# antoni-wojcik/OpenCL-Raytracing

Hardware: AMD Instinct MI355X
Metric: Msamples/sec (rays/sec) at 1920×1080, 64 spp; % HBM roofline (higher is better)
Workload: dtype f32

## Files before the change

### include/rt_amd.h

```cpp
#ifndef RT_AMD_H
#define RT_AMD_H

#include <stddef.h>
#include <stdint.h>

#ifdef __cplusplus
extern "C" {
#endif

#define RT_ABI_VERSION 3

#define RT_OK 0
#define RT_EINVAL (-1)
#define RT_ENODEVICE (-2)
#define RT_EHIP (-3)
#define RT_ESTATE (-4)
#define RT_ERANGE (-5)

#define RT_TRIANGLE_EPSILON 0.0000001f
#define RT_MIN_DISTANCE 0.001f
#define RT_MAX_DISTANCE 1000.0f
#define RT_DEPTH 30
#define RT_RANDOM_BUFFER_SIZE 100000
#define RT_RANDOM_TABLE_FLOATS (4 * RT_RANDOM_BUFFER_SIZE)
// ... 140 lines not shown
int rt_sample_counter(const rt_context *ctx, uint32_t *out);

int rt_clear(rt_context *ctx);
int rt_render_spp(rt_context *ctx, const float camera[12], uint32_t first_sample, uint32_t n_samples);
int rt_resolve(rt_context *ctx);

typedef struct rt_adaptive_params {
    uint32_t batch;
    uint32_t min_spp;
    uint32_t max_spp;
    float threshold;
    uint32_t block_w, block_h;
} rt_adaptive_params;

typedef struct rt_adaptive_stats {
    uint32_t rounds;
    uint64_t pixel_samples;
    uint32_t blocks, blocks_at_max;
} rt_adaptive_stats;

int rt_render_adaptive(rt_context *ctx, const float camera[12], const rt_adaptive_params *p, rt_adaptive_stats *out);
int rt_read_sample_counts(rt_context *ctx, uint32_t *counts, size_t bytes);
int rt_read_block_error(rt_context *ctx, float *err, size_t bytes);

typedef struct rt_feature {
    float pos[3];
    float t;
    float normal[3];
    uint32_t object;
    float albedo[3];
    uint32_t material;
    float dir[3];
    uint32_t face;
    float u, v;
    uint32_t tex;
    uint32_t flags;
} rt_feature;
#define RT_FEATURE_HIT 1u

int rt_render_features(rt_context *ctx, const float camera[12]);
int rt_read_features(rt_context *ctx, rt_feature *out, size_t bytes);
int rt_device_features(rt_context *ctx, void **d_features);

#define RT_FOLLOW_REFLECTIVE 1u
#define RT_FOLLOW_REFRACTIVE 2u
#define RT_FOLLOW_DIELECTRIC 4u
#define RT_FEATURE_CHAIN_MAX 29u
#define RT_FEATURE_CUT 2u
#define RT_FEATURE_CHAIN_LENGTH(flags) (((flags) >> 8) & 31u)
#define RT_FEATURE_CHAIN_SIGNATURE(flags) ((flags) & 0xFFFF0000u)
typedef struct rt_feature_chain_params { uint32_t follow; uint32_t max_chain; } rt_feature_chain_params;
int rt_render_features_chain(rt_context *ctx, const float camera[12], const rt_feature_chain_params *p);
int rt_feature_chain_signature(const uint32_t *objects, uint32_t n, uint32_t *sig_out);

typedef struct rt_denoise_params {
    uint32_t iterations;
    float sigma_color, sigma_normal, sigma_position, sigma_albedo;
    uint32_t flags;
} rt_denoise_params;
#define RT_DENOISE_SPLIT_OBJECTS 1u
#define RT_DENOISE_SPLIT_CHAINS 4u
#define RT_DENOISE_MAX_ITERATIONS 8u

int rt_denoise(rt_context *ctx, const rt_denoise_params *p);
int rt_read_denoised(rt_context *ctx, float *rgba, size_t bytes);
int rt_device_denoised(rt_context *ctx, void **d_rgba);

typedef struct rt_denoise_variance_params {
    uint32_t iterations;
    float sigma_luminance;
    float sigma_normal, sigma_position, sigma_albedo;
    uint32_t flags;
} rt_denoise_variance_params;
#define RT_DENOISE_VARIANCE_EPS 1e-4f

int rt_denoise_variance(rt_context *ctx, const rt_denoise_variance_params *p);
int rt_read_variance(rt_context *ctx, int which, float *out, size_t bytes);
int rt_device_variance(rt_context *ctx, int which, void **d_out);

#define RT_DENOISE_MOMENTS_MIN_COUNT 4u
int rt_read_moments(rt_context *ctx, float *m2, size_t bytes);
int rt_device_moments(rt_context *ctx, void **d_m2);
int rt_moments_merge(uint32_t nA, const float sumA[3], float m2A, uint32_t nB, const float sumB[3], float m2B, float *m2_out);
int rt_denoise_moments(rt_context *ctx, const rt_denoise_variance_params *p);

int rt_sync(rt_context *ctx);

int rt_trace_samples(rt_context *ctx, const float camera[12], const uint32_t *x, const uint32_t *y,
                     const uint32_t *sample, size_t n, float *out_rgb);


int rt_read_image(rt_context *ctx, float *rgba, size_t bytes);

int rt_read_linear(rt_context *ctx, float *rgba, size_t bytes);

int rt_device_image(rt_context *ctx, void **d_rgba);
int rt_device_accum(rt_context *ctx, void **d_rgba);

#define RT_OPT_PREFIX_SHARING 1
#define RT_OPT_MAX_THREADS_PER_LAUNCH 2
#define RT_OPT_SAMPLE_QUEUE 3
#define RT_OPT_ACCEL 4
#define RT_OPT_WALK_SLICES 5
#define RT_OPT_PREFIX_TREE 7
#define RT_OPT_WAVE_FILL 8
#define RT_OPT_PREFIX_CACHE 9
#define RT_OPT_LOOKAHEAD 10
#define RT_OPT_EXACT_GRID 11
#define RT_OPT_MOMENTS 12
#define RT_OPT_ARITH 6
#define RT_ARITH_IEEE 0
#define RT_ARITH_ROCM_OCL_NOCONTRACT 1
#define RT_ARITH_ROCM_OCL 2
int rt_set_option(rt_context *ctx, int option, int value);


int rt_enable_counters(rt_context *ctx, int enable);
int rt_reset_counters(rt_context *ctx);
int rt_get_counters(rt_context *ctx, rt_counters *out);

int rt_debug_check_accel(const rt_scene_desc *scene, uint64_t stats[8], char *err, size_t err_len);

int rt_get_debug_counters(rt_context *ctx, uint64_t out[2]);

int rt_walk_overflow(rt_context *ctx, uint32_t *flags_out);

uint64_t rt_counters_bytes(const rt_counters *c);

int rt_last_kernel_ms(rt_context *ctx, float *ms);

int rt_kernel_ms_history(rt_context *ctx, float *ms, size_t cap, size_t *n_out);

int rt_debug_hit(rt_context *ctx, int kind, const float *rays, const uint32_t *prim, const uint32_t *face, size_t n,
                 float *out12);
int rt_debug_material(rt_context *ctx, int routine, const float *in16, size_t n, float *out9);
int rt_debug_div3(rt_context *ctx, const float *in4, size_t n, float *out6);
int rt_debug_builtin(rt_context *ctx, int op, const float *in8, size_t n, float *out4);
int rt_debug_queue_sums(rt_context *ctx, const float *in3, uint32_t npix, uint32_t count, uint32_t group_log2, float *out4);

int rt_stage_ms_history(rt_context *ctx, float *first_ms, float *second_ms, size_t cap, size_t *n_out);

int rt_prefix_cache_stats(rt_context *ctx, uint64_t *hits, uint64_t *misses);

int rt_lookahead_stats(rt_context *ctx, uint64_t *batches, uint64_t *served, uint64_t *direct, uint64_t *discarded);

int rt_lookahead_plan(int width, int height, int option_value, uint32_t sample_counter, uint32_t *batch_out);

int rt_sample_units(uint32_t seg_cap, uint32_t pixels_per_unit, uint32_t count_light, uint32_t count_heavy, uint32_t *units_out);

int rt_sample_grid_stats(rt_context *ctx, uint64_t *launches, uint64_t *exact, uint64_t *workgroups, uint64_t *live_last);

int rt_debug_live_list(rt_context *ctx, uint32_t out[4]);

int rt_device_info(rt_context *ctx, char *name, size_t name_len, int *cu_count, char *arch, size_t arch_len);

#ifdef __cplusplus
}
#endif
#endif
```

### opencl-raytracing_amd/_abi.py

```python
import ctypes as C

import numpy as np

RT_ABI_VERSION = 3
DEPTH = 30
RANDOM_BUFFER_SIZE = 100000
RANDOM_TABLE_FLOATS = 4 * RANDOM_BUFFER_SIZE
MAX_DIM = 16384
MAX_SAMPLE = 65535

T_REFRACTIVE, T_REFLECTIVE, T_DIELECTRIC, T_DIFFUSE, T_TEXTURED, T_LIGHT = range(6)
MAT_NAMES = {
    "refractive": T_REFRACTIVE,
    "reflective": T_REFLECTIVE,
    "dielectric": T_DIELECTRIC,
    "diffuse": T_DIFFUSE,
    "textured": T_TEXTURED,
    "light": T_LIGHT,
}

MATERIAL = np.dtype([("type", "<i4"), ("_p0", "<i4", (3,)), ("color", "<f4", (4,)), ("extra_data", "<f4"),
                     ("_p1", "<i4", (3,))])
SPHERE = np.dtype([("pos", "<f4", (4,)), ("r", "<f4"), ("mat_ID", "<u4"), ("_p", "<u4", (2,))])
PLANE = np.dtype([("pos", "<f4", (4,)), ("normal", "<f4", (4,)), ("mat_ID", "<u4"), ("_p", "<u4", (3,))])
# ... 4 lines not shown
assert (MATERIAL.itemsize, SPHERE.itemsize, PLANE.itemsize, LENS.itemsize, MESH.itemsize, MODEL.itemsize) == \
    (48, 32, 48, 64, 16, 12)


class SceneDesc(C.Structure):
    _fields_ = [(n, C.c_void_p) for n in ("materials", "spheres", "planes", "lenses", "vertices", "uvs", "indices",
                                          "meshes", "models")] + \
               [(n, C.c_uint32) for n in ("material_count", "sphere_count", "plane_count", "lens_count",
                                          "vertex_count", "uv_count", "index_count", "mesh_count", "model_count",
                                          "_pad")]


COUNTER_FIELDS = ("samples", "bounces", "t_sphere", "t_plane", "t_lens", "t_model", "t_mesh", "t_tri", "h_tri",
                  "h_bounce", "n_scatter", "n_dielectric", "n_texfetch", "image_reads")


class Counters(C.Structure):
    _fields_ = [(n, C.c_uint64) for n in COUNTER_FIELDS]

    def as_dict(self):
        return {n: int(getattr(self, n)) for n in COUNTER_FIELDS}

    def algorithmic_bytes(self):
        c = self
        return (32 * c.t_sphere + 48 * c.t_plane + 64 * c.t_lens + 12 * c.t_model + 16 * c.t_mesh + 60 * c.t_tri +
                36 * c.h_tri + 48 * c.h_bounce + 12 * c.n_scatter + 4 * c.n_dielectric + 64 * c.n_texfetch +
                64 * c.samples + 16 * c.image_reads)


class AdaptiveParams(C.Structure):
    _fields_ = [("batch", C.c_uint32), ("min_spp", C.c_uint32), ("max_spp", C.c_uint32), ("threshold", C.c_float),
                ("block_w", C.c_uint32), ("block_h", C.c_uint32)]


ADAPTIVE_STATS_FIELDS = ("rounds", "pixel_samples", "blocks", "blocks_at_max")


class AdaptiveStats(C.Structure):
    _fields_ = [("rounds", C.c_uint32), ("pixel_samples", C.c_uint64), ("blocks", C.c_uint32),
                ("blocks_at_max", C.c_uint32)]

    def as_dict(self):
        return {n: int(getattr(self, n)) for n in ADAPTIVE_STATS_FIELDS}


def adaptive_prototypes(lib):
    vp, sz = C.c_void_p, C.c_size_t
    lib.rt_render_adaptive.argtypes = [vp, vp, C.POINTER(AdaptiveParams), C.POINTER(AdaptiveStats)]
    lib.rt_read_sample_counts.argtypes = [vp, vp, sz]
    lib.rt_read_block_error.argtypes = [vp, vp, sz]


def block_error_reference(accum, half, block_w, block_h):
    accum = np.asarray(accum, dtype=np.float32)
    half = np.asarray(half, dtype=np.float32)
    h, w = accum.shape[:2]
    with np.errstate(divide="ignore", invalid="ignore", over="ignore"):
        i = accum[..., :3] / accum[..., 3:4]
        a = half[..., :3] / half[..., 3:4]
        d = np.abs(i - a)
        num = (d[..., 0] + d[..., 1]) + d[..., 2]
        den = np.sqrt((i[..., 0] + i[..., 1]) + i[..., 2])
        ok = den > 0
        e = np.where(ok, num / np.where(ok, den, np.float32(1)), np.float32(0)).astype(np.float64)
    by, bx = -(-h // block_h), -(-w // block_w)
    pad = np.full((by * block_h, bx * block_w), np.nan)
    pad[:h, :w] = e
    return np.nanmean(pad.reshape(by, block_h, bx, block_w), axis=(1, 3))


FEATURE = np.dtype([("pos", "<f4", (3,)), ("t", "<f4"), ("normal", "<f4", (3,)), ("object", "<u4"),
                    ("albedo", "<f4", (3,)), ("material", "<u4"), ("dir", "<f4", (3,)), ("face", "<u4"),
                    ("u", "<f4"), ("v", "<f4"), ("tex", "<u4"), ("flags", "<u4")])
assert FEATURE.itemsize == 80
FEATURE_HIT = 1
FEATURE_CUT = 2
FOLLOW_REFLECTIVE, FOLLOW_REFRACTIVE, FOLLOW_DIELECTRIC = 1, 2, 4
FOLLOW_NAMES = {"mirror": FOLLOW_REFLECTIVE, "glass": FOLLOW_REFRACTIVE, "dielectric": FOLLOW_DIELECTRIC}
FEATURE_CHAIN_MAX = 29
NO_ID = 0xFFFFFFFF
OBJECT_KINDS = ("sphere", "plane", "lens", "mesh")
DENOISE_SPLIT_OBJECTS = 1
DENOISE_SPLIT_CHAINS = 4
DENOISE_MAX_ITERATIONS = 8
DENOISE_DEFAULTS = dict(iterations=5, sigma_color=0.5, sigma_normal=0.1, sigma_position=2.0, sigma_albedo=0.2,
                        split_objects=True)


def denoise_flags(split_objects, split_chains=False):
    return (DENOISE_SPLIT_OBJECTS if split_objects else 0) | (DENOISE_SPLIT_CHAINS if split_chains else 0)


class FeatureChainParams(C.Structure):
    _fields_ = [("follow", C.c_uint32), ("max_chain", C.c_uint32)]


class DenoiseParams(C.Structure):
    _fields_ = [("iterations", C.c_uint32), ("sigma_color", C.c_float), ("sigma_normal", C.c_float),
                ("sigma_position", C.c_float), ("sigma_albedo", C.c_float), ("flags", C.c_uint32)]


DENOISE_VARIANCE_EPS = 1e-4
DENOISE_VARIANCE_DEFAULTS = dict(iterations=5, sigma_luminance=4.0, sigma_normal=0.1, sigma_position=2.0,
                                 sigma_albedo=0.2, split_objects=True)


class DenoiseVarianceParams(C.Structure):
    _fields_ = [("iterations", C.c_uint32), ("sigma_luminance", C.c_float), ("sigma_normal", C.c_float),
                ("sigma_position", C.c_float), ("sigma_albedo", C.c_float), ("flags", C.c_uint32)]


def denoise_prototypes(lib):
    vp, sz = C.c_void_p, C.c_size_t
    lib.rt_render_features.argtypes = [vp, vp]
    lib.rt_read_features.argtypes = [vp, vp, sz]
    lib.rt_device_features.argtypes = [vp, C.POINTER(vp)]
    lib.rt_denoise.argtypes = [vp, C.POINTER(DenoiseParams)]
    lib.rt_read_denoised.argtypes = [vp, vp, sz]
    lib.rt_device_denoised.argtypes = [vp, C.POINTER(vp)]
    lib.rt_denoise_variance.argtypes = [vp, C.POINTER(DenoiseVarianceParams)]
    lib.rt_read_variance.argtypes = [vp, C.c_int, vp, sz]
    lib.rt_device_variance.argtypes = [vp, C.c_int, C.POINTER(vp)]
    lib.rt_render_features_chain.argtypes = [vp, vp, C.POINTER(FeatureChainParams)]
    lib.rt_feature_chain_signature.argtypes = [vp, C.c_uint32, C.POINTER(C.c_uint32)]


DENOISE_MOMENTS_MIN_COUNT = 4


def moments_prototypes(lib):
    vp, sz, u32, f32 = C.c_void_p, C.c_size_t, C.c_uint32, C.c_float
    f3 = C.POINTER(f32)
    lib.rt_read_moments.argtypes = [vp, vp, sz]
    lib.rt_device_moments.argtypes = [vp, C.POINTER(vp)]
    lib.rt_moments_merge.argtypes = [u32, f3, f32, u32, f3, f32, f3]
    lib.rt_denoise_moments.argtypes = [vp, C.POINTER(DenoiseVarianceParams)]


def prefix_cache_prototypes(lib):
    lib.rt_prefix_cache_stats.argtypes = [C.c_void_p, C.POINTER(C.c_uint64), C.POINTER(C.c_uint64)]


def lookahead_prototypes(lib):
    p64 = C.POINTER(C.c_uint64)
    lib.rt_lookahead_stats.argtypes = [C.c_void_p, p64, p64, p64, p64]
    lib.rt_lookahead_plan.argtypes = [C.c_int, C.c_int, C.c_int, C.c_uint32, C.POINTER(C.c_uint32)]


def sample_grid_prototypes(lib):
    p64, u32 = C.POINTER(C.c_uint64), C.c_uint32
    lib.rt_sample_units.argtypes = [u32, u32, u32, u32, C.POINTER(u32)]
    lib.rt_sample_grid_stats.argtypes = [C.c_void_p, p64, p64, p64, p64]
    lib.rt_debug_live_list.argtypes = [C.c_void_p, C.POINTER(u32)]


def queue_sums_prototypes(lib):
    u32 = C.c_uint32
    lib.rt_debug_queue_sums.argtypes = [C.c_void_p, C.c_void_p, u32, u32, u32, C.c_void_p]


def split_features(rec):
    return {"position": rec["pos"].copy(), "depth": rec["t"].copy(), "normal": rec["normal"].copy(),
            "albedo": rec["albedo"].copy(), "object": rec["object"].copy(), "material": rec["material"].copy(),
            "face": rec["face"].copy(), "direction": rec["dir"].copy(),
            "uv": np.stack([rec["u"], rec["v"]], axis=-1), "texture": rec["tex"].copy(),
            "hit": (rec["flags"] & FEATURE_HIT) != 0,
            "chain_length": ((rec["flags"] >> 8) & 31).astype(np.uint32),
            "chain_signature": (rec["flags"] & np.uint32(0xFFFF0000)).astype(np.uint32),
            "cut": (rec["flags"] & FEATURE_CUT) != 0, "chain_word": (rec["flags"] >> 8).astype(np.uint32)}


def ptr(a):
    if a is None or a.size == 0:
        return None
    return a.ctypes.data_as(C.c_void_p)
```

### opencl-raytracing_amd/csrc/pt_device.hpp

```cpp
#pragma once
#include "pt_arith.hpp"

namespace PT_NS {

#ifndef PT_RNG_PREFETCH
#define PT_RNG_PREFETCH 0
#endif
#ifndef PT_BEHIND_SKIP
#define PT_BEHIND_SKIP 1
#endif

#ifndef PT_FACE_MASK
#define PT_FACE_MASK 1
#endif
#ifndef PT_NO_MODELS
#define PT_NO_MODELS 0
#endif
#ifndef PT_STAMPS
#define PT_STAMPS 0
#endif
#if PT_STAMPS
#define PT_STAMP(c, k)                                                         \
    do {                                                                       \
        unsigned long long now_ = __builtin_amdgcn_s_memtime();                \
        (c).st[k] += now_ - (c).st_last;                                       \
        (c).st_last = now_;                                                    \
    } while (0)
#else
#define PT_STAMP(c, k) do { } while (0)
#endif


typedef float v4f __attribute__((ext_vector_type(4)));
typedef const v4f __attribute__((address_space(3))) *LdsV4;
PT_DEV float4 lds_ld(LdsV4 p, uint32_t i) {
    v4f t = p[i];
    return make_float4(t.x, t.y, t.z, t.w);
}
PT_DEV LdsV4 lds_ptr(const float4 *generic) { return (LdsV4)generic; }

struct Ctx {
    const DeviceScene &sc;
    LdsV4 lmat;
    LaneCounters *cn;
    LdsV4 lwin = nullptr;
    LdsV4 lpln = nullptr;
    LdsV4 lfaces = nullptr;
#if PT_STAMPS
    mutable unsigned long long st[8] = {0, 0, 0, 0, 0, 0, 0, 0};
    mutable unsigned long long st_last = 0;
#endif
};

PT_DEV float schlick_r0(float ratio) {
    float r0 = (1.0f - ratio) / (1.0f + ratio);
    r0 *= r0;
    return r0;
}

PT_DEV LdsV4 stage_materials(const DeviceScene &sc, float4 *lds) {
    const uint32_t nm = lds_mat_n(sc.material_count), nw = lds_win_n(sc.sphere_count), np = lds_pln_n(sc.plane_count);
    if (nm)
        for (uint32_t i = threadIdx.x; i < sc.material_count; i += blockDim.x) {
            const rt_material &m = sc.materials[i];
            lds[2 * i] = make_float4(m.color.x, m.color.y, m.color.z, m.extra_data);
            float inv = 1.0f / m.extra_data;
            lds[2 * i + 1] = make_float4(__int_as_float(m.type), inv, schlick_r0(m.extra_data), schlick_r0(inv));
        }
    if (nw)
        for (uint32_t i = threadIdx.x; i < sc.sphere_count; i += blockDim.x) {
            const rt_sphere &s = sc.spheres[i];
            lds[nm + 2 * i] = make_float4(s.pos.x, s.pos.y, s.pos.z, s.r);
            lds[nm + 2 * i + 1] = make_float4(__uint_as_float(s.mat_ID), 0.0f, 0.0f, 0.0f);
        }
    if (np)
        for (uint32_t i = threadIdx.x; i < sc.plane_count; i += blockDim.x) {
            const rt_plane &p = sc.planes[i];
            lds[nm + nw + i] = make_float4(p.normal.x, p.normal.y, p.normal.z, __uint_as_float(p.mat_ID));
        }
    __syncthreads();
    return nm ? lds_ptr(lds) : (LdsV4) nullptr;
}
PT_DEV LdsV4 staged_winners(const DeviceScene &sc, const float4 *lds) {
    return lds_win_n(sc.sphere_count) ? lds_ptr(lds + lds_mat_n(sc.material_count)) : (LdsV4) nullptr;
}
PT_DEV LdsV4 staged_planes(const DeviceScene &sc, const float4 *lds) {
    return lds_pln_n(sc.plane_count) ? lds_ptr(lds + lds_mat_n(sc.material_count) + lds_win_n(sc.sphere_count)) : (LdsV4) nullptr;
}

PT_DEV void load_material(const Ctx &c, uint32_t id, int &type, float &extra, V3 &col) {
    if (c.lmat) {
        float4 a = lds_ld(c.lmat, 2 * id);
        type = __float_as_int(lds_ld(c.lmat, 2 * id + 1).x);
        extra = a.w;
        col = mk(a.x, a.y, a.z);
    } else {
        const rt_material &m = c.sc.materials[id];
        type = m.type;
        extra = m.extra_data;
        col = ld3(m.color);
    }
}

PT_DEV uint32_t dir_hash(V3 d) {
    float dp = dot(d, mk(123.9898f, 348.233f, 433.3314f));
    return (uint32_t)fabs((double)dp * 438.5453);
}
struct Rnd {
    V3 v;
    float u;
};
PT_DEV Rnd fetch_rnd(const float *__restrict__ table, V3 dir, uint32_t s_seed, uint32_t gx, uint32_t gy) {
    uint32_t hsh = dir_hash(dir);
    uint32_t iv = (hsh + (s_seed * 2683u + gx * 3931u + gy * 2504u) * 3u) % RT_RANDOM_BUFFER_SIZE;
    uint32_t iu = (hsh + (s_seed * 2683u + gx * 3931u + gy)) % RT_RANDOM_BUFFER_SIZE;
    const float *t = table + iv;
    Rnd r;
    r.v = mk(t[0], t[1], t[2]);
    r.u = table[3 * RT_RANDOM_BUFFER_SIZE + iu];
    return r;
}

PT_DEV uint32_t rnd_base_v(uint32_t sample, uint32_t gx, uint32_t gy) { return (sample * 2683u + gx * 3931u + gy * 2504u) * 3u; }
PT_DEV uint32_t rnd_base_u(uint32_t sample, uint32_t gx, uint32_t gy) { return sample * 2683u + gx * 3931u + gy; }
PT_DEV Rnd fetch_rnd_b(const float *__restrict__ table, V3 dir, uint32_t depth, uint32_t bv, uint32_t bu) {
    uint32_t hsh = dir_hash(dir);
    uint32_t iv = (hsh + bv + depth * 8049u) % RT_RANDOM_BUFFER_SIZE;
    uint32_t iu = (hsh + bu + depth * 2683u) % RT_RANDOM_BUFFER_SIZE;
    const float *t = table + iv;
    Rnd r;
    r.v = mk(t[0], t[1], t[2]);
    r.u = table[3 * RT_RANDOM_BUFFER_SIZE + iu];
    return r;
}

enum : uint32_t { K_SPHERE = 0u << 30, K_PLANE = 1u << 30, K_LENS = 2u << 30, K_MESH = 3u << 30, K_MASK = 3u << 30 };
#define PT_NO_HIT 0xFFFFFFFFu

#define PT_MISS INFINITY
template <bool FAST = false>
PT_DEV float sphere_root(float b, float cc, float dis);
PT_DEV void sphere_disc(const Ray &r, float4 s, float &b, float &cc, float &dis) {
    V3 oc = xyz(s) - r.o;
    b = dot(oc, r.d);
#if PT_CONTRACT
    cc = __builtin_fmaf(-s.w, s.w, dot(oc, oc));
    dis = __builtin_fmaf(b, b, -cc);
#else
    cc = dot(oc, oc) - s.w;
    dis = b * b - cc;
#endif
}
template <bool FAST = false>
PT_DEV float sphere_t(const Ray &r, float4 s) {
    float b, cc, dis;
    sphere_disc(r, s, b, cc, dis);
    return sphere_root<FAST>(b, cc, dis);
}
#define PT_SPHERE_W_IS_RADIUS PT_CONTRACT
#define PT_BVH_END 0x0FFFFFFFu
#ifndef PT_SPHERE_LEAF_EVERY
#define PT_SPHERE_LEAF_EVERY 4u
#endif
PT_DEV bool sphere_needs_roots(float b, float cc, float dis) {
    return dis > 0 && !(PT_BEHIND_SKIP && b < 0.0f && cc > 0.0f && b > (PT_OCL ? -1024.0f : -4096.0f));
}
template <bool FAST = false>
PT_DEV float sphere_roots(float b, float dis) {
    float d = sqrt1<FAST>(dis);
    float t = PT_MISS;
    float t0 = b - d;
    if (in_range(t0)) t = t0;
    else {
        float t1 = b + d;
        if (in_range(t1)) t = t1;
    }
    return t;
}
template <bool FAST>
PT_DEV float sphere_root(float b, float cc, float dis) {
    return sphere_needs_roots(b, cc, dis) ? sphere_roots<FAST>(b, dis) : PT_MISS;
}
#ifndef PT_ROOT_UPDATE
#define PT_ROOT_UPDATE 1
#endif
template <bool FAST>
PT_DEV void sphere_take(const Ray &r, float4 s, uint32_t id, float &best_t, uint32_t &best_id) {
    float b, cc, dis;
    sphere_disc(r, s, b, cc, dis);
    if (sphere_needs_roots(b, cc, dis)) {
        const float t = sphere_roots<FAST>(b, dis);
        if (t < best_t) {
            best_t = t;
            best_id = id;
        }
    }
}
template <class T>
PT_DEV const T *at32(const T *base, uint32_t byte_offset) {
    return reinterpret_cast<const T *>(reinterpret_cast<const char *>(base) + byte_offset);
}

PT_DEV V3 cull_inverse(V3 d) {
    V3 i = mk(__builtin_amdgcn_rcpf(d.x), __builtin_amdgcn_rcpf(d.y), __builtin_amdgcn_rcpf(d.z));
    return mk(fminf(fmaxf(i.x, -1.0e30f), 1.0e30f), fminf(fmaxf(i.y, -1.0e30f), 1.0e30f), fminf(fmaxf(i.z, -1.0e30f), 1.0e30f));
}
template <bool COUNT>
PT_DEV void hit_spheres_bvh(const DeviceScene &sc, const Ray &r, float &best_t, uint32_t &best_id, LaneCounters *cn) {
    float dd = dot(r.d, r.d);
    float c_ray = 2.0e-6f + 2.0f * fabsf(dd - 1.0f) * (__builtin_amdgcn_rcpf(fminf(dd, 1.0f)) * 1.000002f);
    float k_ray = __builtin_amdgcn_sqrtf(2.0f * c_ray) * 1.02f;
    float o_max = fmaxf(fmaxf(fabsf(r.o.x), fabsf(r.o.y)), fabsf(r.o.z));
    V3 inv = cull_inverse(r.d);
    const uint32_t oct = (r.d.x < 0.0f ? 1u : 0u) | (r.d.y < 0.0f ? 2u : 0u) | (r.d.z < 0.0f ? 4u : 0u);

    uint32_t cur = 1u;
    uint32_t best_slot = PT_NO_HIT;
    bool at_leaf = false;
    uint32_t leaf_b = 0, leaf_skip = 0;
    for (uint32_t guard = 0; guard < (PT_SPHERE_LEAF_EVERY + 1u) * sc.bvh_node_count + 8u; guard++) {
      if (cur != PT_BVH_END && !at_leaf) {
        float4 a = *at32(sc.bvh_nodes, cur << 4);
        float4 b = *at32(sc.bvh_links, (cur << 7) + (oct << 4));
        uint32_t skip = __float_as_uint(b.x) & PT_BVH_END;
        {
            const uint32_t axis_bits = __float_as_uint(b.x) & 0x30000000u, child = __float_as_uint(a.w);
            a.w = __uint_as_float(axis_bits);
            b = make_float4(b.y, b.z, b.w, __uint_as_float(child));
        }
        uint32_t A = __float_as_uint(a.w), B = __float_as_uint(b.w);
        asm("" : "+v"(A), "+v"(B), "+v"(skip));
        if (COUNT) cn->c[CN_DBG_BVH_NODES]++;
        const V3 dc = mk(a.x - r.o.x, a.y - r.o.y, a.z - r.o.z);
        float fx = fabsf(dc.x) + b.x, fy = fabsf(dc.y) + b.y, fz = fabsf(dc.z) + b.z;
// ... 701 lines not shown
```

### opencl-raytracing_amd/csrc/pt_kernels.hip

```cpp
#include <hip/hip_runtime.h>

#include <algorithm>

#include "pt_device.hpp"
#include "pt_moments.hpp"
#include "pt_chain.hpp"
#include "rt_context.hpp"
#include "pt_kernels.hpp"

namespace PT_NS {
using namespace rtamd;


PT_DEV uint32_t live_take(const FrameParams &fp, const uint32_t *__restrict__ live_count, uint32_t unit, uint32_t want,
                          uint32_t &first) {
    const uint32_t cap = fp.seg_cap;
    const uint32_t cnt_l = min(live_count[0], cap);
    const uint32_t cnt_h = min(live_count[LIVE_HEAVY_COUNTER], cap - cnt_l);
    const uint32_t units_h = want ? (cnt_h + want - 1u) / want : 0u;
    const bool heavy = unit < units_h;
    const uint32_t cnt = heavy ? cnt_h : cnt_l;
    const unsigned long long start64 = (unsigned long long)(heavy ? unit : unit - units_h) * want;
    const uint32_t start = (uint32_t)min(start64, (unsigned long long)cnt);
    first = (heavy ? cap - cnt_h : 0u) + start;
// ... 214 lines not shown
    if (!COUNT && is_final) {
        uint32_t before = 0;
        for (uint32_t k = 0; k < wv; k++) before += s_wave_f[k];
        FinalPix e;
        e.slot = slot;
        e.r = rec.out.x;
        e.g = rec.out.y;
        e.b = rec.out.z;
        finals[blockIdx.x * 256u + before + lanes_below(fm)] = e;
    }
    if (!COUNT && threadIdx.x == 0) final_n[blockIdx.x] = s_wave_f[0] + s_wave_f[1] + s_wave_f[2] + s_wave_f[3];
    flush_counters<COUNT>(cn, counters, fp.count);
    if (!TREES) return;
    const uint32_t tree0 = s_tree0;
    const uint32_t nt = tree0 < fp.tree_cap ? min(s_wave_g[0] + s_wave_g[1] + s_wave_g[2] + s_wave_g[3], fp.tree_cap - tree0) : 0u;
    if (nt == 0u) return;
    if (glass) {
        uint32_t before = 0;
        for (uint32_t k = 0; k < wv; k++) before += s_wave_g[k];
        const uint32_t j = before + lanes_below(gm);
        if (j < nt) {
            s_tpos[j] = pos;
            fp.trees[tree0 + j].dec[0].hsh = 0u;
        }
    }
    __syncthreads();
    for (uint32_t level = 0; level < PT_TREE_LEVELS; level++) {
        const uint32_t items = 2u * (level ? s_wn[level] : nt);
        for (uint32_t t = threadIdx.x; t < items; t += 256u) {
            const uint32_t e = level ? (uint32_t)s_wait[(level - 1u) & 1u][t >> 1] : (1u << 8) | (t >> 1);
            const uint32_t j = e & 0xFFu, heap = e >> 8, which = t & 1u, tree = tree0 + j;
            if (tree_step<ACCEL>(c, fp.trees + tree, tree, heap, which, level + 1u == PT_TREE_LEVELS, recs + s_tpos[j],
                                 fp.tree_wait + (size_t)tree * PT_TREE_WAITS)) {
                const uint32_t k = atomicAdd(&s_wn[level + 1u], 1u);
                s_wait[level & 1u][k] = (uint16_t)(((2u * heap + which) << 8) | j);
            }
        }
        if (level + 1u < PT_TREE_LEVELS) __syncthreads();
    }
}

__global__ __launch_bounds__(256) void pt_final_replay(FrameParams fp, const FinalPix *__restrict__ finals,
                                                       const uint32_t *__restrict__ final_n, float4 *__restrict__ accum) {
    if (threadIdx.x >= min(final_n[blockIdx.x], 256u)) return;
    const FinalPix e = finals[blockIdx.x * 256u + threadIdx.x];
    uint32_t x = 0, y = 0;
    if (!slot_to_pixel(fp, e.slot, x, y)) return;
    const V3 fsum = final_sum(mk(e.r, e.g, e.b), fp.count, fp.group_log2);
    if (fp.m2) moments_update(accum, fp.m2, (size_t)y * fp.w + x, fsum, fp.count, 0.0f);
    accumulate(accum, (size_t)y * fp.w + x, fsum, fp.count);
}

PT_DEV size_t ring_at(const FrameParams &fp, size_t pix, uint32_t j) {
    return PT_RING_PIXEL_MAJOR ? pix * fp.count + j : j * ((size_t)fp.w * fp.h) + pix;
}

__global__ __launch_bounds__(256) void pt_final_retrace(FrameParams fp, const FinalPix *__restrict__ finals,
                                                        const uint32_t *__restrict__ final_n) {
    if (threadIdx.x >= min(final_n[blockIdx.x], 256u)) return;
    const FinalPix e = finals[blockIdx.x * 256u + threadIdx.x];
    uint32_t x = 0, y = 0;
    if (!slot_to_pixel(fp, e.slot, x, y)) return;
    const size_t pix = (size_t)y * fp.w + x;
    const float4 at = fp.la_image[pix];
    V3 prev = mk(at.x, at.y, at.z);
    const V3 sum = mk(0.0f, 0.0f, 0.0f) + mk(e.r, e.g, e.b);
    for (uint32_t j = 0; j < fp.count; j++) {
        prev = retrace_step(prev, sum, fp.first + j);
        fp.la_ring[ring_at(fp, pix, j)] = make_float4(prev.x, prev.y, prev.z, 1.0f);
    }
}

template <bool COUNT, bool ACCEL>
__global__ __launch_bounds__(256) void pt_samples(DeviceScene sc, FrameParams fp, const PixelRec *__restrict__ recs,
                                                  const uint32_t *__restrict__ live,
                                                  const uint32_t *__restrict__ live_count,
                                                  float4 *__restrict__ accum, unsigned long long *counters) {
    __shared__ float4 s_mat[PT_LDS_STATIC_FLOAT4];
    {
        uint32_t e0 = 0;
        if (live_take(fp, live_count, (blockIdx.x * 256u) >> fp.group_log2, 1u, e0) == 0u) return;
    }
    LaneCounters cn;
    if (COUNT) zero_counters(cn);
    Ctx c{sc, stage_materials(sc, s_mat), &cn};
    c.lwin = staged_winners(sc, s_mat);
    c.lpln = staged_planes(sc, s_mat);

    uint32_t tid = blockIdx.x * 256u + threadIdx.x;
    uint32_t g = 1u << fp.group_log2;
    uint32_t li = tid >> fp.group_log2;
    uint32_t lane = tid & (g - 1u);
    uint32_t entry = 0;
    bool valid = live_take(fp, live_count, li, 1u, entry) != 0u;
    uint32_t x = 0, y = 0;
    V3 sum = mk(0.0f, 0.0f, 0.0f);
    const bool mom = fp.m2 != nullptr;
    LaneMoments lm{0.0f, 0.0f};
    if (valid) {
        uint32_t slot = live[entry];
        (void)slot_to_pixel(fp, slot, x, y);
        PixelRec rec = recs[entry];
        for (uint32_t s = fp.first + lane; s < fp.first + fp.count; s += g) {
            if (COUNT) cn.c[CN_SAMPLES]++;
            const V3 rad = radiance_from_rec<COUNT, ACCEL>(c, rec, s, x, y, fp.trees);
            if (mom) moments_fold(lm, sum, rad);
            sum = sum + rad;
        }
    }
    sum = mom ? group_sum_moments(sum, lm, g) : group_sum(sum, g);
    if (valid && lane == 0) {
        if (mom) moments_update(accum, fp.m2, (size_t)y * fp.w + x, sum, fp.count, lm.m2);
        accumulate(accum, (size_t)y * fp.w + x, sum, fp.count);
    }
    flush_counters<COUNT>(cn, counters, 1);
}

#ifndef QUEUE_SLOTS
#define QUEUE_SLOTS 512
#endif
#ifndef PT_REFILL_MIN
#define PT_REFILL_MIN 1
#endif
#ifndef QUEUE_MAX_PIXELS
#define QUEUE_MAX_PIXELS 16
#endif
#define QUEUE_REC_F4 5u
#define QUEUE_XY_F4 1u
static_assert(sizeof(PixelRec) == QUEUE_REC_F4 * sizeof(float4), "a queue record is a PixelRec");
PT_HD uint32_t queue_pixel_bytes(uint32_t count) { return (QUEUE_REC_F4 + QUEUE_XY_F4) * 16u + count * 3u * 4u; }
PT_HD uint32_t queue_xy_f4(uint32_t pixels_per_wave) { return pixels_per_wave * QUEUE_REC_F4; }
PT_HD uint32_t queue_slot_f4(uint32_t pixels_per_wave) { return pixels_per_wave * (QUEUE_REC_F4 + QUEUE_XY_F4); }
PT_HD uint32_t queue_wave_lds_bytes(uint32_t pixels_per_wave, uint32_t count) {
    return (pixels_per_wave * queue_pixel_bytes(count) + 15u) & ~15u;
}
PT_HD uint32_t queue_faces_f4(const DeviceScene &sc) { return lds_static_used(sc.material_count, sc.sphere_count, sc.plane_count); }
PT_HD uint32_t queue_static_f4(const DeviceScene &sc, uint32_t face_f4) { return queue_faces_f4(sc) + face_f4; }
#ifndef PT_Q_WAVES
#define PT_Q_WAVES 6
#endif
#ifndef PT_Q_WAVES_ACCEL
#define PT_Q_WAVES_ACCEL 5
#endif
#ifndef PT_Q_WAVES_SPHERE_BVH
#define PT_Q_WAVES_SPHERE_BVH 6
#endif
static_assert(QUEUE_SLOTS >= RT_SPP_PER_LAUNCH, "rt_render_spp's launches must fit a wave's sample queue");
#ifndef QUEUE_MIN_SAMPLES
#define QUEUE_MIN_SAMPLES 384u
#endif
#ifndef PT_LDS_GRANULE
#define PT_LDS_GRANULE 1024u
#endif
__host__ inline uint32_t queue_pixels_per_wave(uint32_t count, uint32_t waves, uint32_t static_float4) {
    auto fit = [&](uint32_t waves_per_simd) {
        uint32_t workgroups = waves_per_simd * 4u;
        uint32_t budget = 163840u / workgroups / PT_LDS_GRANULE * PT_LDS_GRANULE;
        uint32_t per_wave = budget - static_float4 * (uint32_t)sizeof(float4) - 15u;
        uint32_t p = per_wave / queue_pixel_bytes(count);
        if (p * count > QUEUE_SLOTS) p = QUEUE_SLOTS / count;
        return p > QUEUE_MAX_PIXELS ? (uint32_t)QUEUE_MAX_PIXELS : p;
    };
    uint32_t p = fit(waves);
    if (p * count < QUEUE_MIN_SAMPLES) {
        uint32_t p5 = fit(5u);
        if (p5 > p) p = p5;
    }
    return p < 1u ? 1u : p;
}
#ifndef PT_UNITS_PER_WAVE_SLOT
#define PT_UNITS_PER_WAVE_SLOT 16u
#endif
#ifndef PT_TREE_MIN_SAMPLES
#define PT_TREE_MIN_SAMPLES 24u
#endif
#ifndef PT_LDS_FACE_CAP
#define PT_LDS_FACE_CAP 64u
#endif

struct alignas(16) QueueF4 { float x, y, z, w; };
struct alignas(16) QueueXY { uint32_t x, y, bv, bu; };
typedef QueueF4 __attribute__((address_space(3))) *LdsQueueF4;
typedef QueueXY __attribute__((address_space(3))) *LdsQueueXY;
typedef float __attribute__((address_space(3))) *LdsF32;
typedef v4f __attribute__((address_space(3))) *LdsV4Rw;
struct WaveQueue {
    LdsQueueF4 rec;
    LdsQueueXY xy;
    LdsF32 slot;
    uint32_t npix;
    uint32_t count;
    uint32_t total;
    uint32_t count_log2;
    float inv_count;
};

PT_DEV WaveQueue queue_stage(const DeviceScene &sc, const FrameParams &fp, const PixelRec *__restrict__ recs,
                             const uint32_t *__restrict__ live, uint32_t npix, uint32_t pix0,
                             uint32_t pixels_per_wave, float4 *lds, uint32_t face_f4) {
    float4 *wave_lds = lds + queue_static_f4(sc, face_f4);
    WaveQueue q;
    q.rec = (LdsQueueF4)wave_lds;
    q.xy = (LdsQueueXY)(wave_lds + queue_xy_f4(pixels_per_wave));
    q.slot = (LdsF32)(wave_lds + queue_slot_f4(pixels_per_wave));
    const uint32_t lane = threadIdx.x;
    q.npix = npix;
    q.count = fp.count;
    q.total = q.npix * q.count;
    for (uint32_t i = lane; i < q.npix * QUEUE_REC_F4; i += 64u) {
        uint32_t p = i / QUEUE_REC_F4, part = i - p * QUEUE_REC_F4;
        const float4 t = reinterpret_cast<const float4 *>(recs + pix0 + p)[part];
        *(LdsV4Rw)(q.rec + i) = v4f{t.x, t.y, t.z, t.w};
    }
    if (lane < q.npix) {
        uint32_t x = 0, y = 0;
        (void)slot_to_pixel(fp, live[pix0 + lane], x, y);
        q.xy[lane].x = x;
        q.xy[lane].y = y;
        q.xy[lane].bv = rnd_base_v(0u, x, y);
        q.xy[lane].bu = rnd_base_u(0u, x, y);
    }
    __builtin_amdgcn_fence(__ATOMIC_SEQ_CST, "wavefront");
    __builtin_amdgcn_wave_barrier();
    q.inv_count = fp.inv_count;
    q.count_log2 = (q.count & (q.count - 1u)) == 0u ? (uint32_t)__builtin_ctz(q.count) : 0xFFu;
    return q;
}

struct QueueEntry {
    float4 q0, q1, q2, q3, q4;
    uint32_t bits, bv, bu;
};
PT_DEV QueueEntry queue_fetch(const WaveQueue &q, const DeviceScene &sc, const FrameParams &fp, uint32_t idx) {
    const uint32_t p = q.count_log2 != 0xFFu ? idx >> q.count_log2 : (uint32_t)(((float)idx + 0.5f) * q.inv_count);
    const uint32_t sample = fp.first + (idx - p * q.count);
    auto part = [&](uint32_t k) {
        const LdsQueueF4 f = q.rec + (QUEUE_REC_F4 * p + k);
        return make_float4(f->x, f->y, f->z, f->w);
    };
    QueueEntry e;
    e.q0 = part(0);
    e.q1 = part(1);
    e.q2 = part(2);
    e.q3 = part(3);
    e.q4 = part(4);
    e.bv = sample * 8049u + q.xy[p].bv;
    e.bu = sample * 2683u + q.xy[p].bu;
    e.bits = __float_as_uint(e.q0.w);
    if ((e.bits & 0xFFu) == REC_TREE) {
        const float4 *lf = tree_leaf(fp.trees + __float_as_uint(e.q4.w), sc.table, e.bu);
        e.q0 = lf[0]; e.q1 = lf[1]; e.q2 = lf[2]; e.q3 = lf[3]; e.q4 = lf[4];
        e.bits = __float_as_uint(e.q0.w);
    }
    return e;
}

PT_DEV void queue_put(const WaveQueue &q, uint32_t idx, V3 rgb) {
    q.slot[3 * idx] = rgb.x;
    q.slot[3 * idx + 1] = rgb.y;
    q.slot[3 * idx + 2] = rgb.z;
}

#ifndef PT_QUEUE_SUMS_TREE
#define PT_QUEUE_SUMS_TREE 1
#endif
PT_DEV V3 queue_lane_sum(const WaveQueue &q, uint32_t p, uint32_t l, uint32_t g) {
    V3 sum = mk(0.0f, 0.0f, 0.0f);
    const uint32_t n = p < q.npix ? q.count : 0u;
    for (uint32_t j = l; j < n; j += g) {
        const LdsF32 sl = q.slot + 3u * (p * q.count + j);
        sum = sum + mk(sl[0], sl[1], sl[2]);
    }
    return sum;
}
template <int OFF>
PT_DEV float row_add(float v) {
    return v + __int_as_float(__builtin_amdgcn_update_dpp(0, __float_as_int(v), 0x100 + OFF, 0xF, 0xF, false));
}
template <int OFF>
PT_DEV V3 row_add(V3 v) { return mk(row_add<OFF>(v.x), row_add<OFF>(v.y), row_add<OFF>(v.z)); }
PT_DEV float row_pair_add(float a, float b) {
    const auto r = __builtin_amdgcn_permlane16_swap(__float_as_uint(a), __float_as_uint(b), false, false);
    return __uint_as_float(r[0]) + __uint_as_float(r[1]);
}
PT_DEV void queue_sums_tree(const WaveQueue &q, const FrameParams &fp, float4 *__restrict__ accum) {
    const uint32_t lane = threadIdx.x, gl = fp.group_log2;
    if (gl >= 5u) {
        const uint32_t half = lane >> 5, i = lane & 31u, g = 1u << gl, row = lane >> 4;
        for (uint32_t pb = 0; pb < q.npix; pb += 4u) {
            V3 a = queue_lane_sum(q, pb + half, i, g), b = queue_lane_sum(q, pb + 2u + half, i, g);
            if (gl == 6u) {
                a = a + queue_lane_sum(q, pb + half, i + 32u, g);
                b = b + queue_lane_sum(q, pb + 2u + half, i + 32u, g);
            }
            V3 sum = mk(row_pair_add(a.x, b.x), row_pair_add(a.y, b.y), row_pair_add(a.z, b.z));
            sum = row_add<1>(row_add<2>(row_add<4>(row_add<8>(sum))));
            const uint32_t p = pb + ((row & 1u) << 1 | row >> 1);
            if (p < q.npix && (lane & 15u) == 0u) accumulate(accum, (size_t)q.xy[p].y * fp.w + q.xy[p].x, sum, q.count);
        }
    } else {
        const uint32_t g = 1u << gl, ppp = 64u >> gl;
        for (uint32_t pb = 0; pb < q.npix; pb += ppp) {
            const uint32_t p = pb + (lane >> gl), l = lane & (g - 1u);
            V3 sum = queue_lane_sum(q, p, l, g);
            if (gl >= 4u) sum = row_add<8>(sum);
            if (gl >= 3u) sum = row_add<4>(sum);
            if (gl >= 2u) sum = row_add<2>(sum);
            if (gl >= 1u) sum = row_add<1>(sum);
            if (p < q.npix && l == 0u) accumulate(accum, (size_t)q.xy[p].y * fp.w + q.xy[p].x, sum, q.count);
        }
    }
}
template <bool MOMENTS, bool BUTTERFLY = false>
PT_DEV void queue_sums(const WaveQueue &q, const FrameParams &fp, float4 *__restrict__ accum) {
    __builtin_amdgcn_fence(__ATOMIC_SEQ_CST, "wavefront");
    __builtin_amdgcn_wave_barrier();
    if (PT_QUEUE_SUMS_TREE && !MOMENTS && !BUTTERFLY) return queue_sums_tree(q, fp, accum);
    const uint32_t lane = threadIdx.x;
    const uint32_t g = 1u << fp.group_log2, ppp = 64u >> fp.group_log2;
    for (uint32_t pb = 0; pb < q.npix; pb += ppp) {
        uint32_t p = pb + (lane >> fp.group_log2), l = lane & (g - 1u);
        V3 sum = mk(0.0f, 0.0f, 0.0f);
        if (p < q.npix)
            for (uint32_t j = l; j < q.count; j += g) {
                const LdsF32 sl = q.slot + 3u * (p * q.count + j);
                sum = sum + mk(sl[0], sl[1], sl[2]);
            }
        sum = group_sum(sum, g);
        if (MOMENTS) {
            const float mean = moments_lum(sum.x, sum.y, sum.z) / (float)q.count;
            float dev2 = 0.0f;
            if (p < q.npix)
                for (uint32_t j = l; j < q.count; j += g) {
                    const LdsF32 sl = q.slot + 3u * (p * q.count + j);
                    const float d = moments_lum(sl[0], sl[1], sl[2]) - mean;
                    dev2 += d * d;
                }
            for (uint32_t off = g >> 1; off > 0; off >>= 1) dev2 += __shfl_xor(dev2, off);
            if (p < q.npix && l == 0) moments_update(accum, fp.m2, (size_t)q.xy[p].y * fp.w + q.xy[p].x, sum, q.count, dev2);
        }
        if (p < q.npix && l == 0) accumulate(accum, (size_t)q.xy[p].y * fp.w + q.xy[p].x, sum, q.count);
    }
}

static_assert(QUEUE_MAX_PIXELS * 4u <= 64u, "queue_replay maps (pixel, channel) to the wave's lanes");
PT_DEV void queue_replay(const WaveQueue &q, const FrameParams &fp) {
    __builtin_amdgcn_fence(__ATOMIC_SEQ_CST, "wavefront");
    __builtin_amdgcn_wave_barrier();
    const uint32_t lane = threadIdx.x, ch = lane & 3u;
    const bool alpha = ch == 3u;
    for (uint32_t pb = 0; pb < q.npix; pb += 16u) {
        const uint32_t p = pb + (lane >> 2);
        if (p >= q.npix) continue;
        const size_t pix = (size_t)q.xy[p].y * fp.w + q.xy[p].x;
        float prev = reinterpret_cast<const float *>(fp.la_image)[4u * pix + ch];
        float *out = reinterpret_cast<float *>(fp.la_ring) + ch;
        const LdsF32 sl = q.slot + 3u * (p * q.count) + (alpha ? 0u : ch);
        for (uint32_t j = 0; j < q.count; j++) {
            prev = retrace_step1(prev, 0.0f + sl[3u * j], fp.first + j);
            out[4u * ring_at(fp, pix, j)] = alpha ? 1.0f : prev;
        }
    }
}

template <bool COUNT, bool ACCEL, int GEOM, int WAVES, bool MOMENTS = false>
__global__ __launch_bounds__(64, WAVES) void pt_samples_q(DeviceScene sc, FrameParams fp, const PixelRec *__restrict__ recs,
                                                    const uint32_t *__restrict__ live,
                                                    const uint32_t *__restrict__ live_count,
                                                    float4 *__restrict__ accum, unsigned long long *counters,
                                                    uint32_t pixels_per_wave) {
    extern __shared__ float4 s_dyn[];
    constexpr bool FAST = PT_OCL && !COUNT && !ACCEL && GEOM != 2;
    uint32_t pix0 = 0;
    const uint32_t npix = live_take(fp, live_count, blockIdx.x, pixels_per_wave, pix0);
    if (npix == 0u) return;
    float4 *s_mat = s_dyn;
    LaneCounters cn;
    if (COUNT) zero_counters(cn);
    Ctx c{sc, stage_materials(sc, s_mat), &cn};
    c.lwin = staged_winners(sc, s_mat);
    c.lpln = staged_planes(sc, s_mat);
    if (GEOM != 0 && fp.lds_face_f4) {
        float4 *s_faces = s_dyn + queue_faces_f4(sc);
        for (uint32_t i = threadIdx.x; i < fp.lds_face_f4; i += blockDim.x) s_faces[i] = sc.faces[i];
        __syncthreads();
        c.lfaces = lds_ptr(s_faces);
    }

    const WaveQueue q = queue_stage(sc, fp, recs, live, npix, pix0, pixels_per_wave, s_dyn, GEOM != 0 ? fp.lds_face_f4 : 0u);

    uint32_t next = 0;
    bool active = false;
    uint32_t idx = 0, depth = 0, bv = 0, bu = 0;
    V3 col = mk(0.0f, 0.0f, 0.0f), out = mk(0.0f, 0.0f, 0.0f);
    Ray r;
    r.o = r.d = mk(0.0f, 0.0f, 0.0f);
    V3 hn = mk(0.0f, 0.0f, 0.0f);
    uint32_t hmat = 0;
    Rnd rnd;
    rnd.v = mk(0.0f, 0.0f, 0.0f);
    rnd.u = 0.0f;

#if PT_STAMPS
    c.st_last = __builtin_amdgcn_s_memtime();
#endif
    while (true) {
        PT_STAMP(c, 5);
        bool need = !active;
        unsigned long long m = __ballot(need);
        if (m && next < q.total && ((uint32_t)__popcll(m) >= PT_REFILL_MIN || m == ~0ull)) {
            uint32_t cand = next + lanes_below(m);
            if (need && cand < q.total) {
                idx = cand;
                const QueueEntry e = queue_fetch(q, sc, fp, idx);
                bv = e.bv;
                bu = e.bu;
                if (COUNT) cn.c[CN_SAMPLES]++;
                depth = (e.bits >> 8) & 0xFFu;
                hn = xyz(e.q1);
                r.o = xyz(e.q0);
                r.d = xyz(e.q2);
                hmat = __float_as_uint(e.q2.w);
                out = xyz(e.q3);
                col = xyz(e.q4);
                if ((e.bits & 0xFFu) == REC_FINAL) {
                    queue_put(q, idx, out);
                } else {
                    if (PT_RNG_PREFETCH) rnd = fetch_rnd_b(sc.table, r.d, depth, bv, bu);
                    active = true;
                }
            }
            next += (uint32_t)__popcll(m);
        }
        if (!__any(active) && next >= q.total) break;
        PT_STAMP(c, 0);
#ifdef PT_EXP_PAD
#define PT_STR2(x) #x
#define PT_STR(x) PT_STR2(x)
#ifdef PT_EXP_PAD_NOP
        asm volatile(".rept " PT_STR(PT_EXP_PAD) "\n\tv_nop\n\t.endr");
#else
        asm volatile(".rept " PT_STR(PT_EXP_PAD) "\n\tv_or_b32 %0, %0, %0\n\t.endr" : "+v"(idx));
#endif
#endif
#ifdef PT_QSTAT
        if (COUNT && __any(active)) {
            uint32_t na = (uint32_t)__popcll(__ballot(active));
            if (threadIdx.x == 0) cn.c[CN_DBG_BVH_NODES] += na;
            if (threadIdx.x == 0) cn.c[CN_DBG_BVH_TESTS] += 64u;
        }
#endif
        if (active) {
            if (!PT_RNG_PREFETCH) rnd = fetch_rnd_b(sc.table, r.d, depth, bv, bu);
            Hit at;
            at.p = r.o;
            at.n = hn;
            at.u = at.v = 0.0f;
            at.tex = 0;
            at.mat = hmat;
            int type;
            float extra;
            V3 mcol;
            load_material(c, hmat, type, extra, mcol);
            scatter<COUNT, FAST>(c, r, out, at, type, extra, col, rnd, false);
            depth++;
            if (depth >= RT_DEPTH) {
                queue_put(q, idx, out);
                active = false;
            }
        }
        PT_STAMP(c, 1);
        if (active) {
            if (PT_RNG_PREFETCH == 1) rnd = fetch_rnd_b(sc.table, r.d, depth, bv, bu);
            V3 res;
            bool done = false;
            Hit h;
            Nearest nb;
            hit_primitives<COUNT, ACCEL, GEOM != 0, FAST>(c, r, nb);
            if (GEOM != 0) hit_models<COUNT, GEOM == 2>(c, r, nb);
            if (!hit_finish<COUNT, GEOM == 0>(c, r, nb, h)) {
                res = mk(0.0f, 0.0f, 0.0f);
                done = true;
            } else {
                if (COUNT) cn.c[CN_H_BOUNCE]++;
                r.o = h.p;
                hn = h.n;
                hmat = h.mat;
                int type;
                float extra;
                load_material(c, h.mat, type, extra, col);
                if (type == RT_LIGHT) {
                    res = vmin(out, col);
                    done = true;
                } else if (type == RT_TEXTURED) {
                    if (COUNT) cn.c[CN_N_TEXFETCH]++;
                    col = texture_rgb(c.sc, h.u, h.v, h.tex);
                }
            }
            if (done) {
                queue_put(q, idx, res);
                active = false;
            } else if (PT_RNG_PREFETCH == 2) {
                rnd = fetch_rnd_b(sc.table, r.d, depth, bv, bu);
            }
        }
        PT_STAMP(c, 4);
    }
#if PT_STAMPS
    if (threadIdx.x == 0 && q.npix)
        for (int k = 0; k < 6; k++) atomicAdd(&counters[(size_t)COUNTER_REPLICAS * COUNTER_STRIDE + k], c.st[k]);
#endif
    if (!COUNT && !MOMENTS && fp.la_ring) queue_replay(q, fp);
    else queue_sums<MOMENTS, COUNT || ACCEL>(q, fp, accum);
    flush_counters<COUNT>(cn, counters, 1);
}

#ifndef PT_WALK_STEPS
#define PT_WALK_STEPS 24u
#endif
#ifndef PT_W_CHEAP_AGAIN
#define PT_W_CHEAP_AGAIN 8u
#endif
#ifndef PT_W_CHEAP_REPEATS
#define PT_W_CHEAP_REPEATS 4u
#endif
#ifndef PT_W_WAVES
#define PT_W_WAVES 6
#endif
#ifndef PT_W_WAVES_MULTI
#define PT_W_WAVES_MULTI 4
#endif
template <bool MULTI, bool MOMENTS = false>
__global__ __launch_bounds__(64, MULTI ? PT_W_WAVES_MULTI : PT_W_WAVES) void pt_samples_w(DeviceScene sc, FrameParams fp, const PixelRec *__restrict__ recs,
                                                    const uint32_t *__restrict__ live,
                                                    const uint32_t *__restrict__ live_count,
                                                    float4 *__restrict__ accum, uint32_t pixels_per_wave,
                                                    const uint2 *__restrict__ jobs, uint32_t n_jobs
#ifdef PT_WSTAT
                                                    , unsigned long long *wstat
#endif
                                                    ) {
    extern __shared__ float4 s_dyn[];
    uint32_t pix0 = 0;
    const uint32_t npix = live_take(fp, live_count, blockIdx.x, pixels_per_wave, pix0);
    if (npix == 0u) return;
    float4 *s_mat = s_dyn;
    Ctx c{sc, stage_materials(sc, s_mat), nullptr};
    c.lwin = staged_winners(sc, s_mat);
    c.lpln = staged_planes(sc, s_mat);
    const WaveQueue q = queue_stage(sc, fp, recs, live, npix, pix0, pixels_per_wave, s_dyn, 0u);

    const uint32_t mesh0 = jobs[0].x, mat0 = jobs[0].y;
    const uint32_t faces0 = sc.meshes[mesh0].face_count;
    const uint32_t root0 = sc.mesh_bvh_root[mesh0];

    uint32_t next = 0;
    bool active = false;
    int phase = 0;
    uint32_t idx = 0, depth = 0, bv = 0, bu = 0;
    V3 col = mk(0.0f, 0.0f, 0.0f), out = mk(0.0f, 0.0f, 0.0f);
    Ray r;
    r.o = r.d = mk(0.0f, 0.0f, 0.0f);
    V3 hn = mk(0.0f, 0.0f, 0.0f);
    uint32_t hmat = 0;
    float nb_t = RT_MAX_DISTANCE;
    uint32_t nb_id = PT_NO_HIT;
    MeshWalk wpos = mesh_walk_start(0);
    uint32_t wbest = 0;
    float wt = 0.0f, wu = 0.0f, wv = 0.0f;
    uint32_t job = 0;
    uint32_t nb_face = 0, nb_mat = 0;
    float nb_u = 0.0f, nb_v = 0.0f;

    auto enter_job = [&]() {
        while (job < n_jobs) {
            const uint32_t mesh_n = jobs[job].x;
            wbest = sc.meshes[mesh_n].face_count;
            wt = wu = wv = 0.0f;
            wpos = mesh_walk_first(sc, r, sc.mesh_bvh_root[mesh_n], wbest);
            if (wpos.cur != PT_MESH_END) return true;
            job++;
        }
        return false;
    };
#ifdef PT_WSTAT
    WalkStat ws = {0, 0, 0, 0, 0};
    unsigned long long it_n = 0, it_active = 0, it_p0 = 0, it_p1 = 0, it_p2 = 0, it_walk_calls = 0;
#endif
    for (unsigned long long guard = ((unsigned long long)q.total + 1ull) * (RT_DEPTH + 2ull) * (3ull * (1ull << 28) / PT_WALK_STEPS + 4ull); guard; guard--) {
        const bool walking = active && phase == 1;
        const bool wants_cheap = (active && phase != 1) || (!active && next < q.total);
        const uint32_t n_cheap = (uint32_t)__popcll(__ballot(wants_cheap));
        const bool any_walk = __any(walking);
        if (n_cheap == 0u && !any_walk) break;
#ifdef PT_WSTAT
        it_n++;
        it_active += __popcll(__ballot(active));
        it_p0 += __popcll(__ballot(active && phase == 0));
        it_p1 += __popcll(__ballot(active && phase == 1));
        it_p2 += __popcll(__ballot(active && phase == 2));
#endif
        if (n_cheap) {
          for (uint32_t again = 0;; again++) {
            if (active && phase == 2) {
                Nearest nb;
                nb.t = nb_t;
                nb.id = nb_id;
                if (MULTI) {
                    nb.face = nb_face;
                    nb.mat = nb_mat;
                    nb.u = nb_u;
                    nb.v = nb_v;
                } else if (wbest < faces0 && wt < RT_MAX_DISTANCE && wt < nb.t) {
                    nb.t = wt;
                    nb.id = K_MESH | mesh0;
                    nb.face = wbest;
                    nb.mat = mat0;
                    nb.u = wu;
                    nb.v = wv;
                }
                V3 res;
                bool done = false;
                Hit h;
                h.p = h.n = mk(0.0f, 0.0f, 0.0f);
                h.u = h.v = 0.0f;
                h.tex = h.mat = 0;
                if (!hit_finish<false>(c, r, nb, h)) {
                    res = mk(0.0f, 0.0f, 0.0f);
                    done = true;
                } else {
                    int type;
                    float extra;
                    load_material(c, h.mat, type, extra, col);
                    if (type == RT_LIGHT) {
                        res = vmin(out, col);
                        done = true;
                    } else if (type == RT_TEXTURED) {
                        col = texture_rgb(c.sc, h.u, h.v, h.tex);
                    }
                }
                phase = 0;
                if (done) {
                    queue_put(q, idx, res);
                    active = false;
                } else {
                    r.o = h.p;
                    hn = h.n;
                    hmat = h.mat;
                }
            }
            bool need = !active;
            unsigned long long m = __ballot(need);
            if (m && next < q.total) {
                uint32_t cand = next + lanes_below(m);
                if (need && cand < q.total) {
                    idx = cand;
                    const QueueEntry e = queue_fetch(q, sc, fp, idx);
                    bv = e.bv;
                    bu = e.bu;
                    if ((e.bits & 0xFFu) == REC_FINAL) {
                        queue_put(q, idx, xyz(e.q3));
                    } else {
                        depth = (e.bits >> 8) & 0xFFu;
                        hn = xyz(e.q1);
                        r.o = xyz(e.q0);
                        r.d = xyz(e.q2);
                        hmat = __float_as_uint(e.q2.w);
// ... 261 lines not shown
        }
        if (t < PT_MISS) {
            nb.t = t;
            hit = hit_finish<false>(c, r, nb, h);
            if (kind == 4) h.mat = h.tex = 0;
        }
    }
    put_hit(out + 12 * (size_t)i, hit, nb.t, h);
}

__global__ __launch_bounds__(256) void pt_debug_material(DeviceScene sc, int routine, const float *__restrict__ in,
                                                         uint32_t n, float *__restrict__ out) {
    __shared__ float4 s_mat[PT_LDS_STATIC_FLOAT4];
    Ctx c{sc, stage_materials(sc, s_mat), nullptr};
    uint32_t i = blockIdx.x * 256u + threadIdx.x;
    if (i >= n) return;
    const float *v = in + 16 * (size_t)i;
    Ray r;
    r.o = mk(0.0f, 0.0f, 0.0f);
    r.d = mk(v[0], v[1], v[2]);
    Hit h;
    h.p = mk(v[3], v[4], v[5]);
    h.n = mk(v[6], v[7], v[8]);
    h.u = h.v = 0.0f;
    h.tex = 0;
    h.mat = __float_as_uint(v[12]);
    V3 out_col = mk(v[9], v[10], v[11]);
    uint32_t seed = __float_as_uint(v[13]), gx = __float_as_uint(v[14]), gy = __float_as_uint(v[15]);
    int type;
    float extra;
    V3 col;
    load_material(c, h.mat, type, extra, col);
    int as_type = routine == 0 ? (type == RT_REFLECTIVE ? RT_REFLECTIVE : -1) : routine == 1 ? RT_REFRACTIVE
                  : routine == 2 ? RT_DIFFUSE : RT_DIELECTRIC;
    Rnd rnd = fetch_rnd(sc.table, r.d, seed, gx, gy);
    if (as_type == -1) {
        float k = 2.0f * dot(r.d, h.n);
        r.o = h.p;
        r.d = normalize(nmad(h.n, k, r.d));
    } else {
        scatter<false>(c, r, out_col, h, as_type, extra, mk(INFINITY, INFINITY, INFINITY), rnd);
    }
    float *o = out + 9 * (size_t)i;
    o[0] = r.o.x; o[1] = r.o.y; o[2] = r.o.z;
    o[3] = r.d.x; o[4] = r.d.y; o[5] = r.d.z;
    o[6] = out_col.x; o[7] = out_col.y; o[8] = out_col.z;
}

__global__ __launch_bounds__(256) void pt_debug_div3(const float *__restrict__ in, uint32_t n, float *__restrict__ out) {
    uint32_t i = blockIdx.x * 256u + threadIdx.x;
    if (i >= n) return;
    V3 a = mk(in[4 * i], in[4 * i + 1], in[4 * i + 2]);
    float d = in[4 * i + 3];
    V3 q = a / d, s = q;
    if (div3_in_range(a, d)) {
        float nd = -d, rr = __builtin_amdgcn_rcpf(d);
        float e = __builtin_fmaf(nd, rr, 1.0f);
        rr = __builtin_fmaf(e, rr, rr);
        s = V3{div_shared(a.x, nd, rr), div_shared(a.y, nd, rr), div_shared(a.z, nd, rr)};
    }
    float *o = out + 6 * (size_t)i;
    o[0] = s.x; o[1] = s.y; o[2] = s.z; o[3] = q.x; o[4] = q.y; o[5] = q.z;
}

__global__ __launch_bounds__(64) void pt_debug_queue_sums(const float *__restrict__ in, uint32_t npix, uint32_t count,
                                                          uint32_t group_log2, float4 *__restrict__ accum) {
    __shared__ float4 s_q[QUEUE_MAX_PIXELS * QUEUE_XY_F4 + (QUEUE_SLOTS * 3u + 3u) / 4u];
    WaveQueue q;
    q.rec = nullptr;
    q.xy = (LdsQueueXY)s_q;
    q.slot = (LdsF32)(s_q + QUEUE_MAX_PIXELS * QUEUE_XY_F4);
    q.npix = npix;
    q.count = count;
    q.total = npix * count;
    q.count_log2 = 0xFFu;
    q.inv_count = 0.0f;
    const uint32_t lane = threadIdx.x;
    if (lane < npix) {
        q.xy[lane].x = lane;
        q.xy[lane].y = 0u;
    }
    for (uint32_t i = lane; i < 3u * q.total; i += 64u) q.slot[i] = in[i];
    FrameParams fp = {};
    fp.w = (int)npix;
    fp.h = 1;
    fp.count = count;
    fp.group_log2 = group_log2;
    queue_sums<false>(q, fp, accum);
}


#define PT_DISPATCH(count_on, accel_on, CALL)                           \
    do {                                                                \
        if (count_on) { if (accel_on) CALL(true, true); else CALL(true, false); }   \
        else { if (accel_on) CALL(false, true); else CALL(false, false); }          \
    } while (0)

static void apply_mask(FrameParams &fp, const BlockMask *mask) {
    if (!mask) return;
    fp.block_active = mask->active;
    fp.blk_w_log2 = mask->w_log2;
    fp.blk_h_log2 = mask->h_log2;
    fp.blocks_x = mask->blocks_x;
}

template <int MODE>
int launch_render(rt_context *ctx, const float cam[12], uint32_t first, uint32_t count, uint32_t glog2, float4 *accum,
                  const BlockMask *mask, float *m2) {
    FrameParams fp = frame_params(ctx, cam, first, count, glog2);
    apply_mask(fp, mask);
    fp.m2 = MODE == MODE_ACCUM ? m2 : nullptr;
    DeviceScene sc = device_scene(ctx);
    uint32_t slots = fp.slot_end;
    if (slots == 0) return RT_OK;
    uint32_t slots_per_launch = ctx->max_threads_per_launch >> glog2;
    if (slots_per_launch == 0) slots_per_launch = 1;
    hipEvent_t *evp = ctx->ev[ctx->ev_count % rt_context::EV_RING];
    HIP_TRY(ctx, hipEventRecord(evp[0], ctx->stream));
    HIP_TRY(ctx, hipEventRecord(evp[2], ctx->stream));
    for (uint32_t b = 0; b < slots; b += slots_per_launch) {
        fp.slot_begin = b;
        fp.slot_end = b + slots_per_launch < slots ? b + slots_per_launch : slots;
        uint64_t threads = (uint64_t)(fp.slot_end - fp.slot_begin) << glog2;
        dim3 grid((unsigned)((threads + 255) / 256)), block(256);
#define PT_CALL(C, A) \
    hipLaunchKernelGGL((pt_render<MODE, C, A>), grid, block, 0, ctx->stream, sc, fp, accum, ctx->image.p, ctx->counters.p)
        PT_DISPATCH(ctx->count_enabled, scene_has_accel(sc), PT_CALL);
#undef PT_CALL
    }
    HIP_TRY(ctx, hipGetLastError());
    HIP_TRY(ctx, hipEventRecord(evp[1], ctx->stream));
    ctx->ev_count++;
    return RT_OK;
}

static int launch_fused_any(rt_context *ctx, const float cam[12], uint32_t first, uint32_t count, uint32_t glog2, float4 *accum,
                            const BlockMask *mask, float4 *ring, float *m2) {
    FrameParams fp = frame_params(ctx, cam, first, count, glog2);
    apply_mask(fp, mask);
    fp.m2 = m2;
    if (ring) {
        if (accum || m2 || mask || ctx->count_enabled || ctx->world != 1 || !ctx->sample_queue || count > QUEUE_SLOTS ||
            (ctx->max_threads_per_launch >> glog2) < fp.slot_end)
            return fail(ctx, RT_EINVAL, "a look-ahead launch needs the sample queue, an unsharded frame in one slot range and no counters");
        fp.la_ring = ring;
        fp.la_image = ctx->image.p;
    }
    DeviceScene sc = device_scene(ctx);
    uint32_t slots = fp.slot_end;
    if (slots == 0) return RT_OK;
    int rc = ensure_slots(ctx, slots);
    if (rc) return rc;
    const rt_context::Slots &ss = ctx->slots;
    uint32_t *live_count = ss.live.p + ss.capacity + 256u;
    uint32_t slots_per_launch = ctx->max_threads_per_launch >> glog2;
    if (slots_per_launch == 0) slots_per_launch = 1;
    rt_context::PrefixCache &pc = ctx->prefix_cache;
    const bool tree_on = ctx->prefix_tree == 2 || (ctx->prefix_tree == 1 && count >= PT_TREE_MIN_SAMPLES);
    const bool keepable = !mask && !ctx->count_enabled && slots_per_launch >= slots;
    uint32_t cam_bits[12];
    memcpy(cam_bits, cam, sizeof cam_bits);
    const bool hit = pc.enabled && pc.valid && keepable && pc.key_generation == pc.generation && pc.key_tree_on == tree_on &&
                     memcmp(pc.key_cam, cam_bits, sizeof cam_bits) == 0;
    pc.valid = false;
    rt_context::SampleGrid &sg = ctx->sample_grid;
    if (!hit) pc.counts_state = rt_context::PrefixCache::COUNTS_UNKNOWN;
    else if (sg.exact && pc.counts_state == rt_context::PrefixCache::COUNTS_UNKNOWN) {
        HIP_TRY(ctx, hipMemcpyAsync(sg.h_counts, live_count, LIVE_COUNT_STRIDE * sizeof(uint32_t), hipMemcpyDeviceToHost, ctx->stream));
        HIP_TRY(ctx, hipEventRecord(sg.counts_ev, ctx->stream));
        pc.counts_state = rt_context::PrefixCache::COUNTS_IN_FLIGHT;
    } else if (sg.exact && pc.counts_state == rt_context::PrefixCache::COUNTS_IN_FLIGHT) {
        const hipError_t q = hipEventQuery(sg.counts_ev);
        if (q == hipSuccess) {
            pc.count_light = sg.h_counts[0];
            pc.count_heavy = sg.h_counts[LIVE_HEAVY_COUNTER];
            pc.counts_state = rt_context::PrefixCache::COUNTS_KNOWN;
        } else {
            (void)hipGetLastError();
            if (q != hipErrorNotReady) return fail(ctx, RT_EHIP, "hipEventQuery: %s", hipGetErrorString(q));
        }
    }
    const bool exact = hit && sg.exact && pc.counts_state == rt_context::PrefixCache::COUNTS_KNOWN;
    hipEvent_t *evp = ctx->ev[ctx->ev_count % rt_context::EV_RING];
    HIP_TRY(ctx, hipEventRecord(evp[0], ctx->stream));
    for (uint32_t b = 0; b < slots; b += slots_per_launch) {
        fp.slot_begin = b;
        fp.slot_end = b + slots_per_launch < slots ? b + slots_per_launch : slots;
        uint32_t n = fp.slot_end - fp.slot_begin;
        if (!hit) HIP_TRY(ctx, hipMemsetAsync(live_count, 0, LIVE_COUNT_STRIDE * sizeof(uint32_t), ctx->stream));
        fp.trees = ss.trees.p;
        fp.tree_wait = ss.tree_wait.p;
        fp.tree_count = live_count + LIVE_TREE_COUNTER;
        fp.tree_cap = (tree_on && !ctx->count_enabled) ? (uint32_t)ss.tree_capacity : 0u;
        const uint32_t prefix_blocks = (n + 255) / 256;
        fp.seg_cap = prefix_blocks * 256u;
        dim3 block(256), grid1(prefix_blocks);
        fp.lds_face_f4 = 0u;
        uint32_t static_f4 = queue_static_f4(sc, 0u);
        const bool sphere_bvh_only = sc.bvh_node_count != 0 && sc.mesh_bvh_root == nullptr;
        const bool simple_geom = sc.lens_count == 0 && sc.model_count == 0;
        const uint32_t q_waves = !scene_has_accel(sc) ? PT_Q_WAVES : ((sphere_bvh_only && simple_geom) ? PT_Q_WAVES_SPHERE_BVH : PT_Q_WAVES_ACCEL);
        uint32_t ppw = queue_pixels_per_wave(count, q_waves, static_f4);
        const uint32_t want_units = (uint32_t)(ctx->cu_count > 0 ? ctx->cu_count : 256) * 4u * 6u * PT_UNITS_PER_WAVE_SLOT;
        const uint32_t ppw_full = (64u + count - 1u) / count;
        const uint32_t ppw_par = !ctx->wave_fill ? QUEUE_MAX_PIXELS : std::max(n / want_units, ppw_full);
        if (ppw > ppw_par) ppw = ppw_par;
        if (PT_FACE_MASK && !simple_geom && sc.mesh_bvh_root == nullptr && !ctx->count_enabled) {
            const size_t nf = ctx->h_faces.size() / 3u - (ctx->h_faces.empty() ? 0u : 1u);
            if (nf > 0 && nf <= PT_LDS_FACE_CAP &&
                queue_pixels_per_wave(count, q_waves, static_f4 + 3u * (uint32_t)nf) >= ppw) {
                fp.lds_face_f4 = 3u * (uint32_t)nf;
                static_f4 = queue_static_f4(sc, fp.lds_face_f4);
            }
        }
        bool queue = ctx->sample_queue && count <= QUEUE_SLOTS;
        auto queue_lds = [&](uint32_t pixels_per_wave) { return static_f4 * sizeof(float4) + (size_t)queue_wave_lds_bytes(pixels_per_wave, count); };
#define PT_LAUNCH_PREFIX(K) \
    hipLaunchKernelGGL(K, grid1, block, 0, ctx->stream, sc, fp, ss.recs.p, ss.live.p, live_count, accum, ctx->counters.p, ss.finals.p, ss.final_n.p)
#define PT_CALL_PREFIX(C, A) PT_LAUNCH_PREFIX((pt_prefix<C, A>))
        bool accel_on = scene_has_accel(sc);
        if (hit && !ring) hipLaunchKernelGGL(pt_final_replay, grid1, block, 0, ctx->stream, fp, ss.finals.p, ss.final_n.p, accum);
        else if (hit) {}
        else if (fp.tree_cap) PT_LAUNCH_PREFIX((accel_on ? pt_prefix<false, true, true> : pt_prefix<false, false, true>));
        else PT_DISPATCH(ctx->count_enabled, accel_on, PT_CALL_PREFIX);
#undef PT_CALL_PREFIX
#undef PT_LAUNCH_PREFIX
        if (ring) hipLaunchKernelGGL(pt_final_retrace, grid1, block, 0, ctx->stream, fp, ss.finals.p, ss.final_n.p);
        HIP_TRY(ctx, hipEventRecord(evp[2], ctx->stream));
        uint32_t launched = 0;
        auto units = [&](uint32_t per_unit) {
            uint32_t u = (fp.seg_cap + per_unit - 1) / per_unit + 1u;
            sg.last_cap = fp.seg_cap;
            sg.last_per_unit = per_unit;
            if (exact) (void)rt_sample_units(fp.seg_cap, per_unit, pc.count_light, pc.count_heavy, &u);
            return u;
        };
#define PT_GRID(U, LAUNCH) do { launched = (U); if (launched) { LAUNCH; } } while (0)
#define PT_CALL_QUEUE_M(C, A, G, W, M) \
    PT_GRID(units(ppw), hipLaunchKernelGGL((pt_samples_q<C, A, G, W, M>), dim3(launched), dim3(64), queue_lds(ppw), ctx->stream, sc, fp, ss.recs.p, ss.live.p, live_count, accum, ctx->counters.p, ppw))
#define PT_CALL_QUEUE_W(C, A, G, W) do { if (fp.m2) PT_CALL_QUEUE_M(C, A, G, W, true); else PT_CALL_QUEUE_M(C, A, G, W, false); } while (0)
#define PT_CALL_QUEUE(C, A)                                                                       \
    do {                                                                                          \
        if (!(A)) { if (simple_geom) PT_CALL_QUEUE_W(C, false, 0, PT_Q_WAVES); else PT_CALL_QUEUE_W(C, false, 1, PT_Q_WAVES); } \
        else if (sphere_bvh_only) { if (simple_geom) PT_CALL_QUEUE_W(C, true, 0, PT_Q_WAVES_SPHERE_BVH); else PT_CALL_QUEUE_W(C, true, 1, PT_Q_WAVES_ACCEL); } \
        else PT_CALL_QUEUE_W(C, true, 2, PT_Q_WAVES_ACCEL);                                       \
    } while (0)
#define PT_CALL_FIXED(C, A) \
    PT_GRID(grid2.x, hipLaunchKernelGGL((pt_samples<C, A>), grid2, block, 0, ctx->stream, sc, fp, ss.recs.p, ss.live.p, live_count, accum, ctx->counters.p))
        if (queue && sc.mesh_bvh_root && ctx->walk_jobs.n && ctx->walk_slices && !ctx->count_enabled) {
            const bool multi = ctx->walk_jobs.n != 1;
            uint32_t ppw_w = queue_pixels_per_wave(count, multi ? PT_W_WAVES_MULTI : PT_W_WAVES, static_f4);
            if (ppw_w > ppw_par) ppw_w = ppw_par;
            launched = units(ppw_w);
            if (launched)
            hipLaunchKernelGGL(fp.m2 ? (multi ? pt_samples_w<true, true> : pt_samples_w<false, true>) : (multi ? pt_samples_w<true> : pt_samples_w<false>), dim3(launched), dim3(64), queue_lds(ppw_w), ctx->stream,
                               sc, fp, ss.recs.p, ss.live.p, live_count, accum, ppw_w, ctx->walk_jobs.p, (uint32_t)ctx->walk_jobs.n
#ifdef PT_WSTAT
                               , ctx->counters.p + COUNTER_REPLICAS * COUNTER_STRIDE + 8
#endif
                               );
        } else if (queue) PT_DISPATCH(ctx->count_enabled, accel_on, PT_CALL_QUEUE);
        else {
            dim3 grid2((unsigned)((((uint64_t)units(1u) << glog2) + 255) / 256));
            PT_DISPATCH(ctx->count_enabled, accel_on, PT_CALL_FIXED);
        }
#undef PT_CALL_QUEUE
#undef PT_CALL_QUEUE_W
#undef PT_CALL_QUEUE_M
#undef PT_CALL_FIXED
#undef PT_GRID
        sg.launches++;
        sg.workgroups += launched;
        if (exact) { sg.exact_launches++; sg.live_last = launched; }
    }
    HIP_TRY(ctx, hipGetLastError());
    HIP_TRY(ctx, hipEventRecord(evp[1], ctx->stream));
    ctx->ev_count++;
    if (hit) pc.hits++; else pc.misses++;
    if (keepable) {
        pc.valid = true;
        pc.key_generation = pc.generation;
        pc.key_tree_on = tree_on;
        memcpy(pc.key_cam, cam_bits, sizeof cam_bits);
    }
    return RT_OK;
}

int launch_fused(rt_context *ctx, const float cam[12], uint32_t first, uint32_t count, uint32_t glog2, float4 *accum,
                 const BlockMask *mask, float *m2) {
    return launch_fused_any(ctx, cam, first, count, glog2, accum, mask, nullptr, m2);
}

int launch_lookahead(rt_context *ctx, const float cam[12], uint32_t first, uint32_t count, float4 *ring) {
    if (!ring || count < 1u) return fail(ctx, RT_EINVAL, "look-ahead launch without a ring");
    return launch_fused_any(ctx, cam, first, count, group_log2_for(count), nullptr, nullptr, ring, nullptr);
}

__global__ __launch_bounds__(256) void pt_face_normals(float4 *__restrict__ rec, uint32_t n) {
    uint32_t i = blockIdx.x * 256u + threadIdx.x;
    if (i >= n) return;
    float4 q0 = rec[3 * (size_t)i], q1 = rec[3 * (size_t)i + 1], q2 = rec[3 * (size_t)i + 2];
    V3 e1 = mk(q0.w, q1.x, q1.y), e2 = mk(q1.z, q1.w, q2.x);
    V3 nn = normalize(cross(e1, e2));
    rec[3 * (size_t)i + 2] = make_float4(q2.x, nn.x, nn.y, nn.z);
}

__global__ __launch_bounds__(256) void pt_debug_builtin(int op, const float *__restrict__ in, uint32_t n, float *__restrict__ out) {
    uint32_t i = blockIdx.x * 256u + threadIdx.x;
    if (i >= n) return;
    const float *a = in + 8 * (size_t)i;
    V3 x = mk(a[0], a[1], a[2]), y = mk(a[3], a[4], a[5]);
    float t = a[6];
    float4 o = make_float4(0.0f, 0.0f, 0.0f, 0.0f);
    if (op == 0) o.x = dot(x, y);
    else if (op == 1) { V3 c = cross(x, y); o = make_float4(c.x, c.y, c.z, 0.0f); }
    else if (op == 2) { V3 c = normalize(x); o = make_float4(c.x, c.y, c.z, 0.0f); }
    else if (op == 3) { o.x = a[0] / a[1]; o.y = 1.0f / a[0]; V3 c = x / t; o.z = c.y; o.w = c.z; }
    else if (op == 4) o.x = sqrt1(a[0]);
    else if (op == 5) o = make_float4(mix1(x.x, y.x, t), mix1(x.y, y.y, t), mix1(x.z, y.z, t), 0.0f);
    else if (op == 6) { V3 c = vmin(x, y); o = make_float4(c.x, c.y, c.z, 0.0f); }
    else if (op == 7) o.x = sign1(a[0]);
    else if (op == 8) o.x = pow5(a[0]);
    else if (op == 9) o.x = __uint_as_float(dir_hash(x));
    else if (op == 10) o.x = sqrt1<true>(a[0]);
    else if (op == 11) { V3 c = normalize<true>(x); o = make_float4(c.x, c.y, c.z, 0.0f); }
    reinterpret_cast<float4 *>(out)[i] = o;
}

namespace {

int ks_launch_render(rt_context *ctx, int mode, const float cam[12], uint32_t first, uint32_t count, uint32_t glog2,
                     float4 *accum, const BlockMask *mask, float *m2) {
    switch (mode) {
        case MODE_ACCUM: return launch_render<MODE_ACCUM>(ctx, cam, first, count, glog2, accum, mask, m2);
        case MODE_TRACE: return launch_render<MODE_TRACE>(ctx, cam, first, count, glog2, accum, mask, m2);
        case MODE_RETRACE: return launch_render<MODE_RETRACE>(ctx, cam, first, count, glog2, accum, mask, m2);
        default: return fail(ctx, RT_EINVAL, "unknown render mode %d", mode);
    }
}

int ks_launch_probe(rt_context *ctx, const FrameParams &fp, const DeviceScene &sc, const uint32_t *d_in, uint32_t n, float *d_out) {
    dim3 grid((n + 255u) / 256u), block(256);
    if (scene_has_accel(sc))
        hipLaunchKernelGGL(pt_probe<true>, grid, block, 0, ctx->stream, sc, fp, d_in, d_in + n, d_in + 2 * (size_t)n, n, d_out);
    else
        hipLaunchKernelGGL(pt_probe<false>, grid, block, 0, ctx->stream, sc, fp, d_in, d_in + n, d_in + 2 * (size_t)n, n, d_out);
    HIP_TRY(ctx, hipGetLastError());
    return RT_OK;
}

int ks_launch_features(rt_context *ctx, const FrameParams &fp, const DeviceScene &sc, rt_feature *d_out) {
    const uint32_t n = (uint32_t)fp.w * (uint32_t)fp.h;
    dim3 grid((n + 255u) / 256u), block(256);
    float4 *o = reinterpret_cast<float4 *>(d_out);
    if (scene_has_accel(sc)) hipLaunchKernelGGL(pt_features<true>, grid, block, 0, ctx->stream, sc, fp, o);
    else hipLaunchKernelGGL(pt_features<false>, grid, block, 0, ctx->stream, sc, fp, o);
    HIP_TRY(ctx, hipGetLastError());
    return RT_OK;
}

int ks_launch_features_chain(rt_context *ctx, const FrameParams &fp, const DeviceScene &sc, uint32_t follow, uint32_t max_chain,
                             rt_feature *d_out) {
    const uint32_t n = (uint32_t)fp.w * (uint32_t)fp.h;
    dim3 grid((n + 255u) / 256u), block(256);
    float4 *o = reinterpret_cast<float4 *>(d_out);
    if (scene_has_accel(sc)) hipLaunchKernelGGL(pt_features_chain<true>, grid, block, 0, ctx->stream, sc, fp, follow, max_chain, o);
    else hipLaunchKernelGGL(pt_features_chain<false>, grid, block, 0, ctx->stream, sc, fp, follow, max_chain, o);
    HIP_TRY(ctx, hipGetLastError());
    return RT_OK;
}

int ks_launch_debug_hit(rt_context *ctx, const DeviceScene &sc, int kind, const float *d_rays, const uint32_t *d_prim,
                        const uint32_t *d_face, uint32_t n, float *d_out) {
    dim3 grid((n + 255u) / 256u), block(256);
    if (scene_has_accel(sc))
        hipLaunchKernelGGL(pt_debug_hit<true>, grid, block, 0, ctx->stream, sc, kind, d_rays, d_prim, d_face, n, d_out);
    else
        hipLaunchKernelGGL(pt_debug_hit<false>, grid, block, 0, ctx->stream, sc, kind, d_rays, d_prim, d_face, n, d_out);
    HIP_TRY(ctx, hipGetLastError());
    return RT_OK;
}

int ks_launch_debug_material(rt_context *ctx, const DeviceScene &sc, int routine, const float *d_in, uint32_t n, float *d_out) {
    hipLaunchKernelGGL(pt_debug_material, dim3((n + 255u) / 256u), dim3(256), 0, ctx->stream, sc, routine, d_in, n, d_out);
    HIP_TRY(ctx, hipGetLastError());
    return RT_OK;
}

int ks_launch_debug_div3(rt_context *ctx, const float *d_in, uint32_t n, float *d_out) {
    hipLaunchKernelGGL(pt_debug_div3, dim3((n + 255u) / 256u), dim3(256), 0, ctx->stream, d_in, n, d_out);
    HIP_TRY(ctx, hipGetLastError());
    return RT_OK;
}

int ks_launch_debug_queue_sums(rt_context *ctx, const float *d_in, uint32_t npix, uint32_t count, uint32_t glog2, float *d_out) {
    if (npix < 1u || npix > QUEUE_MAX_PIXELS || count < 1u || npix * count > QUEUE_SLOTS || glog2 > 6u)
        return fail(ctx, RT_EINVAL, "queue_sums probe: %u pixels of %u samples do not fit one wave's queue", npix, count);
    HIP_TRY(ctx, hipMemsetAsync(d_out, 0, npix * sizeof(float4), ctx->stream));
    hipLaunchKernelGGL(pt_debug_queue_sums, dim3(1), dim3(64), 0, ctx->stream, d_in, npix, count, glog2, (float4 *)d_out);
    HIP_TRY(ctx, hipGetLastError());
    return RT_OK;
}

int ks_launch_face_normals(rt_context *ctx, float4 *d_records, uint32_t n_records) {
    if (n_records == 0) return RT_OK;
    hipLaunchKernelGGL(pt_face_normals, dim3((n_records + 255u) / 256u), dim3(256), 0, ctx->stream, d_records, n_records);
    HIP_TRY(ctx, hipGetLastError());
    return RT_OK;
}

int ks_launch_debug_builtin(rt_context *ctx, int op, const float *d_in, uint32_t n, float *d_out) {
    hipLaunchKernelGGL(pt_debug_builtin, dim3((n + 255u) / 256u), dim3(256), 0, ctx->stream, op, d_in, n, d_out);
    HIP_TRY(ctx, hipGetLastError());
    return RT_OK;
}

const pt::KernelSet g_kernel_set = {
    PT_ARITH,
#if PT_ARITH == 0
    "ieee",
#elif PT_ARITH == 1
    "rocm-opencl-nocontract",
#else
    "rocm-opencl",
#endif
    ks_launch_render, launch_fused, launch_lookahead, ks_launch_probe, ks_launch_features, ks_launch_debug_hit, ks_launch_debug_material, ks_launch_debug_div3,
    ks_launch_face_normals, ks_launch_debug_builtin, ks_launch_debug_queue_sums, ks_launch_features_chain};

}

}

namespace pt {
#if PT_ARITH == 0
const KernelSet *kernel_set_a0() { return &pt_a0::g_kernel_set; }
#elif PT_ARITH == 1
const KernelSet *kernel_set_a1() { return &pt_a1::g_kernel_set; }
#else
const KernelSet *kernel_set_a2() { return &pt_a2::g_kernel_set; }
#endif
}
```

### opencl-raytracing_amd/csrc/pt_kernels.hpp

```cpp
#pragma once
#include "rt_context.hpp"

namespace pt {

struct KernelSet {
    int arith;
    const char *name;
    int (*launch_render)(rt_context *ctx, int mode, const float cam[12], uint32_t first, uint32_t count, uint32_t glog2,
                         float4 *accum, const BlockMask *mask, float *m2);
    int (*launch_fused)(rt_context *ctx, const float cam[12], uint32_t first, uint32_t count, uint32_t glog2,
                        float4 *accum, const BlockMask *mask, float *m2);
    int (*launch_lookahead)(rt_context *ctx, const float cam[12], uint32_t first, uint32_t count, float4 *ring);
    int (*launch_probe)(rt_context *ctx, const FrameParams &fp, const DeviceScene &sc, const uint32_t *d_in, uint32_t n, float *d_out);
    int (*launch_features)(rt_context *ctx, const FrameParams &fp, const DeviceScene &sc, rt_feature *d_out);
    int (*launch_debug_hit)(rt_context *ctx, const DeviceScene &sc, int kind, const float *d_rays, const uint32_t *d_prim,
                            const uint32_t *d_face, uint32_t n, float *d_out);
    int (*launch_debug_material)(rt_context *ctx, const DeviceScene &sc, int routine, const float *d_in, uint32_t n, float *d_out);
    int (*launch_debug_div3)(rt_context *ctx, const float *d_in, uint32_t n, float *d_out);
    int (*launch_face_normals)(rt_context *ctx, float4 *d_records, uint32_t n_records);
    int (*launch_debug_builtin)(rt_context *ctx, int op, const float *d_in, uint32_t n, float *d_out);
    int (*launch_debug_queue_sums)(rt_context *ctx, const float *d_in, uint32_t npix, uint32_t count, uint32_t glog2, float *d_out);
    int (*launch_features_chain)(rt_context *ctx, const FrameParams &fp, const DeviceScene &sc, uint32_t follow, uint32_t max_chain,
                                 rt_feature *d_out);
};

const KernelSet *kernel_set_a0();
const KernelSet *kernel_set_a1();
const KernelSet *kernel_set_a2();

}
```

### opencl-raytracing_amd/csrc/pt_types.hpp

```cpp
#pragma once
#include <hip/hip_runtime.h>
#include <stdint.h>

#include "../../include/rt_amd.h"

namespace pt {

#define PT_DEV __device__ __forceinline__
#define PT_HD __host__ __device__ inline

#define PT_LDS_MATERIALS 64
#define PT_LDS_WINNERS 64
#define PT_SPHERE_BATCH 4

struct DeviceScene {
    const rt_material *materials;
    const rt_sphere *spheres;
    const float4 *sph4;
    const rt_plane *planes;
    const rt_lens *lenses;
    const rt_float3 *vertices;
    const rt_float2 *uvs;
    const uint32_t *indices;
    const rt_mesh *meshes;
    const rt_model *models;
    const float *table;
    const float4 *tex;
    int tex_w, tex_h, tex_layers;
    float tex_wf, tex_hf;
    uint32_t material_count, sphere_count, sphere_batches, plane_count, lens_count, model_count;
    const float4 *faces;
    const uint32_t *mesh_face_base;
    const float4 *mbvh_nodes;
    const float4 *mbvh_faces;
    const uint32_t *mbvh_face_idx;
    const uint32_t *mesh_bvh_root;
    const float4 *bvh_nodes;
    const float4 *bvh_sph;
    const uint32_t *bvh_idx;
    const float4 *bvh_links;
    uint32_t bvh_node_count;
    float bvh_lo[3], bvh_hi[3];
    float bvh_rmax;
    uint32_t *walk_overflow;
};

#define PT_N_COUNTERS 16
struct LaneCounters {
    uint32_t c[PT_N_COUNTERS];
};
enum {
    CN_SAMPLES, CN_BOUNCES, CN_T_SPHERE, CN_T_PLANE, CN_T_LENS, CN_T_MODEL, CN_T_MESH, CN_T_TRI, CN_H_TRI,
    CN_H_BOUNCE, CN_N_SCATTER, CN_N_DIELECTRIC, CN_N_TEXFETCH, CN_IMAGE_READS,
    CN_DBG_BVH_NODES,
    CN_DBG_BVH_TESTS
};

#define PT_LDS_PLANES 16
#define PT_LDS_STATIC_FLOAT4 (2 * PT_LDS_MATERIALS + 2 * PT_LDS_WINNERS + PT_LDS_PLANES)

PT_HD uint32_t lds_mat_n(uint32_t material_count) { return material_count <= PT_LDS_MATERIALS ? 2u * material_count : 0u; }
PT_HD uint32_t lds_win_n(uint32_t sphere_count) { return sphere_count <= PT_LDS_WINNERS ? 2u * sphere_count : 0u; }
PT_HD uint32_t lds_pln_n(uint32_t plane_count) { return plane_count <= PT_LDS_PLANES ? plane_count : 0u; }
PT_HD uint32_t lds_static_used(uint32_t material_count, uint32_t sphere_count, uint32_t plane_count) {
    return lds_mat_n(material_count) + lds_win_n(sphere_count) + lds_pln_n(plane_count);
}

struct PixelRec {
    float4 p_kind;
    float4 n_extra;
    float4 d;
    float4 out;
    float4 col;
};
enum { REC_FINAL = 0, REC_VERTEX = 1, REC_TREE = 2 };

struct FinalPix {
    uint32_t slot;
    float r, g, b;
};

#ifndef PT_TREE_LEVELS
#define PT_TREE_LEVELS 2
#endif
#define PT_TREE_DECISIONS ((1 << PT_TREE_LEVELS) - 1)
#define PT_TREE_LEAVES (1 << PT_TREE_LEVELS)
struct TreeDecision {
    uint32_t hsh;
    float prob;
    uint32_t depth;
    uint16_t child[2];
};
struct PixelTree {
    TreeDecision dec[PT_TREE_DECISIONS + 1];
    PixelRec leaf[PT_TREE_LEAVES];
};
#define PT_TREE_WAITS (PT_TREE_LEAVES - 2)

enum RenderMode { MODE_ACCUM = 0, MODE_TRACE = 1, MODE_RETRACE = 2 };

#ifndef PT_RING_PIXEL_MAJOR
#define PT_RING_PIXEL_MAJOR 0
#endif

struct FrameParams {
    float cam[12];
    int w, h;
    int tile_w_log2, tile_h_log2;
    uint32_t tiles_x, tiles_total;
    uint32_t rank, world;
    uint32_t slot_begin, slot_end;
    uint32_t first, count;
    uint32_t group_log2;
    uint32_t seg_cap;
    float inv_count;
    PixelTree *trees;
    PixelRec *tree_wait;
    uint32_t *tree_count;
    uint32_t tree_cap;
    uint32_t lds_face_f4;
    const uint32_t *block_active;
    uint32_t blk_w_log2, blk_h_log2, blocks_x;
    float4 *la_ring;
    const float4 *la_image;
    float *m2;
};

struct BlockMask {
    const uint32_t *active;
    uint32_t w_log2, h_log2, blocks_x;
};

#define LIVE_COUNT_STRIDE 32u
#define LIVE_TREE_COUNTER 16u
#define LIVE_HEAVY_COUNTER 24u

#define COUNTER_REPLICAS 512
#define COUNTER_STRIDE 16

PT_DEV bool slot_to_pixel(const FrameParams &fp, uint32_t slot, uint32_t &x, uint32_t &y) {
    uint32_t tpix_log2 = fp.tile_w_log2 + fp.tile_h_log2;
    uint32_t k = slot >> tpix_log2, in = slot & ((1u << tpix_log2) - 1u);
    uint32_t t = fp.rank + k * fp.world;
    if (t >= fp.tiles_total) return false;
    uint32_t tx = t % fp.tiles_x, ty = t / fp.tiles_x;
    x = (tx << fp.tile_w_log2) + (in & ((1u << fp.tile_w_log2) - 1u));
    y = (ty << fp.tile_h_log2) + (in >> fp.tile_w_log2);
    return x < (uint32_t)fp.w && y < (uint32_t)fp.h;
}

PT_DEV bool pixel_active(const FrameParams &fp, uint32_t x, uint32_t y) {
    return !fp.block_active || fp.block_active[(y >> fp.blk_h_log2) * fp.blocks_x + (x >> fp.blk_w_log2)] != 0u;
}

#define PT_MESH_BVH_NONE 0xFFFFFFFFu

#define PT_OVF_SPHERE_WALK 1u
#define PT_OVF_MESH_WALK 2u
#define PT_OVF_WALK_SLICES 4u

}
```

### opencl-raytracing_amd/csrc/rt_amd.hip

```cpp
#include <hip/hip_runtime.h>

#include <algorithm>
#include <cmath>
#include <cfloat>
#include <cstdarg>
#include <cstdio>
#include <cstdlib>
#include <cstring>
#include <functional>
#include <mutex>
#include <new>
#include <string>
#include <vector>

#include "rt_context.hpp"
#include "pt_kernels.hpp"
#include "pt_moments.hpp"
#include "pt_chain.hpp"
#include "mesh_bvh_build.hpp"

using namespace pt;
using namespace rtamd;


// ... 419 lines not shown
}


extern "C" {

int rt_abi_version(void) { return RT_ABI_VERSION; }

const char *rt_last_error(const rt_context *ctx) {
    if (ctx) return ctx->error.c_str();
    std::lock_guard<std::mutex> lk(g_err_mutex);
    return g_create_error.c_str();
}

int rt_make_random_table(uint64_t seed, float *out, size_t n) {
    if (!out || n != RT_RANDOM_TABLE_FLOATS) return fail(nullptr, RT_EINVAL, "table must hold %d floats", RT_RANDOM_TABLE_FLOATS);
    make_table(seed, out);
    return RT_OK;
}

int rt_create(int device, int width, int height, rt_context **out) {
    if (!out) return fail(nullptr, RT_EINVAL, "out is NULL");
    *out = nullptr;
    if (width < 1 || height < 1 || width > RT_MAX_DIM || height > RT_MAX_DIM)
        return fail(nullptr, RT_EINVAL, "frame size %dx%d outside 1..%d", width, height, RT_MAX_DIM);
    int n = 0;
    if (hipGetDeviceCount(&n) != hipSuccess || n < 1)
        return fail(nullptr, RT_ENODEVICE, "no HIP device visible (this library has no CPU path)");
    if (device < 0 || device >= n) return fail(nullptr, RT_ENODEVICE, "device %d out of range (%d visible)", device, n);
    hipDeviceProp_t prop;
    if (hipGetDeviceProperties(&prop, device) != hipSuccess) return fail(nullptr, RT_EHIP, "hipGetDeviceProperties failed");
    if (strncmp(prop.gcnArchName, "gfx950", 6) != 0)
        return fail(nullptr, RT_ENODEVICE, "device %d is %s; librt_amd.so carries gfx950 code only", device,
                    prop.gcnArchName);
    rt_context *ctx = new (std::nothrow) rt_context();
    if (!ctx) return fail(nullptr, RT_EHIP, "out of host memory");
    ctx->device = device;
    ctx->dev_name = prop.name;
    ctx->dev_arch = prop.gcnArchName;
    ctx->cu_count = prop.multiProcessorCount;
    int rc = RT_OK;
    auto bail = [&](int code) {
        {
            std::lock_guard<std::mutex> lk(g_err_mutex);
            g_create_error = ctx->error;
        }
        rt_destroy(ctx);
        return code;
    };
    if (hipSetDevice(device) != hipSuccess) { ctx->error = "hipSetDevice failed"; return bail(RT_EHIP); }
    if (hipStreamCreateWithFlags(&ctx->own_stream, hipStreamNonBlocking) != hipSuccess) { ctx->error = "hipStreamCreate failed"; return bail(RT_EHIP); }
    ctx->stream = ctx->own_stream;
    for (int i = 0; i < rt_context::EV_RING; i++)
        if (hipEventCreate(&ctx->ev[i][0]) != hipSuccess || hipEventCreate(&ctx->ev[i][1]) != hipSuccess || hipEventCreate(&ctx->ev[i][2]) != hipSuccess) { ctx->error = "hipEventCreate failed"; return bail(RT_EHIP); }
    if (ctx->counters.alloc(COUNTER_REPLICAS * COUNTER_STRIDE + 32) != hipSuccess ||
        hipMemset(ctx->counters.p, 0, (COUNTER_REPLICAS * COUNTER_STRIDE + 32) * sizeof(unsigned long long)) != hipSuccess) { ctx->error = "counter allocation failed"; return bail(RT_EHIP); }
    ctx->d_walk_overflow = reinterpret_cast<uint32_t *>(ctx->counters.p + COUNTER_REPLICAS * COUNTER_STRIDE + 24);

    ctx->arith = RT_ARITH_IEEE;
    ctx->ks = kernel_set_a0();
    if (const char *e = getenv("RT_PREFIX_CACHE")) ctx->prefix_cache.enabled = strcmp(e, "0") != 0;
    if (const char *e = getenv("RT_LOOKAHEAD")) { if (strcmp(e, "0") == 0) ctx->lookahead.k = 0; }
    if (const char *e = getenv("RT_EXACT_GRID")) ctx->sample_grid.exact = strcmp(e, "0") != 0;
    if (hipHostMalloc((void **)&ctx->sample_grid.h_counts, LIVE_COUNT_STRIDE * sizeof(uint32_t), hipHostMallocDefault) != hipSuccess ||
        hipEventCreateWithFlags(&ctx->sample_grid.counts_ev, hipEventDisableTiming) != hipSuccess) { ctx->error = "live-count read-back allocation failed"; return bail(RT_EHIP); }
    if ((rc = alloc_frame(ctx, width, height)) != RT_OK) return bail(rc);
    if ((rc = rt_set_seed(ctx, 0xC0FFEEull)) != RT_OK) return bail(rc);
    if ((rc = rt_set_textures(ctx, nullptr, 0, 0, 0)) != RT_OK) return bail(rc);
    *out = ctx;
    return RT_OK;
}

void rt_destroy(rt_context *ctx) {
    if (!ctx) return;
    (void)hipSetDevice(ctx->device);
    if (ctx->own_stream) (void)hipStreamSynchronize(ctx->own_stream);
    for (int i = 0; i < rt_context::EV_RING; i++)
        for (int k = 0; k < 3; k++)
            if (ctx->ev[i][k]) (void)hipEventDestroy(ctx->ev[i][k]);
    if (ctx->sample_grid.counts_ev) (void)hipEventDestroy(ctx->sample_grid.counts_ev);
    if (ctx->sample_grid.h_counts) (void)hipHostFree(ctx->sample_grid.h_counts);
    if (ctx->own_stream) (void)hipStreamDestroy(ctx->own_stream);
    delete ctx;
}

int rt_resize(rt_context *ctx, int width, int height) {
    if (!ctx) return RT_EINVAL;
    if (width < 1 || height < 1 || width > RT_MAX_DIM || height > RT_MAX_DIM)
        return fail(ctx, RT_EINVAL, "frame size %dx%d outside 1..%d", width, height, RT_MAX_DIM);
    HIP_TRY(ctx, hipSetDevice(ctx->device));
    HIP_TRY(ctx, hipStreamSynchronize(ctx->stream));
    return alloc_frame(ctx, width, height);
}

int rt_set_stream(rt_context *ctx, void *hip_stream) {
    if (!ctx) return RT_EINVAL;
    HIP_TRY(ctx, hipSetDevice(ctx->device));
    HIP_TRY(ctx, hipStreamSynchronize(ctx->stream));
    ctx->stream = hip_stream ? (hipStream_t)hip_stream : ctx->own_stream;
    ctx->prefix_changed();
    ctx->ev_count = 0;
    return RT_OK;
}

int rt_set_scene(rt_context *ctx, const rt_scene_desc *d) {
    if (!ctx) return RT_EINVAL;
    if (!d) return fail(ctx, RT_EINVAL, "scene is NULL");
    ctx->prefix_changed();
    ctx->walk_jobs.release();
    struct { const void *p; uint32_t n; const char *name; } arrs[] = {
        {d->materials, d->material_count, "materials"}, {d->spheres, d->sphere_count, "spheres"},
        {d->planes, d->plane_count, "planes"}, {d->lenses, d->lens_count, "lenses"},
        {d->vertices, d->vertex_count, "vertices"}, {d->uvs, d->uv_count, "uvs"},
        {d->indices, d->index_count, "indices"}, {d->meshes, d->mesh_count, "meshes"},
        {d->models, d->model_count, "models"}};
    for (auto &a : arrs)
        if (a.n && !a.p) return fail(ctx, RT_EINVAL, "%s: count %u but NULL pointer", a.name, a.n);
    if (d->uv_count != 0 && d->uv_count != d->vertex_count)
        return fail(ctx, RT_EINVAL, "uv_count (%u) must be 0 or vertex_count (%u)", d->uv_count, d->vertex_count);
    for (uint32_t i = 0; i < d->material_count; i++)
        if (d->materials[i].type < 0 || d->materials[i].type > RT_LIGHT)
            return fail(ctx, RT_EINVAL, "material %u has unknown type %d", i, d->materials[i].type);
    for (uint32_t i = 0; i < d->sphere_count; i++)
        if (d->spheres[i].mat_ID >= d->material_count) return fail(ctx, RT_ERANGE, "sphere %u: material %u does not exist", i, d->spheres[i].mat_ID);
    for (uint32_t i = 0; i < d->plane_count; i++)
        if (d->planes[i].mat_ID >= d->material_count) return fail(ctx, RT_ERANGE, "plane %u: material %u does not exist", i, d->planes[i].mat_ID);
    for (uint32_t i = 0; i < d->lens_count; i++)
        if (d->lenses[i].mat_ID >= d->material_count) return fail(ctx, RT_ERANGE, "lens %u: material %u does not exist", i, d->lenses[i].mat_ID);
    bool uses_tex = false;
    uint32_t max_tex = 0;
    for (uint32_t i = 0; i < d->model_count; i++) {
        const rt_model &mo = d->models[i];
        if (mo.mat_ID >= d->material_count) return fail(ctx, RT_ERANGE, "model %u: material %u does not exist", i, mo.mat_ID);
        if ((uint64_t)mo.mesh_anchor + mo.mesh_count > d->mesh_count) return fail(ctx, RT_ERANGE, "model %u: meshes [%u,+%u) outside the mesh array (%u)", i, mo.mesh_anchor, mo.mesh_count, d->mesh_count);
        bool textured = d->materials[mo.mat_ID].type == RT_TEXTURED;
        for (uint32_t k = 0; k < mo.mesh_count; k++) {
            const rt_mesh &me = d->meshes[mo.mesh_anchor + k];
            if (textured) {
                uses_tex = true;
                if (me.texture_ID > max_tex) max_tex = me.texture_ID;
            }
        }
    }
    for (uint32_t i = 0; i < d->mesh_count; i++) {
        const rt_mesh &me = d->meshes[i];
        if ((uint64_t)me.index_anchor + 3ull * me.face_count > d->index_count)
            return fail(ctx, RT_ERANGE, "mesh %u: indices [%u,+3*%u) outside the index array (%u)", i, me.index_anchor, me.face_count, d->index_count);
        for (uint64_t k = 0; k < 3ull * me.face_count; k++)
            if ((uint64_t)me.vertex_anchor + d->indices[me.index_anchor + k] >= d->vertex_count)
                return fail(ctx, RT_ERANGE, "mesh %u: vertex index %u (+anchor %u) outside the vertex array (%u)", i, d->indices[me.index_anchor + k], me.vertex_anchor, d->vertex_count);
    }
    HIP_TRY(ctx, hipSetDevice(ctx->device));
    HIP_TRY(ctx, hipStreamSynchronize(ctx->stream));
    ctx->have_scene = false;
    HIP_TRY(ctx, ctx->materials.upload(d->materials, d->material_count));
    HIP_TRY(ctx, ctx->spheres.upload(d->spheres, d->sphere_count));
    ctx->h_spheres.assign(d->spheres, d->spheres + d->sphere_count);
    ctx->h_bvh_idx.clear();
    {
        std::vector<uint32_t> base;
        std::vector<float4> fr;
        if (!build_face_records(d, base, fr)) return fail(ctx, RT_EINVAL, "too many faces");
        HIP_TRY(ctx, ctx->mesh_face_base.upload(base.data(), d->mesh_count));
        std::vector<float4> nodes, lfaces;
        std::vector<uint32_t> lidx, roots(d->mesh_count ? d->mesh_count : 1, PT_MESH_BVH_NONE);
        ctx->have_mesh_bvh = false;
        for (uint32_t m = 0; m < d->mesh_count; m++) {
            if (d->meshes[m].face_count < MESH_BVH_MIN_FACES || d->meshes[m].face_count >= (1u << 27)) continue;
            MeshBvhBuilder mb;
            mb.rec = &fr[3 * (size_t)base[m]];
            mb.n_faces = d->meshes[m].face_count;
            mb.nodes = &nodes;
            mb.leaf_faces = &lfaces;
            mb.leaf_idx = &lidx;
            roots[m] = mb.build();
            ctx->have_mesh_bvh = true;
        }
        if (nodes.size() / 4 >= (1u << 26) || lidx.size() >= (1u << 26)) ctx->have_mesh_bvh = false;
        if (nodes.empty()) nodes.resize(4, make_float4(0, 0, 0, 0));
        if (lfaces.empty()) lfaces.resize(3, make_float4(0, 0, 0, 0));
        {
            std::vector<uint8_t> is_root(nodes.size() / 4, 0);
            for (uint32_t m = 0; m < d->mesh_count; m++) if (roots[m] != PT_MESH_BVH_NONE && roots[m] < is_root.size()) is_root[roots[m]] = 1;
            mesh_collapse_links(nodes, is_root);
            std::vector<float4> packed(nodes.size() / 4 * 3);
            for (size_t n = 0; n < nodes.size() / 4; n++) mesh_node_pack(&nodes[4 * n], &packed[3 * n]);
            HIP_TRY(ctx, ctx->mbvh_nodes.upload(packed.data(), packed.size()));
        }
        ctx->h_faces.swap(fr);
        ctx->h_mbvh_faces.swap(lfaces);
        HIP_TRY(ctx, ctx->mbvh_face_idx.upload(lidx.data(), lidx.size()));
        HIP_TRY(ctx, ctx->mesh_bvh_root.upload(roots.data(), d->mesh_count));
        std::vector<uint2> jobs;
        bool all_bvh = ctx->have_mesh_bvh && d->model_count > 0;
        for (uint32_t mo = 0; mo < d->model_count && all_bvh; mo++)
            for (uint32_t k = 0; k < d->models[mo].mesh_count && all_bvh; k++) {
                uint32_t mi = d->models[mo].mesh_anchor + k;
                all_bvh = mi < d->mesh_count && roots[mi] != PT_MESH_BVH_NONE;
                jobs.push_back(make_uint2(mi, d->models[mo].mat_ID));
            }
        if (all_bvh && !jobs.empty() && jobs.size() < (1u << 16)) HIP_TRY(ctx, ctx->walk_jobs.upload(jobs.data(), jobs.size()));
    }
    ctx->bvh_node_count = 0;
    if (d->sphere_count > 0 && d->sphere_count < (1u << 24)) {
        bool finite = true;
        for (uint32_t i = 0; i < d->sphere_count && finite; i++)
            finite = std::isfinite(d->spheres[i].pos.x) && std::isfinite(d->spheres[i].pos.y) &&
                     std::isfinite(d->spheres[i].pos.z) && std::isfinite(d->spheres[i].r);
        if (finite) {
            BvhBuild bb;
            bb.sph = d->spheres;
            bb.order.resize(d->sphere_count);
            for (uint32_t i = 0; i < d->sphere_count; i++) bb.order[i] = i;
            bb.build(0, d->sphere_count);
            {
                std::vector<float4> boxes(bb.nodes.size() / 4), links(bb.nodes.size() * 2);
                for (size_t n = 0; n < bb.nodes.size() / 4; n++) {
                    boxes[n] = bb.nodes[4 * n];
                    boxes[n].w = bb.nodes[4 * n + 1].w;
                    uint32_t A, s8[8];
                    memcpy(&A, &bb.nodes[4 * n].w, 4);
                    memcpy(s8, &bb.nodes[4 * n + 2], 32);
                    for (int o = 0; o < 8; o++) {
                        const uint32_t w = s8[o] | (A & 0x30000000u);
                        float4 &l = links[8 * n + o];
                        l = make_float4(0.0f, bb.nodes[4 * n + 1].x, bb.nodes[4 * n + 1].y, bb.nodes[4 * n + 1].z);
                        memcpy(&l.x, &w, 4);
                    }
                }
                HIP_TRY(ctx, ctx->bvh_nodes.upload(boxes.data(), boxes.size()));
                HIP_TRY(ctx, ctx->bvh_links.upload(links.data(), links.size()));
            }
            HIP_TRY(ctx, ctx->bvh_idx.upload(bb.leaf_idx.data(), bb.leaf_idx.size()));
            ctx->h_bvh_idx = bb.leaf_idx;
            ctx->bvh_node_count = (bb.nodes.size() / 4 < (1u << 25) && bb.leaf_sph.size() < (1u << 28)) ? (uint32_t)(bb.nodes.size() / 4) : 0u;
            ctx->bvh_rmax = 0;
            for (int k = 0; k < 3; k++) { ctx->bvh_lo[k] = INFINITY; ctx->bvh_hi[k] = -INFINITY; }
            for (uint32_t i = 0; i < d->sphere_count; i++) {
                const float c[3] = {d->spheres[i].pos.x, d->spheres[i].pos.y, d->spheres[i].pos.z};
                for (int k = 0; k < 3; k++) { ctx->bvh_lo[k] = std::fmin(ctx->bvh_lo[k], c[k]); ctx->bvh_hi[k] = std::fmax(ctx->bvh_hi[k], c[k]); }
                ctx->bvh_rmax = std::fmax(ctx->bvh_rmax, std::fabs(d->spheres[i].r));
            }
        }
    }
    HIP_TRY(ctx, ctx->planes.upload(d->planes, d->plane_count));
    HIP_TRY(ctx, ctx->lenses.upload(d->lenses, d->lens_count));
    HIP_TRY(ctx, ctx->vertices.upload(d->vertices, d->vertex_count));
    if (d->uv_count) HIP_TRY(ctx, ctx->uvs.upload(d->uvs, d->uv_count));
    else {
        std::vector<rt_float2> zeros(d->vertex_count ? d->vertex_count : 1, rt_float2{0.0f, 0.0f});
        HIP_TRY(ctx, ctx->uvs.upload(zeros.data(), d->vertex_count));
    }
    HIP_TRY(ctx, ctx->indices.upload(d->indices, d->index_count));
    HIP_TRY(ctx, ctx->meshes.upload(d->meshes, d->mesh_count));
    HIP_TRY(ctx, ctx->models.upload(d->models, d->model_count));
    ctx->scene_uses_textures = uses_tex;
    ctx->max_texture_id = max_tex;
    {
        int rc = apply_arith(ctx);
        if (rc != RT_OK) return rc;
    }
    ctx->have_scene = true;
    ctx->sample_counter = 0;
    return RT_OK;
}

int rt_set_textures(rt_context *ctx, const float *rgba, int w, int h, int layers) {
    if (!ctx) return RT_EINVAL;
    ctx->prefix_changed();
    HIP_TRY(ctx, hipSetDevice(ctx->device));
    HIP_TRY(ctx, hipStreamSynchronize(ctx->stream));
    if (layers == 0) {
        float4 zero = make_float4(0.0f, 0.0f, 0.0f, 0.0f);
        HIP_TRY(ctx, ctx->tex.upload(&zero, 1));
        ctx->tex_w = ctx->tex_h = 1;
        ctx->tex_layers = 0;
        return RT_OK;
    }
    if (!rgba || w < 1 || h < 1 || layers < 1 || w > 32768 || h > 32768 || layers > 2048)
        return fail(ctx, RT_EINVAL, "bad texture array %dx%dx%d", w, h, layers);
    HIP_TRY(ctx, ctx->tex.upload((const float4 *)rgba, (size_t)w * h * layers));
    ctx->tex_w = w;
    ctx->tex_h = h;
    ctx->tex_layers = layers;
    return RT_OK;
}

int rt_set_random_table(rt_context *ctx, const float *table, size_t n) {
    if (!ctx) return RT_EINVAL;
    if (!table || n != RT_RANDOM_TABLE_FLOATS) return fail(ctx, RT_EINVAL, "table must hold %d floats", RT_RANDOM_TABLE_FLOATS);
    ctx->prefix_changed();
    HIP_TRY(ctx, hipSetDevice(ctx->device));
    HIP_TRY(ctx, hipStreamSynchronize(ctx->stream));
    HIP_TRY(ctx, ctx->table.upload(table, n));
    return RT_OK;
}

int rt_set_seed(rt_context *ctx, uint64_t seed) {
    if (!ctx) return RT_EINVAL;
    std::vector<float> t(RT_RANDOM_TABLE_FLOATS);
    make_table(seed, t.data());
    return rt_set_random_table(ctx, t.data(), t.size());
}

int rt_get_random_table(rt_context *ctx, float *out, size_t n) {
    if (!ctx) return RT_EINVAL;
    if (!out || n != RT_RANDOM_TABLE_FLOATS) return fail(ctx, RT_EINVAL, "table must hold %d floats", RT_RANDOM_TABLE_FLOATS);
    HIP_TRY(ctx, hipSetDevice(ctx->device));
// ... 846 lines not shown
    DeviceScene sc = device_scene(ctx);
    return debug_roundtrip(ctx, in16, 16 * n * sizeof(float), out9, 9 * n * sizeof(float), [&](void *d_in, void *d_out) {
        return ctx->ks->launch_debug_material(ctx, sc, routine, (const float *)d_in, (uint32_t)n, (float *)d_out);
    });
}

int rt_debug_div3(rt_context *ctx, const float *in4, size_t n, float *out6) {
    if (!ctx || !in4 || !out6 || n > (1u << 28)) return RT_EINVAL;
    if (n == 0) return RT_OK;
    HIP_TRY(ctx, hipSetDevice(ctx->device));
    return debug_roundtrip(ctx, in4, 4 * n * sizeof(float), out6, 6 * n * sizeof(float), [&](void *d_in, void *d_out) {
        return ctx->ks->launch_debug_div3(ctx, (const float *)d_in, (uint32_t)n, (float *)d_out);
    });
}

int rt_debug_queue_sums(rt_context *ctx, const float *in3, uint32_t npix, uint32_t count, uint32_t group_log2, float *out4) {
    if (!ctx || !in3 || !out4) return RT_EINVAL;
    if (npix < 1u || npix > 16u || count < 1u || npix * (uint64_t)count > 512u || group_log2 > 6u)
        return fail(ctx, RT_EINVAL, "queue_sums probe: %u pixels of %u samples do not fit one wave's queue", npix, count);
    HIP_TRY(ctx, hipSetDevice(ctx->device));
    return debug_roundtrip(ctx, in3, (size_t)npix * count * 3 * sizeof(float), out4, (size_t)npix * 4 * sizeof(float), [&](void *d_in, void *d_out) {
        return ctx->ks->launch_debug_queue_sums(ctx, (const float *)d_in, npix, count, group_log2, (float *)d_out);
    });
}

int rt_shard_slots(rt_context *ctx, int world, uint32_t *slots_out) {
    if (!ctx || !slots_out || world < 1) return RT_EINVAL;
    uint32_t tw = 1u << ctx->tile_w_log2, th = 1u << ctx->tile_h_log2;
    uint32_t tiles = ((ctx->width + tw - 1) / tw) * ((ctx->height + th - 1) / th);
    *slots_out = ((tiles + world - 1) / world) * tw * th;
    return RT_OK;
}

int rt_pack_accum(rt_context *ctx, void *d_packed, size_t bytes) {
    if (!ctx || !d_packed) return RT_EINVAL;
    uint32_t n = 0;
    rt_shard_slots(ctx, ctx->world, &n);
    if (bytes != (size_t)n * sizeof(float4)) return fail(ctx, RT_EINVAL, "packed buffer must be %zu bytes", (size_t)n * sizeof(float4));
    HIP_TRY(ctx, hipSetDevice(ctx->device));
    float cam0[12] = {0};
    FrameParams fp = frame_params(ctx, cam0, 0, 0, 0);
    hipLaunchKernelGGL(pt_pack, dim3((n + 255) / 256), dim3(256), 0, ctx->stream, fp, ctx->accum.p, (float4 *)d_packed, n);
    HIP_TRY(ctx, hipGetLastError());
    return RT_OK;
}

int rt_unpack_accum(rt_context *ctx, const void *d_packed, size_t bytes, int src_rank, int world) {
    if (!ctx || !d_packed) return RT_EINVAL;
    if (world < 1 || src_rank < 0 || src_rank >= world) return fail(ctx, RT_EINVAL, "rank %d of %d", src_rank, world);
    uint32_t n = 0;
    rt_shard_slots(ctx, world, &n);
    if (bytes != (size_t)n * sizeof(float4)) return fail(ctx, RT_EINVAL, "packed buffer must be %zu bytes", (size_t)n * sizeof(float4));
    HIP_TRY(ctx, hipSetDevice(ctx->device));
    float cam0[12] = {0};
    FrameParams fp = frame_params(ctx, cam0, 0, 0, 0, src_rank, world);
    if (fp.slot_end)
        hipLaunchKernelGGL(pt_unpack, dim3((fp.slot_end + 255) / 256), dim3(256), 0, ctx->stream, fp, (const float4 *)d_packed, ctx->accum.p);
    HIP_TRY(ctx, hipGetLastError());
    return RT_OK;
}

int rt_set_option(rt_context *ctx, int option, int value) {
    if (!ctx) return RT_EINVAL;
    ctx->prefix_changed();
    switch (option) {
        case RT_OPT_PREFIX_CACHE: ctx->prefix_cache.enabled = value != 0; return RT_OK;
        case RT_OPT_PREFIX_SHARING: ctx->prefix_sharing = value != 0; return RT_OK;
        case RT_OPT_SAMPLE_QUEUE: ctx->sample_queue = value != 0; return RT_OK;
        case RT_OPT_WALK_SLICES: ctx->walk_slices = value != 0; return RT_OK;
        case RT_OPT_WAVE_FILL: ctx->wave_fill = value != 0; return RT_OK;
        case RT_OPT_EXACT_GRID: ctx->sample_grid.exact = value != 0; return RT_OK;
        case RT_OPT_MOMENTS:
            if (value != 0 && value != 1) return fail(ctx, RT_EINVAL, "RT_OPT_MOMENTS takes 0 or 1");
            if (value == 1 && ctx->world > 1)
                return fail(ctx, RT_EINVAL, "sample moments on a sharded context (rank %d of %d)", ctx->rank, ctx->world);
            if ((value != 0) != ctx->moments.on) ctx->moments.valid = false;
            ctx->moments.on = value != 0;
            return RT_OK;
        case RT_OPT_LOOKAHEAD:
            if (value < 0 || value == 1 || value > RT_LOOKAHEAD_MAX) return fail(ctx, RT_EINVAL, "RT_OPT_LOOKAHEAD takes 0 or 2..%d", RT_LOOKAHEAD_MAX);
            ctx->lookahead.k = value;
            ctx->lookahead.ring_failed = false;
            return RT_OK;
        case RT_OPT_PREFIX_TREE:
            if (value < 0 || value > 2) return fail(ctx, RT_EINVAL, "RT_OPT_PREFIX_TREE takes 0, 1 or 2");
            ctx->prefix_tree = value;
            return RT_OK;
        case RT_OPT_ACCEL:
            if (value < 0 || value > 2) return fail(ctx, RT_EINVAL, "RT_OPT_ACCEL takes 0, 1 or 2");
            ctx->accel = value;
            return RT_OK;
        case RT_OPT_ARITH: {
            const KernelSet *ks = value == RT_ARITH_IEEE ? kernel_set_a0() : value == RT_ARITH_ROCM_OCL_NOCONTRACT ? kernel_set_a1()
                                  : value == RT_ARITH_ROCM_OCL ? kernel_set_a2() : nullptr;
            if (!ks) return fail(ctx, RT_EINVAL, "RT_OPT_ARITH takes RT_ARITH_IEEE (0), RT_ARITH_ROCM_OCL_NOCONTRACT (1) or RT_ARITH_ROCM_OCL (2)");
            HIP_TRY(ctx, hipSetDevice(ctx->device));
            HIP_TRY(ctx, hipStreamSynchronize(ctx->stream));
            ctx->arith = value;
            ctx->ks = ks;
            ctx->sample_counter = 0;
            return ctx->have_scene ? apply_arith(ctx) : RT_OK;
        }
        case RT_OPT_MAX_THREADS_PER_LAUNCH:
            if (value < 256) return fail(ctx, RT_EINVAL, "max threads per launch must be >= 256");
            ctx->max_threads_per_launch = (uint32_t)value;
            return RT_OK;
        default: return fail(ctx, RT_EINVAL, "unknown option %d", option);
    }
}

int rt_prefix_cache_stats(rt_context *ctx, uint64_t *hits, uint64_t *misses) {
    if (!ctx || !hits || !misses) return RT_EINVAL;
    *hits = ctx->prefix_cache.hits;
    *misses = ctx->prefix_cache.misses;
    return RT_OK;
}

int rt_sample_units(uint32_t seg_cap, uint32_t pixels_per_unit, uint32_t count_light, uint32_t count_heavy, uint32_t *units_out) {
    if (!units_out) return fail(nullptr, RT_EINVAL, "units_out is NULL");
    *units_out = 0;
    if (pixels_per_unit == 0) return fail(nullptr, RT_EINVAL, "pixels_per_unit is 0");
    const uint32_t cnt_l = std::min(count_light, seg_cap);
    const uint32_t cnt_h = std::min(count_heavy, seg_cap - cnt_l);
    const uint32_t units_h = cnt_h / pixels_per_unit + (cnt_h % pixels_per_unit != 0u);
    const uint32_t units_l = cnt_l / pixels_per_unit + (cnt_l % pixels_per_unit != 0u);
    *units_out = units_h + units_l;
    return RT_OK;
}

int rt_sample_grid_stats(rt_context *ctx, uint64_t *launches, uint64_t *exact, uint64_t *workgroups, uint64_t *live_last) {
    if (!ctx || !launches || !exact || !workgroups || !live_last) return RT_EINVAL;
    *launches = ctx->sample_grid.launches;
    *exact = ctx->sample_grid.exact_launches;
    *workgroups = ctx->sample_grid.workgroups;
    *live_last = ctx->sample_grid.live_last;
    return RT_OK;
}

int rt_debug_live_list(rt_context *ctx, uint32_t out[4]) {
    if (!ctx || !out) return RT_EINVAL;
    const rt_context::Slots &ss = ctx->slots;
    if (!ss.live.p || ctx->sample_grid.last_per_unit == 0) return fail(ctx, RT_EINVAL, "no fused launch yet");
    HIP_TRY(ctx, hipSetDevice(ctx->device));
    uint32_t h[LIVE_COUNT_STRIDE];
    HIP_TRY(ctx, hipMemcpyAsync(h, ss.live.p + ss.capacity + 256u, sizeof h, hipMemcpyDeviceToHost, ctx->stream));
    HIP_TRY(ctx, hipStreamSynchronize(ctx->stream));
    out[0] = ctx->sample_grid.last_cap;
    out[1] = ctx->sample_grid.last_per_unit;
    out[2] = h[0];
    out[3] = h[LIVE_HEAVY_COUNTER];
    return RT_OK;
}

int rt_reset_counters(rt_context *ctx) {
    if (!ctx) return RT_EINVAL;
    HIP_TRY(ctx, hipSetDevice(ctx->device));
    HIP_TRY(ctx, hipMemsetAsync(ctx->counters.p, 0, COUNTER_REPLICAS * COUNTER_STRIDE * sizeof(unsigned long long), ctx->stream));
    HIP_TRY(ctx, hipMemsetAsync(ctx->d_walk_overflow, 0, sizeof(uint32_t), ctx->stream));
    return RT_OK;
}

int rt_get_counters(rt_context *ctx, rt_counters *out) {
    if (!ctx || !out) return RT_EINVAL;
    HIP_TRY(ctx, hipSetDevice(ctx->device));
    std::vector<unsigned long long> h(COUNTER_REPLICAS * COUNTER_STRIDE);
    HIP_TRY(ctx, hipMemcpyAsync(h.data(), ctx->counters.p, h.size() * sizeof(unsigned long long), hipMemcpyDeviceToHost, ctx->stream));
    HIP_TRY(ctx, hipStreamSynchronize(ctx->stream));
    uint64_t *o = (uint64_t *)out;
    for (int i = 0; i < 14; i++) {
        o[i] = 0;
        for (int r = 0; r < COUNTER_REPLICAS; r++) o[i] += h[(size_t)r * COUNTER_STRIDE + i];
    }
    return RT_OK;
}

int rt_get_debug_counters(rt_context *ctx, uint64_t out[2]) {
    if (!ctx || !out) return RT_EINVAL;
    HIP_TRY(ctx, hipSetDevice(ctx->device));
    std::vector<unsigned long long> h(COUNTER_REPLICAS * COUNTER_STRIDE);
    HIP_TRY(ctx, hipMemcpyAsync(h.data(), ctx->counters.p, h.size() * sizeof(unsigned long long), hipMemcpyDeviceToHost, ctx->stream));
    HIP_TRY(ctx, hipStreamSynchronize(ctx->stream));
    out[0] = out[1] = 0;
    for (int r = 0; r < COUNTER_REPLICAS; r++) {
        out[0] += h[(size_t)r * COUNTER_STRIDE + 14];
        out[1] += h[(size_t)r * COUNTER_STRIDE + 15];
    }
#ifdef PT_WSTAT
    {
        unsigned long long v[12];
        if (hipMemcpy(v, ctx->counters.p + COUNTER_REPLICAS * COUNTER_STRIDE + 8, sizeof v, hipMemcpyDeviceToHost) == hipSuccess) {
            const char *names[12] = {"outer iterations", "active lanes", "phase-0 lanes", "phase-1 lanes", "phase-2 lanes", "walk slices",
                                     "walk steps", "node-test lanes", "(unused)", "leaf phases", "leaf lanes", "finished (idle) lanes"};
            for (int k = 0; k < 12; k++) fprintf(stderr, "[wstat] %-24s %llu\n", names[k], v[k]);
            (void)hipMemset(ctx->counters.p + COUNTER_REPLICAS * COUNTER_STRIDE + 8, 0, sizeof v);
        }
    }
#endif
#if PT_STAMPS
    {
        unsigned long long st[8];
        if (hipMemcpy(st, ctx->counters.p + COUNTER_REPLICAS * COUNTER_STRIDE, sizeof st, hipMemcpyDeviceToHost) == hipSuccess) {
            const char *names[6] = {"refill", "scatter", "hit:spheres", "hit:planes/lenses/models", "hit:rebuild+material", "loop"};
            double tot = 0;
            for (int k = 0; k < 6; k++) tot += (double)st[k];
            for (int k = 0; k < 6; k++) fprintf(stderr, "[stamps] %-26s %5.1f %%\n", names[k], tot > 0 ? 100.0 * st[k] / tot : 0.0);
        }
    }
#endif
    return RT_OK;
}

int rt_walk_overflow(rt_context *ctx, uint32_t *flags_out) {
    if (!ctx || !flags_out) return RT_EINVAL;
    HIP_TRY(ctx, hipSetDevice(ctx->device));
    HIP_TRY(ctx, hipMemcpyAsync(flags_out, ctx->d_walk_overflow, sizeof(uint32_t), hipMemcpyDeviceToHost, ctx->stream));
    HIP_TRY(ctx, hipStreamSynchronize(ctx->stream));
    return RT_OK;
}

int rt_debug_builtin(rt_context *ctx, int op, const float *in8, size_t n, float *out4) {
    if (!ctx || !in8 || !out4 || op < 0 || op > 11 || n > (1u << 26)) return RT_EINVAL;
    if (n == 0) return RT_OK;
    HIP_TRY(ctx, hipSetDevice(ctx->device));
    return debug_roundtrip(ctx, in8, 8 * n * sizeof(float), out4, 4 * n * sizeof(float), [&](void *d_in, void *d_out) {
        return ctx->ks->launch_debug_builtin(ctx, op, (const float *)d_in, (uint32_t)n, (float *)d_out);
    });
}

uint64_t rt_counters_bytes(const rt_counters *c) {
    if (!c) return 0;
    return 32 * c->t_sphere + 48 * c->t_plane + 64 * c->t_lens + 12 * c->t_model + 16 * c->t_mesh + 60 * c->t_tri +
           36 * c->h_tri + 48 * c->h_bounce + 12 * c->n_scatter + 4 * c->n_dielectric + 64 * c->n_texfetch +
           (48 + 16) * c->samples + 16 * c->image_reads;
}

int rt_kernel_ms_history(rt_context *ctx, float *ms, size_t cap, size_t *n_out) {
    if (!ctx || !ms || !n_out) return RT_EINVAL;
    HIP_TRY(ctx, hipSetDevice(ctx->device));
    size_t have = ctx->ev_count < (uint64_t)rt_context::EV_RING ? (size_t)ctx->ev_count : (size_t)rt_context::EV_RING;
    size_t n = have < cap ? have : cap;
    for (size_t i = 0; i < n; i++) {
        hipEvent_t *evp = ctx->ev[(ctx->ev_count - n + i) % rt_context::EV_RING];
        HIP_TRY(ctx, hipEventSynchronize(evp[1]));
        HIP_TRY(ctx, hipEventElapsedTime(&ms[i], evp[0], evp[1]));
    }
    *n_out = n;
    return RT_OK;
}

int rt_stage_ms_history(rt_context *ctx, float *first_ms, float *second_ms, size_t cap, size_t *n_out) {
    if (!ctx || !first_ms || !second_ms || !n_out) return RT_EINVAL;
    HIP_TRY(ctx, hipSetDevice(ctx->device));
    size_t have = ctx->ev_count < (uint64_t)rt_context::EV_RING ? (size_t)ctx->ev_count : (size_t)rt_context::EV_RING;
    size_t n = have < cap ? have : cap;
    for (size_t i = 0; i < n; i++) {
        hipEvent_t *evp = ctx->ev[(ctx->ev_count - n + i) % rt_context::EV_RING];
        HIP_TRY(ctx, hipEventSynchronize(evp[1]));
        HIP_TRY(ctx, hipEventElapsedTime(&first_ms[i], evp[0], evp[2]));
        HIP_TRY(ctx, hipEventElapsedTime(&second_ms[i], evp[2], evp[1]));
    }
    *n_out = n;
    return RT_OK;
}

int rt_last_kernel_ms(rt_context *ctx, float *ms) {
    if (!ctx || !ms) return RT_EINVAL;
    if (ctx->ev_count == 0) return fail(ctx, RT_ESTATE, "no render call has been timed yet");
    size_t n = 0;
    return rt_kernel_ms_history(ctx, ms, 1, &n);
}

int rt_device_info(rt_context *ctx, char *name, size_t name_len, int *cu_count, char *arch, size_t arch_len) {
    if (!ctx) return RT_EINVAL;
    if (name && name_len) snprintf(name, name_len, "%s", ctx->dev_name.c_str());
    if (arch && arch_len) snprintf(arch, arch_len, "%s", ctx->dev_arch.c_str());
    if (cu_count) *cu_count = ctx->cu_count;
    return RT_OK;
}

}
```

### opencl-raytracing_amd/csrc/rt_context.hpp

```cpp
#pragma once
#include <hip/hip_runtime.h>

#include <cstdarg>
#include <cstdint>
#include <cstring>
#include <string>
#include <utility>
#include <vector>

#include "pt_types.hpp"

template <class T>
struct DevBuf {
    T *p = nullptr;
    size_t n = 0;
    DevBuf() = default;
    DevBuf(const DevBuf &) = delete;
    DevBuf &operator=(const DevBuf &) = delete;
    DevBuf(DevBuf &&o) noexcept : p(o.p), n(o.n) { o.p = nullptr; o.n = 0; }
    DevBuf &operator=(DevBuf &&o) noexcept {
        std::swap(p, o.p);
        std::swap(n, o.n);
        return *this;
    }
    ~DevBuf() { release(); }
    hipError_t alloc(size_t count) {
        release();
        hipError_t e = hipMalloc((void **)&p, count * sizeof(T));
        if (e != hipSuccess) { p = nullptr; return e; }
        n = count;
        return e;
    }
    hipError_t upload(const T *src, size_t count) {
        release();
        size_t alloc = count ? count : 1;
        hipError_t e = hipMalloc((void **)&p, alloc * sizeof(T));
        if (e != hipSuccess) { p = nullptr; return e; }
        n = count;
        if (count) e = hipMemcpy(p, src, count * sizeof(T), hipMemcpyHostToDevice);
        else e = hipMemset(p, 0, sizeof(T));
        return e;
    }
    void release() {
        if (p) (void)hipFree(p);
        p = nullptr;
        n = 0;
    }
};

namespace pt { struct KernelSet; }

#define ACCEL_MIN_SPHERES 64
#define RT_SPP_PER_LAUNCH 512u
#define RT_LOOKAHEAD_MAX 64
#define RT_LOOKAHEAD_MAX_BYTES (1ull << 30)
#ifndef MESH_BVH_MIN_FACES
#define MESH_BVH_MIN_FACES 32
#endif

struct rt_context {
    int device = 0;
    int width = 0, height = 0;
    hipStream_t own_stream = nullptr;
    hipStream_t stream = nullptr;
    static constexpr int EV_RING = 64;
    hipEvent_t ev[EV_RING][3] = {};
    uint64_t ev_count = 0;
    std::string error;
    std::string dev_name, dev_arch;
    int cu_count = 0;

    DevBuf<rt_material> materials;
    DevBuf<rt_sphere> spheres;
    DevBuf<float4> sph4;
    uint32_t sphere_batches = 0;
    DevBuf<float4> faces;
    DevBuf<uint32_t> mesh_face_base;
    DevBuf<float4> mbvh_nodes, mbvh_faces;
    DevBuf<uint32_t> mbvh_face_idx, mesh_bvh_root;
    bool have_mesh_bvh = false;
    DevBuf<float4> bvh_nodes, bvh_sph;
    DevBuf<uint32_t> bvh_idx;
    DevBuf<float4> bvh_links;
    uint32_t bvh_node_count = 0;
    float bvh_lo[3] = {0, 0, 0}, bvh_hi[3] = {0, 0, 0}, bvh_rmax = 0;
    int accel = 1;
    int arith = 0;
    const pt::KernelSet *ks = nullptr;
    std::vector<rt_sphere> h_spheres;
    std::vector<uint32_t> h_bvh_idx;
    std::vector<float4> h_faces, h_mbvh_faces;
    DevBuf<rt_plane> planes;
    DevBuf<rt_lens> lenses;
    DevBuf<rt_float3> vertices;
    DevBuf<rt_float2> uvs;
    DevBuf<uint32_t> indices;
    DevBuf<rt_mesh> meshes;
    DevBuf<rt_model> models;
    DevBuf<float> table;
    DevBuf<float4> tex;
    int tex_w = 1, tex_h = 1, tex_layers = 0;
    bool have_scene = false;
    bool scene_uses_textures = false;
    uint32_t max_texture_id = 0;

    DevBuf<float4> image, accum;
    DevBuf<unsigned long long> counters;
    uint32_t *d_walk_overflow = nullptr;
    struct Slots {
        DevBuf<pt::PixelRec> recs;
        DevBuf<uint32_t> live;
        size_t capacity = 0;
        DevBuf<pt::PixelTree> trees;
        DevBuf<pt::PixelRec> tree_wait;
        size_t tree_capacity = 0;
        DevBuf<pt::FinalPix> finals;
        DevBuf<uint32_t> final_n;
    } slots;
    struct PrefixCache {
        bool enabled = true;
        bool valid = false;
        uint64_t generation = 0;
        uint64_t key_generation = 0;
        uint32_t key_cam[12] = {};
        bool key_tree_on = false;
        uint64_t hits = 0, misses = 0;
        enum { COUNTS_UNKNOWN, COUNTS_IN_FLIGHT, COUNTS_KNOWN } counts_state = COUNTS_UNKNOWN;
        uint32_t count_light = 0, count_heavy = 0;
    } prefix_cache;
    void prefix_changed() { prefix_cache.generation++; }
    struct SampleGrid {
        bool exact = true;
        uint32_t *h_counts = nullptr;
        hipEvent_t counts_ev = nullptr;
        uint64_t launches = 0;
        uint64_t exact_launches = 0;
        uint64_t workgroups = 0;
        uint64_t live_last = 0;
        uint32_t last_cap = 0, last_per_unit = 0;
    } sample_grid;
    struct Lookahead {
        int k = 16;
        DevBuf<float4> ring;
        size_t ring_frames = 0;
        bool ring_failed = false;
        uint32_t pending = 0;
        uint32_t batch_frames = 0;
        uint32_t next_frame = 0;
        uint32_t next_sample = 0;
        uint64_t key_generation = 0, key_epoch = 0;
        uint32_t key_cam[12] = {};
        bool have_last_cam = false;
        uint32_t last_cam[12] = {};
        uint64_t batches = 0, served = 0, direct = 0, discarded = 0;
    } lookahead;
    uint64_t image_epoch = 0;
    bool wave_fill = true;
    int prefix_tree = 1;
    bool prefix_sharing = true;
    bool sample_queue = true;
    DevBuf<uint2> walk_jobs;
    bool walk_slices = true;
    uint32_t accum_count = 0;
    uint32_t sample_counter = 0;
    bool count_enabled = false;

    struct Adaptive {
        DevBuf<float4> scratch;
        DevBuf<float4> half;
        DevBuf<uint32_t> block_active;
        DevBuf<float> block_err;
        DevBuf<unsigned long long> stats;
        DevBuf<float> m2_scratch;
        size_t block_capacity = 0;
        uint32_t blocks = 0;
    } adaptive;
    struct Features {
        DevBuf<rt_feature> records;
        bool ready = false;
    } features;
    struct Denoise {
        DevBuf<float4> pingpong[2];
        DevBuf<float4> out;
        bool ready = false;
        DevBuf<float> var[2];
        bool var_ready = false;
    } denoise;

    struct Moments {
        bool on = false;
        bool valid = false;
        DevBuf<float> m2;
        float *target() const { return on && valid ? m2.p : nullptr; }
    } moments;

    int rank = 0, world = 1, tile_w_log2 = 3, tile_h_log2 = 3;
    uint32_t max_threads_per_launch = 1u << 30;
};

namespace rtamd {
using namespace pt;

int fail(rt_context *ctx, int code, const char *fmt, ...);
int read_back(rt_context *ctx, void *dst, size_t bytes, const void *src, size_t need, const char *what, bool ready = true,
              const char *producer = nullptr);

#define HIP_TRY(ctx, expr)                                                                        \
    do {                                                                                          \
        hipError_t e_ = (expr);                                                                   \
        if (e_ != hipSuccess) return fail(ctx, RT_EHIP, "%s: %s", #expr, hipGetErrorString(e_)); \
    } while (0)

inline DeviceScene device_scene(const rt_context *ctx) {
    DeviceScene s;
    s.materials = ctx->materials.p;
    s.spheres = ctx->spheres.p;
    s.sph4 = ctx->sph4.p;
    s.sphere_batches = ctx->sphere_batches;
    s.material_count = (uint32_t)ctx->materials.n;
    s.faces = ctx->faces.p;
    s.mesh_face_base = ctx->mesh_face_base.p;
    s.mbvh_nodes = ctx->mbvh_nodes.p;
    s.mbvh_faces = ctx->mbvh_faces.p;
    s.mbvh_face_idx = ctx->mbvh_face_idx.p;
    s.mesh_bvh_root = (ctx->have_mesh_bvh && ctx->accel != 0) ? ctx->mesh_bvh_root.p : nullptr;
    bool use_bvh = ctx->bvh_node_count && (ctx->accel == 2 || (ctx->accel == 1 && ctx->spheres.n >= ACCEL_MIN_SPHERES));
    s.bvh_nodes = ctx->bvh_nodes.p;
    s.bvh_sph = ctx->bvh_sph.p;
    s.bvh_idx = ctx->bvh_idx.p;
    s.bvh_links = ctx->bvh_links.p;
    s.bvh_node_count = use_bvh ? ctx->bvh_node_count : 0;
    for (int k = 0; k < 3; k++) { s.bvh_lo[k] = ctx->bvh_lo[k]; s.bvh_hi[k] = ctx->bvh_hi[k]; }
    s.bvh_rmax = ctx->bvh_rmax;
    s.walk_overflow = ctx->d_walk_overflow;
    s.planes = ctx->planes.p;
    s.lenses = ctx->lenses.p;
    s.vertices = ctx->vertices.p;
    s.uvs = ctx->uvs.p;
    s.indices = ctx->indices.p;
    s.meshes = ctx->meshes.p;
    s.models = ctx->models.p;
    s.table = ctx->table.p;
    s.tex = ctx->tex.p;
    s.tex_w = ctx->tex_w;
    s.tex_h = ctx->tex_h;
    s.tex_layers = ctx->tex_layers;
    s.tex_wf = (float)ctx->tex_w;
    s.tex_hf = (float)ctx->tex_h;
    s.sphere_count = (uint32_t)ctx->spheres.n;
    s.plane_count = (uint32_t)ctx->planes.n;
    s.lens_count = (uint32_t)ctx->lenses.n;
    s.model_count = (uint32_t)ctx->models.n;
    return s;
}

struct Shard {
    uint32_t tiles_x, tiles_total, owned_tiles, slots;
};
inline Shard shard_of(const rt_context *ctx, int rank, int world) {
    Shard s;
    uint32_t tw = 1u << ctx->tile_w_log2, th = 1u << ctx->tile_h_log2;
    s.tiles_x = (ctx->width + tw - 1) / tw;
    uint32_t tiles_y = (ctx->height + th - 1) / th;
    s.tiles_total = s.tiles_x * tiles_y;
    s.owned_tiles = s.tiles_total > (uint32_t)rank ? (s.tiles_total - rank + world - 1) / world : 0;
    s.slots = s.owned_tiles * tw * th;
    return s;
}

inline FrameParams frame_params(const rt_context *ctx, const float cam[12], uint32_t first, uint32_t count, uint32_t glog2,
                         int rank = -1, int world = 1) {
    if (rank < 0) { rank = ctx->rank; world = ctx->world; }
    FrameParams fp;
    memcpy(fp.cam, cam, sizeof fp.cam);
    Shard sh = shard_of(ctx, rank, world);
    fp.w = ctx->width;
    fp.h = ctx->height;
    fp.tile_w_log2 = ctx->tile_w_log2;
    fp.tile_h_log2 = ctx->tile_h_log2;
    fp.tiles_x = sh.tiles_x;
    fp.tiles_total = sh.tiles_total;
    fp.rank = (uint32_t)rank;
    fp.world = (uint32_t)world;
    fp.slot_begin = 0;
    fp.slot_end = sh.slots;
    fp.first = first;
    fp.count = count;
    fp.group_log2 = glog2;
    fp.seg_cap = 0;
    fp.trees = nullptr;
    fp.tree_wait = nullptr;
    fp.tree_count = nullptr;
// ... 48 lines not shown
```

### opencl-raytracing_amd/raytracer.py

```python
import ctypes as C
import os

import numpy as np

from . import _abi
from .scene import SceneCreator

_HERE = os.path.dirname(os.path.abspath(__file__))
LIB_PATH = os.path.join(_HERE, "librt_amd.so")

SYMBOLS = (
    "rt_abi_version", "rt_last_error", "rt_create", "rt_destroy", "rt_resize", "rt_set_stream", "rt_set_scene",
    "rt_set_textures", "rt_set_seed", "rt_set_random_table", "rt_get_random_table", "rt_make_random_table",
    "rt_set_shard", "rt_render", "rt_render_again", "rt_sample_counter", "rt_clear", "rt_render_spp", "rt_resolve",
    "rt_sync", "rt_trace_samples", "rt_read_image", "rt_read_linear", "rt_device_image", "rt_device_accum",
    "rt_enable_counters", "rt_reset_counters", "rt_get_counters", "rt_counters_bytes", "rt_last_kernel_ms",
    "rt_kernel_ms_history", "rt_stage_ms_history", "rt_debug_hit", "rt_debug_material", "rt_debug_div3", "rt_device_info", "rt_set_option", "rt_shard_slots", "rt_pack_accum", "rt_unpack_accum",
    "rt_get_debug_counters", "rt_debug_check_accel", "rt_walk_overflow", "rt_debug_builtin",
    "rt_render_adaptive", "rt_read_sample_counts", "rt_read_block_error",
    "rt_render_features", "rt_read_features", "rt_device_features", "rt_render_features_chain", "rt_feature_chain_signature",
    "rt_denoise", "rt_read_denoised", "rt_device_denoised",
    "rt_denoise_variance", "rt_read_variance", "rt_device_variance",
    "rt_read_moments", "rt_device_moments", "rt_moments_merge", "rt_denoise_moments",
    "rt_prefix_cache_stats", "rt_lookahead_stats", "rt_lookahead_plan",
    "rt_sample_units", "rt_sample_grid_stats", "rt_debug_live_list", "rt_debug_queue_sums",
)

OPT_PREFIX_SHARING, OPT_MAX_THREADS_PER_LAUNCH, OPT_SAMPLE_QUEUE, OPT_ACCEL, OPT_WALK_SLICES, OPT_ARITH, OPT_PREFIX_TREE, OPT_WAVE_FILL = 1, 2, 3, 4, 5, 6, 7, 8
OPT_PREFIX_CACHE = 9
OPT_LOOKAHEAD = 10
OPT_EXACT_GRID = 11
OPT_MOMENTS = 12
ARITH_IEEE, ARITH_ROCM_OCL_NOCONTRACT, ARITH_ROCM_OCL = 0, 1, 2
FOLLOW_REFLECTIVE, FOLLOW_REFRACTIVE, FOLLOW_DIELECTRIC = _abi.FOLLOW_REFLECTIVE, _abi.FOLLOW_REFRACTIVE, _abi.FOLLOW_DIELECTRIC
FOLLOW_ALL = FOLLOW_REFLECTIVE | FOLLOW_REFRACTIVE | FOLLOW_DIELECTRIC
ARITH_NAMES = {"ieee": ARITH_IEEE, "rocm-opencl-nocontract": ARITH_ROCM_OCL_NOCONTRACT, "rocm-opencl": ARITH_ROCM_OCL}


class RtError(RuntimeError):
    def __init__(self, code, msg):
        super().__init__("librt_amd: %s (code %d)" % (msg, code))
        self.code = code


_lib = None


def load_library(path=LIB_PATH):
    global _lib
    if _lib is not None:
        return _lib
    if not os.path.isfile(path):
        raise OSError("%s not found — the HIP library is not built (run __graft_entry__.build()); "
                      "there is no CPU fallback" % path)
    try:
        import torch
    except ImportError:
        pass
    lib = C.CDLL(path)
    for s in SYMBOLS:
        getattr(lib, s)
    vp, u32, u64, sz, fp = C.c_void_p, C.c_uint32, C.c_uint64, C.c_size_t, C.POINTER(C.c_float)
    lib.rt_last_error.restype = C.c_char_p
    lib.rt_last_error.argtypes = [vp]
    lib.rt_create.argtypes = [C.c_int, C.c_int, C.c_int, C.POINTER(vp)]
    lib.rt_destroy.argtypes = [vp]
    lib.rt_destroy.restype = None
    lib.rt_resize.argtypes = [vp, C.c_int, C.c_int]
    lib.rt_set_stream.argtypes = [vp, vp]
    lib.rt_set_scene.argtypes = [vp, C.POINTER(_abi.SceneDesc)]
    lib.rt_set_textures.argtypes = [vp, vp, C.c_int, C.c_int, C.c_int]
    lib.rt_set_seed.argtypes = [vp, u64]
    lib.rt_set_random_table.argtypes = [vp, vp, sz]
    lib.rt_get_random_table.argtypes = [vp, vp, sz]
    lib.rt_make_random_table.argtypes = [u64, vp, sz]
    lib.rt_set_shard.argtypes = [vp, C.c_int, C.c_int, C.c_int, C.c_int]
    lib.rt_render.argtypes = [vp, vp]
    lib.rt_render_again.argtypes = [vp, vp]
    lib.rt_sample_counter.argtypes = [vp, C.POINTER(u32)]
    lib.rt_clear.argtypes = [vp]
    lib.rt_render_spp.argtypes = [vp, vp, u32, u32]
    lib.rt_resolve.argtypes = [vp]
    lib.rt_sync.argtypes = [vp]
    lib.rt_trace_samples.argtypes = [vp, vp, vp, vp, vp, sz, vp]
    lib.rt_read_image.argtypes = [vp, vp, sz]
    lib.rt_read_linear.argtypes = [vp, vp, sz]
    lib.rt_device_image.argtypes = [vp, C.POINTER(vp)]
    lib.rt_device_accum.argtypes = [vp, C.POINTER(vp)]
    lib.rt_enable_counters.argtypes = [vp, C.c_int]
    lib.rt_reset_counters.argtypes = [vp]
    lib.rt_get_counters.argtypes = [vp, C.POINTER(_abi.Counters)]
    lib.rt_counters_bytes.argtypes = [C.POINTER(_abi.Counters)]
    lib.rt_counters_bytes.restype = u64
    lib.rt_last_kernel_ms.argtypes = [vp, fp]
    lib.rt_kernel_ms_history.argtypes = [vp, fp, sz, C.POINTER(sz)]
    lib.rt_stage_ms_history.argtypes = [vp, fp, fp, sz, C.POINTER(sz)]
    lib.rt_debug_hit.argtypes = [vp, C.c_int, vp, vp, vp, sz, vp]
    lib.rt_debug_material.argtypes = [vp, C.c_int, vp, sz, vp]
    lib.rt_debug_div3.argtypes = [vp, vp, sz, vp]
    lib.rt_set_option.argtypes = [vp, C.c_int, C.c_int]
    lib.rt_shard_slots.argtypes = [vp, C.c_int, C.POINTER(u32)]
    lib.rt_pack_accum.argtypes = [vp, vp, sz]
    lib.rt_unpack_accum.argtypes = [vp, vp, sz, C.c_int, C.c_int]
    lib.rt_device_info.argtypes = [vp, C.c_char_p, sz, C.POINTER(C.c_int), C.c_char_p, sz]
    lib.rt_walk_overflow.argtypes = [vp, C.POINTER(u32)]
    lib.rt_debug_builtin.argtypes = [vp, C.c_int, vp, sz, vp]
    _abi.adaptive_prototypes(lib)
    _abi.denoise_prototypes(lib)
    _abi.moments_prototypes(lib)
    _abi.prefix_cache_prototypes(lib)
    _abi.lookahead_prototypes(lib)
    _abi.sample_grid_prototypes(lib)
    _abi.queue_sums_prototypes(lib)
    if lib.rt_abi_version() != _abi.RT_ABI_VERSION:
        raise OSError("librt_amd.so ABI %d != expected %d" % (lib.rt_abi_version(), _abi.RT_ABI_VERSION))
    _lib = lib
    return lib


def check_accel(scene):
    lib = load_library()
    d = scene.desc()
    stats = (C.c_uint64 * 8)()
    err = C.create_string_buffer(256)
    rc = lib.rt_debug_check_accel(C.byref(d), stats, err, 256)
    if rc:
        raise RtError(rc, err.value.decode() or "accel check failed")
    keys = ("sphere_nodes", "sphere_leaves", "sphere_depth", "mesh_nodes", "mesh_leaves", "mesh_depth", "meshes")
    return dict(zip(keys, [int(v) for v in stats]))


def make_random_table(seed):
    lib = load_library()
    out = np.empty(_abi.RANDOM_TABLE_FLOATS, dtype=np.float32)
    rc = lib.rt_make_random_table(seed, out.ctypes.data, out.size)
    if rc:
        raise RtError(rc, lib.rt_last_error(None).decode())
    return out


def lookahead_plan(width, height, option=16, sample_counter=0):
    lib = load_library()
    out = C.c_uint32()
    rc = lib.rt_lookahead_plan(int(width), int(height), int(option), int(sample_counter), C.byref(out))
    if rc:
        raise RtError(rc, lib.rt_last_error(None).decode())
    return int(out.value)


def sample_units(seg_cap, pixels_per_unit, count_light, count_heavy):
    lib = load_library()
    out = C.c_uint32()
    rc = lib.rt_sample_units(int(seg_cap), int(pixels_per_unit), int(count_light), int(count_heavy), C.byref(out))
    if rc:
        raise RtError(rc, lib.rt_last_error(None).decode())
    return int(out.value)


def moments_merge(nA, sumA, m2A, nB, sumB, m2B):
    lib = load_library()
    a = (C.c_float * 3)(*[float(v) for v in sumA])
    b = (C.c_float * 3)(*[float(v) for v in sumB])
    out = C.c_float()
    rc = lib.rt_moments_merge(int(nA), a, float(m2A), int(nB), b, float(m2B), C.byref(out))
    if rc:
        raise RtError(rc, lib.rt_last_error(None).decode())
    return np.float32(out.value)


def feature_chain_signature(objects):
    lib = load_library()
    o = np.ascontiguousarray(objects, dtype=np.uint32).reshape(-1)
    out = C.c_uint32()
    rc = lib.rt_feature_chain_signature(o.ctypes.data if len(o) else None, len(o), C.byref(out))
    if rc:
        raise RtError(rc, lib.rt_last_error(None).decode())
    return int(out.value)


def _cam_block(camera):
    block = camera.transferData() if hasattr(camera, "transferData") else camera
    block = np.ascontiguousarray(block, dtype=np.float32)
    if block.shape != (12,):
        raise ValueError("camera block must be 12 floats")
    return block


class DeviceBuffer:

    def __init__(self, ptr, h, w, owner):
        self._owner = owner
        self.__cuda_array_interface__ = {"shape": (h, w, 4), "typestr": "<f4", "data": (int(ptr), False),
                                         "version": 3, "strides": None}


class RayTracer:
    DEFAULT_SCENE = os.path.join("assets", "scenes", "scene.scene")
    REPO_DEFAULT_SCENE = os.path.join(os.path.dirname(_HERE), "assets", "scenes", "scene.scene")

    def __init__(self, w, h, kernel_path=None, scene=None, device=0, seed=0xC0FFEE):
        self._lib = load_library()
        self._ctx = C.c_void_p()
        rc = self._lib.rt_create(device, w, h, C.byref(self._ctx))
        if rc:
            self._ctx = C.c_void_p()
            raise RtError(rc, self._lib.rt_last_error(None).decode())
        self.width, self.height = w, h
        if seed != 0xC0FFEE:
            self.setSeed(seed)
        if scene is None:
            scene = self.DEFAULT_SCENE if os.path.isfile(self.DEFAULT_SCENE) else self.REPO_DEFAULT_SCENE
        if isinstance(scene, str):
            path = scene
            scene = SceneCreator()
            scene.loadScene(path)
            scene.loadTextures()
        self.setScene(scene)

    def _check(self, rc):
        if rc:
            raise RtError(rc, self._lib.rt_last_error(self._ctx).decode())

    def close(self):
        if getattr(self, "_ctx", None) and self._ctx.value:
            self._lib.rt_destroy(self._ctx)
            self._ctx = C.c_void_p()

    def __del__(self):
        try:
            self.close()
        except Exception:
            pass

    def setScene(self, scene):
        self.scene = scene
        d = scene.desc()
        self._check(self._lib.rt_set_scene(self._ctx, C.byref(d)))
        tex, tw, th, layers = scene.texture_args()
        self._check(self._lib.rt_set_textures(self._ctx, tex, tw, th, layers))

    def setSeed(self, seed):
        self._check(self._lib.rt_set_seed(self._ctx, seed))

    def setRandomTable(self, table):
        table = np.ascontiguousarray(table, dtype=np.float32)
        self._check(self._lib.rt_set_random_table(self._ctx, table.ctypes.data, table.size))

    def getRandomTable(self):
        out = np.empty(_abi.RANDOM_TABLE_FLOATS, dtype=np.float32)
        self._check(self._lib.rt_get_random_table(self._ctx, out.ctypes.data, out.size))
        return out

    def setShard(self, rank, world, tile_w=8, tile_h=8):
        self._check(self._lib.rt_set_shard(self._ctx, rank, world, tile_w, tile_h))

    OPT_PREFIX_SHARING, OPT_MAX_THREADS_PER_LAUNCH, OPT_SAMPLE_QUEUE, OPT_ACCEL, OPT_WALK_SLICES, OPT_ARITH, OPT_PREFIX_TREE, OPT_WAVE_FILL = 1, 2, 3, 4, 5, 6, 7, 8
    OPT_PREFIX_CACHE = 9
    OPT_LOOKAHEAD = 10
    OPT_EXACT_GRID = 11
    OPT_MOMENTS = 12

    def setOption(self, option, value):
        self._check(self._lib.rt_set_option(self._ctx, option, int(value)))

    def shardSlots(self, world):
        n = C.c_uint32()
        self._check(self._lib.rt_shard_slots(self._ctx, world, C.byref(n)))
        return n.value

    def packAccum(self, device_ptr, nbytes):
        self._check(self._lib.rt_pack_accum(self._ctx, C.c_void_p(device_ptr), nbytes))

    def unpackAccum(self, device_ptr, nbytes, src_rank, world):
        self._check(self._lib.rt_unpack_accum(self._ctx, C.c_void_p(device_ptr), nbytes, src_rank, world))

    def setStream(self, hip_stream):
        self._check(self._lib.rt_set_stream(self._ctx, C.c_void_p(hip_stream or 0)))

    def resize(self, w, h):
        self._check(self._lib.rt_resize(self._ctx, w, h))
        self.width, self.height = w, h

    def setTime(self, time):
        """Declared, never defined in the reference (include/raytracer.h:45); a stub."""

    def render(self, camera):
        self._check(self._lib.rt_render(self._ctx, _cam_block(camera).ctypes.data))

    def renderAgain(self, camera):
        self._check(self._lib.rt_render_again(self._ctx, _cam_block(camera).ctypes.data))

    @property
    def sample_counter(self):
        v = C.c_uint32()
        self._check(self._lib.rt_sample_counter(self._ctx, C.byref(v)))
        return v.value

    def clear(self):
        self._check(self._lib.rt_clear(self._ctx))

    def renderSamples(self, camera, first_sample, n_samples):
        self._check(self._lib.rt_render_spp(self._ctx, _cam_block(camera).ctypes.data, first_sample, n_samples))

    def resolve(self):
        self._check(self._lib.rt_resolve(self._ctx))

    def sync(self):
        self._check(self._lib.rt_sync(self._ctx))

    def renderFrame(self, camera, spp):
        self.clear()
        self.renderSamples(camera, 0, spp)
        self.resolve()
        return self.transferImage()

    def renderFrameOnDevice(self, camera, spp):
        self.clear()
        self.renderSamples(camera, 0, spp)
        self.resolve()

    def renderAdaptive(self, camera, threshold, batch=64, min_spp=128, max_spp=1024, block=(8, 8)):
        p = _abi.AdaptiveParams(int(batch), int(min_spp), int(max_spp), float(threshold), int(block[0]), int(block[1]))
        st = _abi.AdaptiveStats()
        self._check(self._lib.rt_render_adaptive(self._ctx, _cam_block(camera).ctypes.data, C.byref(p), C.byref(st)))
        self._adaptive_block = (int(block[0]), int(block[1]))
        return st.as_dict()

    def sampleCounts(self):
        out = np.empty((self.height, self.width), dtype=np.uint32)
        self._check(self._lib.rt_read_sample_counts(self._ctx, out.ctypes.data, out.nbytes))
        return out

    def blockError(self):
        bw, bh = getattr(self, "_adaptive_block", (8, 8))
        out = np.empty((-(-self.height // bh), -(-self.width // bw)), dtype=np.float32)
        self._check(self._lib.rt_read_block_error(self._ctx, out.ctypes.data, out.nbytes))
        return out

    def renderFeatures(self, camera):
        self._check(self._lib.rt_render_features(self._ctx, _cam_block(camera).ctypes.data))

    def renderFeaturesChain(self, camera, follow=FOLLOW_ALL, max_chain=_abi.FEATURE_CHAIN_MAX):
        p = _abi.FeatureChainParams(int(follow), int(max_chain))
        self._check(self._lib.rt_render_features_chain(self._ctx, _cam_block(camera).ctypes.data, C.byref(p)))

    def featureRecords(self):
        out = np.empty((self.height, self.width), dtype=_abi.FEATURE)
        self._check(self._lib.rt_read_features(self._ctx, out.ctypes.data, out.nbytes))
# ... 27 lines not shown

    def denoiseVariance(self, camera=None, iterations=_abi.DENOISE_VARIANCE_DEFAULTS["iterations"],
                        sigma_luminance=_abi.DENOISE_VARIANCE_DEFAULTS["sigma_luminance"],
                        sigma_normal=_abi.DENOISE_VARIANCE_DEFAULTS["sigma_normal"],
                        sigma_position=_abi.DENOISE_VARIANCE_DEFAULTS["sigma_position"],
                        sigma_albedo=_abi.DENOISE_VARIANCE_DEFAULTS["sigma_albedo"], split_objects=True, split_chains=False):
        if camera is not None:
            self.renderFeatures(camera)
        self.denoiseVarianceOnDevice(iterations, sigma_luminance, sigma_normal, sigma_position, sigma_albedo,
                                     split_objects, split_chains)
        return self.denoisedImage()

    def denoiseVarianceOnDevice(self, iterations=_abi.DENOISE_VARIANCE_DEFAULTS["iterations"],
                                sigma_luminance=_abi.DENOISE_VARIANCE_DEFAULTS["sigma_luminance"],
                                sigma_normal=_abi.DENOISE_VARIANCE_DEFAULTS["sigma_normal"],
                                sigma_position=_abi.DENOISE_VARIANCE_DEFAULTS["sigma_position"],
                                sigma_albedo=_abi.DENOISE_VARIANCE_DEFAULTS["sigma_albedo"], split_objects=True, split_chains=False):
        p = _abi.DenoiseVarianceParams(int(iterations), float(sigma_luminance), float(sigma_normal),
                                       float(sigma_position), float(sigma_albedo),
                                       _abi.denoise_flags(split_objects, split_chains))
        self._check(self._lib.rt_denoise_variance(self._ctx, C.byref(p)))

    def variance(self, which=0):
        out = np.empty((self.height, self.width), dtype=np.float32)
        self._check(self._lib.rt_read_variance(self._ctx, int(which), out.ctypes.data, out.nbytes))
        return out

    def deviceVariance(self, which=0):
        p = C.c_void_p()
        self._check(self._lib.rt_device_variance(self._ctx, int(which), C.byref(p)))
        return p.value

    def moments(self):
        out = np.empty((self.height, self.width), dtype=np.float32)
        self._check(self._lib.rt_read_moments(self._ctx, out.ctypes.data, out.nbytes))
        return out

    def deviceMoments(self):
        p = C.c_void_p()
        self._check(self._lib.rt_device_moments(self._ctx, C.byref(p)))
        return p.value

    def sampleVariance(self):
        m2 = self.moments().astype(np.float64)
        n = self.sampleCounts().astype(np.float64)
        ok = n >= 2
        return np.where(ok, m2 / np.where(ok, n * (n - 1.0), 1.0), 0.0).astype(np.float32)

    def denoiseMoments(self, camera=None, iterations=_abi.DENOISE_VARIANCE_DEFAULTS["iterations"],
                       sigma_luminance=_abi.DENOISE_VARIANCE_DEFAULTS["sigma_luminance"],
                       sigma_normal=_abi.DENOISE_VARIANCE_DEFAULTS["sigma_normal"],
                       sigma_position=_abi.DENOISE_VARIANCE_DEFAULTS["sigma_position"],
                       sigma_albedo=_abi.DENOISE_VARIANCE_DEFAULTS["sigma_albedo"], split_objects=True, split_chains=False):
        if camera is not None:
            self.renderFeatures(camera)
        self.denoiseMomentsOnDevice(iterations, sigma_luminance, sigma_normal, sigma_position, sigma_albedo,
                                    split_objects, split_chains)
        return self.denoisedImage()

    def denoiseMomentsOnDevice(self, iterations=_abi.DENOISE_VARIANCE_DEFAULTS["iterations"],
                               sigma_luminance=_abi.DENOISE_VARIANCE_DEFAULTS["sigma_luminance"],
                               sigma_normal=_abi.DENOISE_VARIANCE_DEFAULTS["sigma_normal"],
                               sigma_position=_abi.DENOISE_VARIANCE_DEFAULTS["sigma_position"],
                               sigma_albedo=_abi.DENOISE_VARIANCE_DEFAULTS["sigma_albedo"], split_objects=True, split_chains=False):
        p = _abi.DenoiseVarianceParams(int(iterations), float(sigma_luminance), float(sigma_normal),
                                       float(sigma_position), float(sigma_albedo),
                                       _abi.denoise_flags(split_objects, split_chains))
        self._check(self._lib.rt_denoise_moments(self._ctx, C.byref(p)))

    def deviceFeatures(self):
        p = C.c_void_p()
        self._check(self._lib.rt_device_features(self._ctx, C.byref(p)))
        return p.value

    def deviceDenoised(self):
        p = C.c_void_p()
        self._check(self._lib.rt_device_denoised(self._ctx, C.byref(p)))
        return DeviceBuffer(p.value, self.height, self.width, self)

    def traceSamples(self, camera, xs, ys, samples):
        xs = np.ascontiguousarray(xs, dtype=np.uint32)
        ys = np.ascontiguousarray(ys, dtype=np.uint32)
        ss = np.ascontiguousarray(samples, dtype=np.uint32)
        out = np.zeros((len(xs), 3), dtype=np.float32)
        self._check(self._lib.rt_trace_samples(self._ctx, _cam_block(camera).ctypes.data, xs.ctypes.data,
                                               ys.ctypes.data, ss.ctypes.data, len(xs), out.ctypes.data))
        return out

    def transferImage(self, screen=None, shader_tex_id=None):
        out = np.empty((self.height, self.width, 4), dtype=np.float32)
        self._check(self._lib.rt_read_image(self._ctx, out.ctypes.data, out.nbytes))
        return out

    def readLinear(self):
        out = np.empty((self.height, self.width, 4), dtype=np.float32)
        self._check(self._lib.rt_read_linear(self._ctx, out.ctypes.data, out.nbytes))
        return out

    def deviceImage(self):
        p = C.c_void_p()
        self._check(self._lib.rt_device_image(self._ctx, C.byref(p)))
        return DeviceBuffer(p.value, self.height, self.width, self)

    def deviceAccum(self):
        p = C.c_void_p()
        self._check(self._lib.rt_device_accum(self._ctx, C.byref(p)))
        return DeviceBuffer(p.value, self.height, self.width, self)

    def enableCounters(self, on=True):
        self._check(self._lib.rt_enable_counters(self._ctx, 1 if on else 0))

    def resetCounters(self):
        self._check(self._lib.rt_reset_counters(self._ctx))

    def counters(self):
        c = _abi.Counters()
        self._check(self._lib.rt_get_counters(self._ctx, C.byref(c)))
        return c

    def debugCounters(self):
        out = (C.c_uint64 * 2)()
        self._check(self._lib.rt_get_debug_counters(self._ctx, out))
        return int(out[0]), int(out[1])

    def walkOverflow(self):
        out = C.c_uint32()
        self._check(self._lib.rt_walk_overflow(self._ctx, C.byref(out)))
        return int(out.value)

    def prefixCacheStats(self):
        hits, misses = C.c_uint64(), C.c_uint64()
        self._check(self._lib.rt_prefix_cache_stats(self._ctx, C.byref(hits), C.byref(misses)))
        return int(hits.value), int(misses.value)

    def lookaheadStats(self):
        v = [C.c_uint64() for _ in range(4)]
        self._check(self._lib.rt_lookahead_stats(self._ctx, *[C.byref(x) for x in v]))
        return tuple(int(x.value) for x in v)

    lookaheadPlan = staticmethod(lookahead_plan)

    def sampleGridStats(self):
        v = [C.c_uint64() for _ in range(4)]
        self._check(self._lib.rt_sample_grid_stats(self._ctx, *[C.byref(x) for x in v]))
        return tuple(int(x.value) for x in v)

    sampleUnits = staticmethod(sample_units)

    def liveList(self):
        out = (C.c_uint32 * 4)()
        self._check(self._lib.rt_debug_live_list(self._ctx, out))
        return tuple(int(v) for v in out)

    def setArith(self, arith):
        if isinstance(arith, str):
            arith = ARITH_NAMES[arith]
        self.setOption(OPT_ARITH, int(arith))
        self.arith = int(arith)

    def lastKernelMs(self):
        ms = C.c_float()
        self._check(self._lib.rt_last_kernel_ms(self._ctx, C.byref(ms)))
        return ms.value

    def kernelMsHistory(self, n=64):
        buf = (C.c_float * n)()
        got = C.c_size_t()
        self._check(self._lib.rt_kernel_ms_history(self._ctx, buf, n, C.byref(got)))
        return [buf[i] for i in range(got.value)]

    def stageMsHistory(self, n=64):
        a, b = (C.c_float * n)(), (C.c_float * n)()
        got = C.c_size_t()
        self._check(self._lib.rt_stage_ms_history(self._ctx, a, b, n, C.byref(got)))
        return [a[i] for i in range(got.value)], [b[i] for i in range(got.value)]

    def debugHit(self, kind, rays, prim=None, face=None):
        rays = np.ascontiguousarray(rays, dtype=np.float32).reshape(-1, 6)
        n = len(rays)
        prim = np.zeros(n, np.uint32) if prim is None else np.ascontiguousarray(prim, dtype=np.uint32)
        face = np.zeros(n, np.uint32) if face is None else np.ascontiguousarray(face, dtype=np.uint32)
        out = np.zeros((n, 12), dtype=np.float32)
        self._check(self._lib.rt_debug_hit(self._ctx, kind, rays.ctypes.data, prim.ctypes.data, face.ctypes.data, n,
                                           out.ctypes.data))
        return out

    def debugMaterial(self, routine, vec):
        vec = np.ascontiguousarray(vec, dtype=np.float32).reshape(-1, 16)
        out = np.zeros((len(vec), 9), dtype=np.float32)
        self._check(self._lib.rt_debug_material(self._ctx, routine, vec.ctypes.data, len(vec), out.ctypes.data))
        return out

    def debugBuiltin(self, op, vec):
        vec = np.ascontiguousarray(vec, dtype=np.float32).reshape(-1, 8)
        out = np.zeros((len(vec), 4), dtype=np.float32)
        self._check(self._lib.rt_debug_builtin(self._ctx, op, vec.ctypes.data, len(vec), out.ctypes.data))
        return out

    def debugDiv3(self, vec):
        vec = np.ascontiguousarray(vec, dtype=np.float32).reshape(-1, 4)
        out = np.zeros((len(vec), 6), dtype=np.float32)
        self._check(self._lib.rt_debug_div3(self._ctx, vec.ctypes.data, len(vec), out.ctypes.data))
        return out

    def debugQueueSums(self, slots, group_log2):
        slots = np.ascontiguousarray(slots, dtype=np.float32)
        npix, count = slots.shape[0], slots.shape[1]
        out = np.zeros((npix, 4), dtype=np.float32)
        self._check(self._lib.rt_debug_queue_sums(self._ctx, slots.ctypes.data, npix, count, group_log2, out.ctypes.data))
        return out

    def deviceInfo(self):
        name, arch, cu = C.create_string_buffer(128), C.create_string_buffer(64), C.c_int()
        self._check(self._lib.rt_device_info(self._ctx, name, 128, C.byref(cu), arch, 64))
        return {"name": name.value.decode(), "arch": arch.value.decode(), "cu_count": cu.value}
```

Measured before the change: 119,200.

## Specialize queue kernel for 64 spp and pre-stage LDS scene tables

Adds a compile-time specialization of the sample-queue kernel for count=64 and group_log2=6, so the per-entry index divides, modulo and the reduction tree use shifts and a fixed two-pass sum. Scene tables are built once into a packed device block after the materials, and each workgroup copies it straight into LDS instead of rebuilding it per block. Also adds a float-reciprocal pixel-coordinate path and an asm barrier that delays texture UV use. In exchange it adds template instantiations, extra allocation tail bytes and a one-time build kernel.

```diff
diff --git a/include/rt_amd.h b/include/rt_amd.h
--- a/include/rt_amd.h
+++ b/include/rt_amd.h
@@ -316,6 +316,14 @@
 
 int rt_debug_live_list(rt_context *ctx, uint32_t out[4]);
 
+int rt_debug_queue_pixels(uint32_t count, uint32_t waves_per_simd, uint32_t static_float4, uint32_t granule, uint32_t *pixels_out);
+
+int rt_debug_queue_occupancy(rt_context *ctx, uint32_t lds_bytes, int *blocks_out);
+
+int rt_debug_wave_fixed(rt_context *ctx, uint64_t out[2]);
+
+int rt_debug_stage_block(rt_context *ctx, float *out, size_t capacity_float4, uint32_t *float4_out);
+
 int rt_device_info(rt_context *ctx, char *name, size_t name_len, int *cu_count, char *arch, size_t arch_len);
 
 #ifdef __cplusplus
diff --git a/opencl-raytracing_amd/_abi.py b/opencl-raytracing_amd/_abi.py
--- a/opencl-raytracing_amd/_abi.py
+++ b/opencl-raytracing_amd/_abi.py
@@ -180,6 +180,20 @@
     lib.rt_sample_units.argtypes = [u32, u32, u32, u32, C.POINTER(u32)]
     lib.rt_sample_grid_stats.argtypes = [C.c_void_p, p64, p64, p64, p64]
     lib.rt_debug_live_list.argtypes = [C.c_void_p, C.POINTER(u32)]
+    lib.rt_debug_wave_fixed.argtypes = [C.c_void_p, C.POINTER(C.c_uint64)]
+    lib.rt_debug_stage_block.argtypes = [C.c_void_p, C.c_void_p, C.c_size_t, C.POINTER(u32)]
+    lib.rt_debug_queue_pixels.argtypes = [u32, u32, u32, u32, C.POINTER(u32)]
+    lib.rt_debug_queue_occupancy.argtypes = [C.c_void_p, u32, C.POINTER(C.c_int)]
+
+
+LDS_MATERIALS, LDS_WINNERS, LDS_PLANES = 64, 64, 16
+
+
+def stage_block_layout(n_materials, n_spheres, n_planes):
+    nm = 2 * n_materials if n_materials <= LDS_MATERIALS else 0
+    nw = 2 * n_spheres if n_spheres <= LDS_WINNERS else 0
+    npl = n_planes if n_planes <= LDS_PLANES else 0
+    return 0, nm, nm + nw, nm + nw + npl
 
 
 def queue_sums_prototypes(lib):
diff --git a/opencl-raytracing_amd/csrc/pt_device.hpp b/opencl-raytracing_amd/csrc/pt_device.hpp
--- a/opencl-raytracing_amd/csrc/pt_device.hpp
+++ b/opencl-raytracing_amd/csrc/pt_device.hpp
@@ -58,8 +58,7 @@
     return r0;
 }
 
-PT_DEV LdsV4 stage_materials(const DeviceScene &sc, float4 *lds) {
-    const uint32_t nm = lds_mat_n(sc.material_count), nw = lds_win_n(sc.sphere_count), np = lds_pln_n(sc.plane_count);
+PT_DEV void stage_tables(const DeviceScene &sc, float4 *lds, const uint32_t nm, const uint32_t nw, const uint32_t np) {
     if (nm)
         for (uint32_t i = threadIdx.x; i < sc.material_count; i += blockDim.x) {
             const rt_material &m = sc.materials[i];
@@ -78,8 +77,22 @@
             const rt_plane &p = sc.planes[i];
             lds[nm + nw + i] = make_float4(p.normal.x, p.normal.y, p.normal.z, __uint_as_float(p.mat_ID));
         }
+}
+PT_DEV LdsV4 stage_materials(const DeviceScene &sc, float4 *lds) {
+    const uint32_t nm = lds_mat_n(sc.material_count), nw = lds_win_n(sc.sphere_count), np = lds_pln_n(sc.plane_count);
+    stage_tables(sc, lds, nm, nw, np);
     __syncthreads();
     return nm ? lds_ptr(lds) : (LdsV4) nullptr;
+}
+PT_DEV const float4 *stage_block_of(const DeviceScene &sc) {
+    return reinterpret_cast<const float4 *>(reinterpret_cast<const char *>(sc.materials) + stage_block_offset(sc.material_count));
+}
+PT_DEV LdsV4 stage_materials_copy(const DeviceScene &sc, float4 *lds) {
+    const uint32_t n = lds_static_used(sc.material_count, sc.sphere_count, sc.plane_count);
+    const float4 *__restrict__ blk = stage_block_of(sc);
+    for (uint32_t i = threadIdx.x; i < n; i += blockDim.x) lds[i] = blk[i];
+    __syncthreads();
+    return lds_mat_n(sc.material_count) ? lds_ptr(lds) : (LdsV4) nullptr;
 }
 PT_DEV LdsV4 staged_winners(const DeviceScene &sc, const float4 *lds) {
     return lds_win_n(sc.sphere_count) ? lds_ptr(lds + lds_mat_n(sc.material_count)) : (LdsV4) nullptr;
diff --git a/opencl-raytracing_amd/csrc/pt_kernels.hip b/opencl-raytracing_amd/csrc/pt_kernels.hip
--- a/opencl-raytracing_amd/csrc/pt_kernels.hip
+++ b/opencl-raytracing_amd/csrc/pt_kernels.hip
@@ -390,10 +390,10 @@
 #ifndef PT_LDS_GRANULE
 #define PT_LDS_GRANULE 1024u
 #endif
-__host__ inline uint32_t queue_pixels_per_wave(uint32_t count, uint32_t waves, uint32_t static_float4) {
+__host__ inline uint32_t queue_pixels_per_wave(uint32_t count, uint32_t waves, uint32_t static_float4, uint32_t granule = PT_LDS_GRANULE) {
     auto fit = [&](uint32_t waves_per_simd) {
         uint32_t workgroups = waves_per_simd * 4u;
-        uint32_t budget = 163840u / workgroups / PT_LDS_GRANULE * PT_LDS_GRANULE;
+        uint32_t budget = 163840u / workgroups / granule * granule;
         uint32_t per_wave = budget - static_float4 * (uint32_t)sizeof(float4) - 15u;
         uint32_t p = per_wave / queue_pixel_bytes(count);
         if (p * count > QUEUE_SLOTS) p = QUEUE_SLOTS / count;
@@ -433,6 +433,34 @@
     float inv_count;
 };
 
+#ifndef PT_Q_COUNT64
+#define PT_Q_COUNT64 1
+#endif
+#ifndef PT_TEXEL_LAZY
+#define PT_TEXEL_LAZY 1
+#endif
+#ifndef PT_STAGE_XY_FAST
+#define PT_STAGE_XY_FAST 1
+#endif
+#ifndef PT_STAGE_COPY
+#define PT_STAGE_COPY 1
+#endif
+
+#define PT_XY_FAST_MAX_TILES (1u << 20)
+template <bool FAST>
+PT_DEV void stage_xy(const FrameParams &fp, uint32_t slot, uint32_t &x, uint32_t &y) {
+    if (FAST && PT_STAGE_XY_FAST && fp.world == 1u && fp.tiles_total <= PT_XY_FAST_MAX_TILES) {
+        const uint32_t tpix_log2 = fp.tile_w_log2 + fp.tile_h_log2;
+        const uint32_t t = slot >> tpix_log2, in = slot & ((1u << tpix_log2) - 1u);
+        const uint32_t ty = (uint32_t)(((float)t + 0.5f) * __builtin_amdgcn_rcpf((float)fp.tiles_x)), tx = t - ty * fp.tiles_x;
+        x = (tx << fp.tile_w_log2) + (in & ((1u << fp.tile_w_log2) - 1u));
+        y = (ty << fp.tile_h_log2) + (in >> fp.tile_w_log2);
+    } else {
+        (void)slot_to_pixel(fp, slot, x, y);
+    }
+}
+
+template <int CL = -1, bool XY_FAST = false>
 PT_DEV WaveQueue queue_stage(const DeviceScene &sc, const FrameParams &fp, const PixelRec *__restrict__ recs,
                              const uint32_t *__restrict__ live, uint32_t npix, uint32_t pix0,
                              uint32_t pixels_per_wave, float4 *lds, uint32_t face_f4) {
@@ -443,7 +471,7 @@
     q.slot = (LdsF32)(wave_lds + queue_slot_f4(pixels_per_wave));
     const uint32_t lane = threadIdx.x;
     q.npix = npix;
-    q.count = fp.count;
+    q.count = CL >= 0 ? 1u << (CL & 31) : fp.count;
     q.total = q.npix * q.count;
     for (uint32_t i = lane; i < q.npix * QUEUE_REC_F4; i += 64u) {
         uint32_t p = i / QUEUE_REC_F4, part = i - p * QUEUE_REC_F4;
@@ -452,7 +480,7 @@
     }
     if (lane < q.npix) {
         uint32_t x = 0, y = 0;
-        (void)slot_to_pixel(fp, live[pix0 + lane], x, y);
+        stage_xy<XY_FAST>(fp, live[pix0 + lane], x, y);
         q.xy[lane].x = x;
         q.xy[lane].y = y;
         q.xy[lane].bv = rnd_base_v(0u, x, y);
@@ -461,7 +489,7 @@
     __builtin_amdgcn_fence(__ATOMIC_SEQ_CST, "wavefront");
     __builtin_amdgcn_wave_barrier();
     q.inv_count = fp.inv_count;
-    q.count_log2 = (q.count & (q.count - 1u)) == 0u ? (uint32_t)__builtin_ctz(q.count) : 0xFFu;
+    q.count_log2 = CL >= 0 ? (uint32_t)CL : (q.count & (q.count - 1u)) == 0u ? (uint32_t)__builtin_ctz(q.count) : 0xFFu;
     return q;
 }
 
@@ -469,9 +497,10 @@
     float4 q0, q1, q2, q3, q4;
     uint32_t bits, bv, bu;
 };
+template <int CL = -1>
 PT_DEV QueueEntry queue_fetch(const WaveQueue &q, const DeviceScene &sc, const FrameParams &fp, uint32_t idx) {
-    const uint32_t p = q.count_log2 != 0xFFu ? idx >> q.count_log2 : (uint32_t)(((float)idx + 0.5f) * q.inv_count);
-    const uint32_t sample = fp.first + (idx - p * q.count);
+    const uint32_t p = CL >= 0 ? idx >> (CL & 31) : q.count_log2 != 0xFFu ? idx >> q.count_log2 : (uint32_t)(((float)idx + 0.5f) * q.inv_count);
+    const uint32_t sample = fp.first + (CL >= 0 ? idx & ((1u << (CL & 31)) - 1u) : idx - p * q.count);
     auto part = [&](uint32_t k) {
         const LdsQueueF4 f = q.rec + (QUEUE_REC_F4 * p + k);
         return make_float4(f->x, f->y, f->z, f->w);
@@ -521,7 +550,32 @@
     const auto r = __builtin_amdgcn_permlane16_swap(__float_as_uint(a), __float_as_uint(b), false, false);
     return __uint_as_float(r[0]) + __uint_as_float(r[1]);
 }
+PT_DEV V3 queue_lane_slot64(const WaveQueue &q, uint32_t p, uint32_t l) {
+    V3 sum = mk(0.0f, 0.0f, 0.0f);
+    if (p < q.npix) {
+        const LdsF32 sl = q.slot + 3u * (p * 64u + l);
+        sum = sum + mk(sl[0], sl[1], sl[2]);
+    }
+    return sum;
+}
+template <int CL = -1>
 PT_DEV void queue_sums_tree(const WaveQueue &q, const FrameParams &fp, float4 *__restrict__ accum) {
+    if (CL == 6) {
+        static_assert(QUEUE_SLOTS / 64u <= 8u, "two passes of four pixels");
+        const uint32_t lane = threadIdx.x, half = lane >> 5, i = lane & 31u, row = lane >> 4;
+#pragma unroll
+        for (uint32_t pb = 0; pb < 8u; pb += 4u) {
+            if (pb >= q.npix) break;
+            V3 a = queue_lane_slot64(q, pb + half, i), b = queue_lane_slot64(q, pb + 2u + half, i);
+            a = a + queue_lane_slot64(q, pb + half, i + 32u);
+            b = b + queue_lane_slot64(q, pb + 2u + half, i + 32u);
+            V3 sum = mk(row_pair_add(a.x, b.x), row_pair_add(a.y, b.y), row_pair_add(a.z, b.z));
+            sum = row_add<1>(row_add<2>(row_add<4>(row_add<8>(sum))));
+            const uint32_t p = pb + ((row & 1u) << 1 | row >> 1);
+            if (p < q.npix && (lane & 15u) == 0u) accumulate(accum, (size_t)q.xy[p].y * fp.w + q.xy[p].x, sum, 64u);
+        }
+        return;
+    }
     const uint32_t lane = threadIdx.x, gl = fp.group_log2;
     if (gl >= 5u) {
         const uint32_t half = lane >> 5, i = lane & 31u, g = 1u << gl, row = lane >> 4;
@@ -549,11 +603,11 @@
         }
     }
 }
-template <bool MOMENTS, bool BUTTERFLY = false>
+template <bool MOMENTS, bool BUTTERFLY = false, int CL = -1>
 PT_DEV void queue_sums(const WaveQueue &q, const FrameParams &fp, float4 *__restrict__ accum) {
     __builtin_amdgcn_fence(__ATOMIC_SEQ_CST, "wavefront");
     __builtin_amdgcn_wave_barrier();
-    if (PT_QUEUE_SUMS_TREE && !MOMENTS && !BUTTERFLY) return queue_sums_tree(q, fp, accum);
+    if (PT_QUEUE_SUMS_TREE && !MOMENTS && !BUTTERFLY) return queue_sums_tree<CL>(q, fp, accum);
     const uint32_t lane = threadIdx.x;
     const uint32_t g = 1u << fp.group_log2, ppp = 64u >> fp.group_log2;
     for (uint32_t pb = 0; pb < q.npix; pb += ppp) {
@@ -601,7 +655,7 @@
     }
 }
 
-template <bool COUNT, bool ACCEL, int GEOM, int WAVES, bool MOMENTS = false>
+template <bool COUNT, bool ACCEL, int GEOM, int WAVES, bool MOMENTS = false, int COUNT_LOG2 = -1>
 __global__ __launch_bounds__(64, WAVES) void pt_samples_q(DeviceScene sc, FrameParams fp, const PixelRec *__restrict__ recs,
                                                     const uint32_t *__restrict__ live,
                                                     const uint32_t *__restrict__ live_count,
@@ -615,7 +669,7 @@
     float4 *s_mat = s_dyn;
     LaneCounters cn;
     if (COUNT) zero_counters(cn);
-    Ctx c{sc, stage_materials(sc, s_mat), &cn};
+    Ctx c{sc, PT_STAGE_COPY && !COUNT && !ACCEL ? stage_materials_copy(sc, s_mat) : stage_materials(sc, s_mat), &cn};
     c.lwin = staged_winners(sc, s_mat);
     c.lpln = staged_planes(sc, s_mat);
     if (GEOM != 0 && fp.lds_face_f4) {
@@ -625,7 +679,7 @@
         c.lfaces = lds_ptr(s_faces);
     }
 
-    const WaveQueue q = queue_stage(sc, fp, recs, live, npix, pix0, pixels_per_wave, s_dyn, GEOM != 0 ? fp.lds_face_f4 : 0u);
+    const WaveQueue q = queue_stage<COUNT_LOG2, !COUNT && !ACCEL>(sc, fp, recs, live, npix, pix0, pixels_per_wave, s_dyn, GEOM != 0 ? fp.lds_face_f4 : 0u);
 
     uint32_t next = 0;
     bool active = false;
@@ -650,7 +704,7 @@
             uint32_t cand = next + lanes_below(m);
             if (need && cand < q.total) {
                 idx = cand;
-                const QueueEntry e = queue_fetch(q, sc, fp, idx);
+                const QueueEntry e = queue_fetch<COUNT_LOG2>(q, sc, fp, idx);
                 bv = e.bv;
                 bu = e.bu;
                 if (COUNT) cn.c[CN_SAMPLES]++;
@@ -732,7 +786,9 @@
                     done = true;
                 } else if (type == RT_TEXTURED) {
                     if (COUNT) cn.c[CN_N_TEXFETCH]++;
-                    col = texture_rgb(c.sc, h.u, h.v, h.tex);
+                    float tu = h.u, tv = h.v;
+                    if (PT_TEXEL_LAZY && GEOM == 0 && !COUNT && !ACCEL) asm("" : "+v"(tu), "+v"(tv));
+                    col = texture_rgb(c.sc, tu, tv, h.tex);
                 }
             }
             if (done) {
@@ -749,8 +805,12 @@
         for (int k = 0; k < 6; k++) atomicAdd(&counters[(size_t)COUNTER_REPLICAS * COUNTER_STRIDE + k], c.st[k]);
 #endif
     if (!COUNT && !MOMENTS && fp.la_ring) queue_replay(q, fp);
-    else queue_sums<MOMENTS, COUNT || ACCEL>(q, fp, accum);
+    else queue_sums<MOMENTS, COUNT || ACCEL, COUNT_LOG2>(q, fp, accum);
     flush_counters<COUNT>(cn, counters, 1);
+}
+
+__global__ __launch_bounds__(64) void pt_stage_block(DeviceScene sc, float4 *__restrict__ block) {
+    stage_tables(sc, block, lds_mat_n(sc.material_count), lds_win_n(sc.sphere_count), lds_pln_n(sc.plane_count));
 }
 
 #ifndef PT_WALK_STEPS
@@ -1318,6 +1378,13 @@
     int rc = ensure_slots(ctx, slots);
     if (rc) return rc;
     const rt_context::Slots &ss = ctx->slots;
+    if (PT_STAGE_COPY && ctx->stage_block.generation != ctx->prefix_cache.generation) {
+        if (lds_static_used(sc.material_count, sc.sphere_count, sc.plane_count))
+            hipLaunchKernelGGL(pt_stage_block, dim3(1), dim3(64), 0, ctx->stream, sc,
+                               reinterpret_cast<float4 *>(reinterpret_cast<char *>(ctx->materials.p) + stage_block_offset(sc.material_count)));
+        ctx->stage_block.generation = ctx->prefix_cache.generation;
+        ctx->stage_block.builds++;
+    }
     uint32_t *live_count = ss.live.p + ss.capacity + 256u;
     uint32_t slots_per_launch = ctx->max_threads_per_launch >> glog2;
     if (slots_per_launch == 0) slots_per_launch = 1;
@@ -1404,10 +1471,19 @@
 #define PT_GRID(U, LAUNCH) do { launched = (U); if (launched) { LAUNCH; } } while (0)
 #define PT_CALL_QUEUE_M(C, A, G, W, M) \
     PT_GRID(units(ppw), hipLaunchKernelGGL((pt_samples_q<C, A, G, W, M>), dim3(launched), dim3(64), queue_lds(ppw), ctx->stream, sc, fp, ss.recs.p, ss.live.p, live_count, accum, ctx->counters.p, ppw))
+    const bool count64 = PT_Q_COUNT64 && count == 64u && fp.group_log2 == 6u;
+    (void)count64;
+#define PT_CALL_QUEUE_64(G, W) \
+    do { PT_GRID(units(ppw), hipLaunchKernelGGL((pt_samples_q<false, false, G, W, false, 6>), dim3(launched), dim3(64), queue_lds(ppw), ctx->stream, sc, fp, ss.recs.p, ss.live.p, live_count, accum, ctx->counters.p, ppw)); if (launched) sg.count64_launches++; } while (0)
 #define PT_CALL_QUEUE_W(C, A, G, W) do { if (fp.m2) PT_CALL_QUEUE_M(C, A, G, W, true); else PT_CALL_QUEUE_M(C, A, G, W, false); } while (0)
+#if PT_Q_COUNT64
+#define PT_CALL_QUEUE_N(C, G) do { if (!(C) && count64 && !fp.m2) PT_CALL_QUEUE_64(G, PT_Q_WAVES); else PT_CALL_QUEUE_W(C, false, G, PT_Q_WAVES); } while (0)
+#else
+#define PT_CALL_QUEUE_N(C, G) PT_CALL_QUEUE_W(C, false, G, PT_Q_WAVES)
+#endif
 #define PT_CALL_QUEUE(C, A)                                                                       \
     do {                                                                                          \
-        if (!(A)) { if (simple_geom) PT_CALL_QUEUE_W(C, false, 0, PT_Q_WAVES); else PT_CALL_QUEUE_W(C, false, 1, PT_Q_WAVES); } \
+        if (!(A)) { if (simple_geom) PT_CALL_QUEUE_N(C, 0); else PT_CALL_QUEUE_N(C, 1); } \
         else if (sphere_bvh_only) { if (simple_geom) PT_CALL_QUEUE_W(C, true, 0, PT_Q_WAVES_SPHERE_BVH); else PT_CALL_QUEUE_W(C, true, 1, PT_Q_WAVES_ACCEL); } \
         else PT_CALL_QUEUE_W(C, true, 2, PT_Q_WAVES_ACCEL);                                       \
     } while (0)
@@ -1432,6 +1508,8 @@
         }
 #undef PT_CALL_QUEUE
 #undef PT_CALL_QUEUE_W
+#undef PT_CALL_QUEUE_N
+#undef PT_CALL_QUEUE_64
 #undef PT_CALL_QUEUE_M
 #undef PT_CALL_FIXED
 #undef PT_GRID
@@ -1581,6 +1659,15 @@
     return RT_OK;
 }
 
+uint32_t ks_queue_pixels(uint32_t count, uint32_t waves, uint32_t static_float4, uint32_t granule) {
+    return queue_pixels_per_wave(count, waves, static_float4, granule ? granule : PT_LDS_GRANULE);
+}
+
+int ks_queue_occupancy(rt_context *ctx, uint32_t lds_bytes, int *blocks) {
+    HIP_TRY(ctx, hipOccupancyMaxActiveBlocksPerMultiprocessor(blocks, pt_samples_q<false, false, 0, PT_Q_WAVES, false, -1>, 64, lds_bytes));
+    return RT_OK;
+}
+
 const pt::KernelSet g_kernel_set = {
     PT_ARITH,
 #if PT_ARITH == 0
@@ -1591,7 +1678,8 @@
     "rocm-opencl",
 #endif
     ks_launch_render, launch_fused, launch_lookahead, ks_launch_probe, ks_launch_features, ks_launch_debug_hit, ks_launch_debug_material, ks_launch_debug_div3,
-    ks_launch_face_normals, ks_launch_debug_builtin, ks_launch_debug_queue_sums, ks_launch_features_chain};
+    ks_launch_face_normals, ks_launch_debug_builtin, ks_launch_debug_queue_sums, ks_launch_features_chain,
+    ks_queue_pixels, ks_queue_occupancy};
 
 }
 
diff --git a/opencl-raytracing_amd/csrc/pt_kernels.hpp b/opencl-raytracing_amd/csrc/pt_kernels.hpp
--- a/opencl-raytracing_amd/csrc/pt_kernels.hpp
+++ b/opencl-raytracing_amd/csrc/pt_kernels.hpp
@@ -22,6 +22,8 @@
     int (*launch_debug_queue_sums)(rt_context *ctx, const float *d_in, uint32_t npix, uint32_t count, uint32_t glog2, float *d_out);
     int (*launch_features_chain)(rt_context *ctx, const FrameParams &fp, const DeviceScene &sc, uint32_t follow, uint32_t max_chain,
                                  rt_feature *d_out);
+    uint32_t (*queue_pixels)(uint32_t count, uint32_t waves, uint32_t static_float4, uint32_t granule);
+    int (*queue_occupancy)(rt_context *ctx, uint32_t lds_bytes, int *blocks);
 };
 
 const KernelSet *kernel_set_a0();
diff --git a/opencl-raytracing_amd/csrc/pt_types.hpp b/opencl-raytracing_amd/csrc/pt_types.hpp
--- a/opencl-raytracing_amd/csrc/pt_types.hpp
+++ b/opencl-raytracing_amd/csrc/pt_types.hpp
@@ -65,6 +65,9 @@
 PT_HD uint32_t lds_static_used(uint32_t material_count, uint32_t sphere_count, uint32_t plane_count) {
     return lds_mat_n(material_count) + lds_win_n(sphere_count) + lds_pln_n(plane_count);
 }
+
+static_assert(sizeof(rt_material) % 16 == 0, "the staged scene block follows the materials 16-byte aligned");
+PT_HD size_t stage_block_offset(uint32_t material_count) { return (size_t)(material_count ? material_count : 1u) * sizeof(rt_material); }
 
 struct PixelRec {
     float4 p_kind;
diff --git a/opencl-raytracing_amd/csrc/rt_amd.hip b/opencl-raytracing_amd/csrc/rt_amd.hip
--- a/opencl-raytracing_amd/csrc/rt_amd.hip
+++ b/opencl-raytracing_amd/csrc/rt_amd.hip
@@ -595,7 +595,9 @@
     HIP_TRY(ctx, hipSetDevice(ctx->device));
     HIP_TRY(ctx, hipStreamSynchronize(ctx->stream));
     ctx->have_scene = false;
-    HIP_TRY(ctx, ctx->materials.upload(d->materials, d->material_count));
+    HIP_TRY(ctx, ctx->materials.upload(d->materials, d->material_count,
+                                       lds_static_used(d->material_count, d->sphere_count, d->plane_count) * sizeof(float4)));
+    ctx->stage_block.generation = ~0ull;
     HIP_TRY(ctx, ctx->spheres.upload(d->spheres, d->sphere_count));
     ctx->h_spheres.assign(d->spheres, d->spheres + d->sphere_count);
     ctx->h_bvh_idx.clear();
@@ -1748,6 +1750,42 @@
     return RT_OK;
 }
 
+int rt_debug_queue_pixels(uint32_t count, uint32_t waves_per_simd, uint32_t static_float4, uint32_t granule, uint32_t *pixels_out) {
+    if (!pixels_out || count < 1u || waves_per_simd < 1u || waves_per_simd > 8u || static_float4 > PT_LDS_STATIC_FLOAT4 ||
+        (granule != 0u && (granule < 16u || granule > 8192u)))
+        return RT_EINVAL;
+    *pixels_out = pt::kernel_set_a2()->queue_pixels(count, waves_per_simd, static_float4, granule);
+    return RT_OK;
+}
+
+int rt_debug_queue_occupancy(rt_context *ctx, uint32_t lds_bytes, int *blocks_out) {
+    if (!ctx || !blocks_out) return RT_EINVAL;
+    HIP_TRY(ctx, hipSetDevice(ctx->device));
+    return ctx->ks->queue_occupancy(ctx, lds_bytes, blocks_out);
+}
+
+int rt_debug_wave_fixed(rt_context *ctx, uint64_t out[2]) {
+    if (!ctx || !out) return RT_EINVAL;
+    out[0] = ctx->sample_grid.count64_launches;
+    out[1] = ctx->stage_block.builds;
+    return RT_OK;
+}
+
+int rt_debug_stage_block(rt_context *ctx, float *out, size_t capacity_float4, uint32_t *float4_out) {
+    if (!ctx || !float4_out) return RT_EINVAL;
+    if (!ctx->have_scene || ctx->stage_block.generation != ctx->prefix_cache.generation)
+        return fail(ctx, RT_EINVAL, "the staged scene block is not built (no fused launch since the last change)");
+    const uint32_t n = lds_static_used((uint32_t)ctx->materials.n, (uint32_t)ctx->spheres.n, (uint32_t)ctx->planes.n);
+    *float4_out = n;
+    if (n == 0) return RT_OK;
+    if (!out || capacity_float4 < n) return fail(ctx, RT_EINVAL, "the staged scene block holds %u float4", n);
+    HIP_TRY(ctx, hipSetDevice(ctx->device));
+    HIP_TRY(ctx, hipMemcpyAsync(out, reinterpret_cast<const char *>(ctx->materials.p) + stage_block_offset((uint32_t)ctx->materials.n),
+                                n * sizeof(float4), hipMemcpyDeviceToHost, ctx->stream));
+    HIP_TRY(ctx, hipStreamSynchronize(ctx->stream));
+    return RT_OK;
+}
+
 int rt_reset_counters(rt_context *ctx) {
     if (!ctx) return RT_EINVAL;
     HIP_TRY(ctx, hipSetDevice(ctx->device));
diff --git a/opencl-raytracing_amd/csrc/rt_context.hpp b/opencl-raytracing_amd/csrc/rt_context.hpp
--- a/opencl-raytracing_amd/csrc/rt_context.hpp
+++ b/opencl-raytracing_amd/csrc/rt_context.hpp
@@ -31,10 +31,10 @@
         n = count;
         return e;
     }
-    hipError_t upload(const T *src, size_t count) {
+    hipError_t upload(const T *src, size_t count, size_t tail_bytes = 0) {
         release();
         size_t alloc = count ? count : 1;
-        hipError_t e = hipMalloc((void **)&p, alloc * sizeof(T));
+        hipError_t e = hipMalloc((void **)&p, alloc * sizeof(T) + tail_bytes);
         if (e != hipSuccess) { p = nullptr; return e; }
         n = count;
         if (count) e = hipMemcpy(p, src, count * sizeof(T), hipMemcpyHostToDevice);
@@ -129,6 +129,10 @@
         uint32_t count_light = 0, count_heavy = 0;
     } prefix_cache;
     void prefix_changed() { prefix_cache.generation++; }
+    struct StageBlock {
+        uint64_t generation = ~0ull;
+        uint64_t builds = 0;
+    } stage_block;
     struct SampleGrid {
         bool exact = true;
         uint32_t *h_counts = nullptr;
@@ -138,6 +142,7 @@
         uint64_t workgroups = 0;
         uint64_t live_last = 0;
         uint32_t last_cap = 0, last_per_unit = 0;
+        uint64_t count64_launches = 0;
     } sample_grid;
     struct Lookahead {
         int k = 16;
diff --git a/opencl-raytracing_amd/raytracer.py b/opencl-raytracing_amd/raytracer.py
--- a/opencl-raytracing_amd/raytracer.py
+++ b/opencl-raytracing_amd/raytracer.py
@@ -23,7 +23,7 @@
     "rt_denoise_variance", "rt_read_variance", "rt_device_variance",
     "rt_read_moments", "rt_device_moments", "rt_moments_merge", "rt_denoise_moments",
     "rt_prefix_cache_stats", "rt_lookahead_stats", "rt_lookahead_plan",
-    "rt_sample_units", "rt_sample_grid_stats", "rt_debug_live_list", "rt_debug_queue_sums",
+    "rt_sample_units", "rt_sample_grid_stats", "rt_debug_live_list", "rt_debug_wave_fixed", "rt_debug_stage_block", "rt_debug_queue_pixels", "rt_debug_queue_occupancy", "rt_debug_queue_sums",
 )
 
 OPT_PREFIX_SHARING, OPT_MAX_THREADS_PER_LAUNCH, OPT_SAMPLE_QUEUE, OPT_ACCEL, OPT_WALK_SLICES, OPT_ARITH, OPT_PREFIX_TREE, OPT_WAVE_FILL = 1, 2, 3, 4, 5, 6, 7, 8
@@ -194,6 +194,14 @@
                                          "version": 3, "strides": None}
 
 
+def queue_pixels(count, waves_per_simd=6, static_float4=0, granule=0):
+    n = C.c_uint32()
+    rc = load_library().rt_debug_queue_pixels(int(count), int(waves_per_simd), int(static_float4), int(granule), C.byref(n))
+    if rc:
+        raise RtError(rc, "rt_debug_queue_pixels: invalid argument")
+    return int(n.value)
+
+
 class RayTracer:
     DEFAULT_SCENE = os.path.join("assets", "scenes", "scene.scene")
     REPO_DEFAULT_SCENE = os.path.join(os.path.dirname(_HERE), "assets", "scenes", "scene.scene")
@@ -527,6 +535,23 @@
         self._check(self._lib.rt_debug_live_list(self._ctx, out))
         return tuple(int(v) for v in out)
 
+    def waveFixedStats(self):
+        out = (C.c_uint64 * 2)()
+        self._check(self._lib.rt_debug_wave_fixed(self._ctx, out))
+        return tuple(int(v) for v in out)
+
+    def queueOccupancy(self, lds_bytes):
+        n = C.c_int()
+        self._check(self._lib.rt_debug_queue_occupancy(self._ctx, int(lds_bytes), C.byref(n)))
+        return int(n.value)
+
+    def stageBlock(self):
+        cap = 2 * 64 + 2 * 64 + 16
+        out = np.zeros((cap, 4), dtype=np.float32)
+        n = C.c_uint32()
+        self._check(self._lib.rt_debug_stage_block(self._ctx, out.ctypes.data, cap, C.byref(n)))
+        return out[:n.value].copy()
+
     def setArith(self, arith):
         if isinstance(arith, str):
             arith = ARITH_NAMES[arith]
```

Result: faster. 123,900, median of 6 (+3.9%).
